# 2235854410/CCVPE

Measured on AMD Instinct MI355X. Metric: query images/sec (VIGOR, 512x512 sat / 320x640 grd), higher is better.
Workload: dtype f32; 1 GPU; vigor_samearea_fov360_b32; variant=vigor_ori_prior, batch_per_gpu=32, global_batch=32, parallelism=image-parallel x1, all_gather of 20 B/query results, schedule=two streams per GPU (aerial encoder + orientation decoder on the second)

## Files before the change

ccvpe_amd/csrc/ccvpe_api.hip:

```cpp
#include "ccvpe_internal.h"

namespace ccvpe { thread_local unsigned long long g_launches = 0; }
static thread_local std::string g_err_storage;
std::string& ccvpe_err() { return g_err_storage; }
int ccvpe_fail(int code, const char* fmt, ...) {
    char buf[1024];
    va_list ap;
    va_start(ap, fmt);
    vsnprintf(buf, sizeof(buf), fmt, ap);
    va_end(ap);
    g_err_storage = buf;
    return code;
}

__global__ __launch_bounds__(256) void checksum_kernel(const uint32_t* __restrict__ p, size_t n, unsigned long long* out) {
    unsigned long long s = 0;
    for (size_t i = (size_t)blockIdx.x * 256 + threadIdx.x; i < n; i += (size_t)gridDim.x * 256) s += (unsigned long long)p[i] * (unsigned long long)((i & 1023) + 1);
    for (int o = 32; o > 0; o >>= 1) s += __shfl_down(s, o);
    if ((threadIdx.x & 63) == 0) atomicAdd(out, s);
}


Switches read_switches() {
    Switches s;
    auto set = [](const char* name) { return getenv(name) != nullptr; };
    auto off = [](const char* name) { const char* e = getenv(name); return e && std::atoi(e) == 0; };
    if (const char* e = getenv("CCVPE_AUTOTUNE")) s.autotune = std::atoi(e) != 0;
    if (const char* e = getenv("CCVPE_FUSE_MBCONV")) s.fuse_mbconv = std::atoi(e);
    if (const char* e = getenv("CCVPE_FUSE_L1")) s.fuse_level1 = std::atoi(e) != 0;
    if (const char* e = getenv("CCVPE_L1_TILE")) s.l1_tile = std::atoi(e);
    if (const char* e = getenv("CCVPE_COMPOSE_L6")) s.compose_l6 = std::atoi(e);
    if (const char* e = getenv("CCVPE_WINOGRAD")) s.wino = std::atoi(e) != 0;
    if (const char* e = getenv("CCVPE_GRAPH")) s.graph_mode = std::atoi(e) != 0;
    if (const char* e = getenv("CCVPE_STREAMS")) s.two_streams = std::atoi(e) >= 2;
    if (const char* e = getenv("CCVPE_PRECISION")) s.precision = (std::string(e) == "bf16x3") ? 1 : 0;
    s.stem_dw = !off("CCVPE_STEM_DW");
    if (const char* e = getenv("CCVPE_FRONT_SPREAD")) s.front_spread = std::atoi(e);
    s.mbconv_image = !off("CCVPE_MBCONV_IMAGE");
    s.se_ticket = !off("CCVPE_SE_TICKET");
    if (const char* e = getenv("CCVPE_SE_PROLOGUE")) s.se_prologue = std::atoi(e) == 1;
    s.split_planes = !set("CCVPE_NO_SPLIT_PLANES");
    s.match_prep_early = !off("CCVPE_MATCH_PREP_EARLY");
    s.match_wide = !off("CCVPE_MATCH_WIDE");
    s.issue_interleaved = !off("CCVPE_ISSUE_ORDER");
    s.log_schedule = set("CCVPE_LOG_SCHEDULE");
    s.no_reuse = set("CCVPE_NO_REUSE");
    s.tune_prefer_pw = set("CCVPE_TUNE_PREFER_PW");
    if (const char* e = getenv("CCVPE_TUNE_PREFER_PROJ")) { s.tune_prefer_proj = true; s.tune_prefer_lat = std::strcmp(e, "lat") == 0; }
    if (const char* e = getenv("CCVPE_TUNE_SPLITK")) s.tune_splitk = std::atoi(e);
    s.tune_no_bf16x3 = set("CCVPE_TUNE_NO_BF16X3");
    s.no_pw = set("CCVPE_NO_PW");
    s.tune_ignore_table = set("CCVPE_TUNE_IGNORE_TABLE");
    s.tune_lat_rows = set("CCVPE_TUNE_LAT_ROWS");
    s.tune_lat_split = set("CCVPE_TUNE_LAT_SPLIT");
    s.tune_no_fused_split = set("CCVPE_TUNE_NO_FUSED_SPLIT");
    if (const char* e = getenv("CCVPE_TUNE_VERBOSE")) s.tune_verbose = e;
    s.no_proj = set("CCVPE_NO_PROJ");
    if (const char* e = getenv("CCVPE_WINO4_MIN_N")) s.wino4_min_n = std::atoi(e);
    s.no_wino4 = set("CCVPE_NO_WINO4");
    s.no_wino4x = set("CCVPE_NO_WINO4X");
    s.pad_concat = !off("CCVPE_PAD_CONCAT");
    if (const char* e = getenv("CCVPE_DIAG_SYNC_BEFORE")) s.diag_sync = e;
    if (const char* e = getenv("CCVPE_DIAG_SNAP")) s.diag_snap = e;
    return s;
}

static int max_micro_batch(const Switches& sw, int variant, float ori_noise, int grd_h, int grd_w) {
    if (variant < 0 || variant > 3) return ccvpe_fail(CCVPE_EINVAL, "unknown variant %d", variant);
    ccvpe_handle_s tmp;
    tmp.cfg.variant = variant; tmp.cfg.ori_noise = ori_noise; tmp.cfg.micro_batch = 1;
    tmp.vs = make_variant(variant);
    tmp.sw = sw;
    tmp.sw.fuse_mbconv = 0; tmp.sw.fuse_level1 = false; tmp.sw.two_streams = false; tmp.sw.graph_mode = 0;
    const int n = (int)(ori_noise / 18.f);
    for (int k = 0; k < 6; ++k) tmp.rolls[k] = (variant == CCVPE_VARIANT_VIGOR_ORI_PRIOR && k > 0) ? 2 * n + 1 : tmp.vs.n_rolls;
    int lo = 0, hi = 1024;
    while (hi - lo > 1) {
        const int mid = (lo + hi) / 2;
        Plan pl;
        PlanKey key;
        key.B = mid; key.gh = grd_h; key.gw = grd_w;
        if (build_plan(&tmp, pl, key) == 0) lo = mid; else hi = mid;
    }
    if (lo == 0) return ccvpe_fail(CCVPE_EINVAL, "ground size %d x %d is not valid for variant %d: %s", grd_h, grd_w, variant, ccvpe_err().c_str());
    return lo;
}

extern "C" {

const char* ccvpe_last_error(void) { return ccvpe_err().c_str(); }
const char* ccvpe_version(void) { return "ccvpe-hip 0.1 (gfx950, fp32 MFMA)"; }
uint64_t ccvpe_launch_count(void) { return ccvpe::g_launches; }

int ccvpe_create(const ccvpe_config* cfg, ccvpe_handle* out) {
    if (!cfg || !out) return ccvpe_fail(CCVPE_EINVAL, "null argument");
    if (cfg->variant < 0 || cfg->variant > 3) return ccvpe_fail(CCVPE_EINVAL, "unknown variant %d", cfg->variant);
    int ndev = 0;
    if (hipGetDeviceCount(&ndev) != hipSuccess || ndev <= 0)
        return ccvpe_fail(CCVPE_EHIP, "no HIP device visible: libccvpe_hip has no CPU fallback");
    if (cfg->device < 0 || cfg->device >= ndev) return ccvpe_fail(CCVPE_EINVAL, "device %d out of range (%d visible)", cfg->device, ndev);
    HIPCHK(hipSetDevice(cfg->device));
    hipDeviceProp_t prop;
    HIPCHK(hipGetDeviceProperties(&prop, cfg->device));
    if (std::string(prop.gcnArchName).find("gfx950") == std::string::npos)
        return ccvpe_fail(CCVPE_EHIP, "device %d is %s; this library carries gfx950 code objects only", cfg->device, prop.gcnArchName);
    auto* h = new ccvpe_handle_s();
    h->cfg = *cfg;
    if (h->cfg.micro_batch <= 0) h->cfg.micro_batch = 32;
    h->vs = make_variant(cfg->variant);
    h->sw = read_switches();
    if (h->sw.precision) h->cfg.reserved[0] = *h->sw.precision;
    if (h->cfg.reserved[0] != 0 && h->cfg.reserved[0] != 1) { delete h; return ccvpe_fail(CCVPE_EINVAL, "unknown precision mode %d", cfg->reserved[0]); }
    const int n = (int)(cfg->ori_noise / 18.f);
    for (int k = 0; k < 6; ++k)
        h->rolls[k] = (cfg->variant == CCVPE_VARIANT_VIGOR_ORI_PRIOR && k > 0) ? 2 * n + 1 : h->vs.n_rolls;
    if (cfg->variant == CCVPE_VARIANT_VIGOR_ORI_PRIOR && (n < 0 || 2 * n + 1 > 32)) {
        delete h;
        return ccvpe_fail(CCVPE_EINVAL, "ori_noise %.1f out of range", cfg->ori_noise);
    }
    build_expect(h);
    *out = h;
    return 0;
}

int ccvpe_max_micro_batch(int32_t variant, float ori_noise, int32_t grd_h, int32_t grd_w) {
    return max_micro_batch(read_switches(), variant, ori_noise, grd_h, grd_w);
}

int ccvpe_destroy(ccvpe_handle h) {
    if (!h) return 0;
    (void)hipSetDevice(h->cfg.device);
    for (void* p : h->dev_allocs) (void)hipFree(p);
    release_level6(h);
    if (h->arena) (void)hipFree(h->arena);
    for (auto* buf : {&h->post_scratch, &h->topk_scratch, &h->prior_scratch}) if (buf->ptr) (void)hipFree(buf->ptr);
    h->plans.clear();
    for (int k = 0; k < 2; ++k) if (h->snap[k]) (void)hipFree(h->snap[k]);
    if (h->capture_stream) (void)hipStreamDestroy(h->capture_stream);
    if (h->aux_stream) (void)hipStreamDestroy(h->aux_stream);
    delete h;
    return 0;
}

int ccvpe_output_channels(ccvpe_handle h, int32_t level) {
    if (!h || level < 0 || level > 5) return ccvpe_fail(CCVPE_EINVAL, "bad level");
    return h->rolls[level];
}

size_t ccvpe_workspace_bytes(ccvpe_handle h, int32_t batch, int32_t grd_h, int32_t grd_w) {
    if (!h || !h->finalized || batch <= 0) { ccvpe_fail(CCVPE_ESTATE, "handle not ready"); return 0; }
    Plan pl;
    PlanKey key;
    key.B = std::min(batch, h->cfg.micro_batch); key.gh = grd_h; key.gw = grd_w;
    if (build_plan(h, pl, key)) return 0;
    return pl.total * sizeof(float);
}

}

static void check_issued_tile(Plan& pl, const Op& op) {
    const int got = conv_tile_last();
    if (!op.tile || (*op.tile & 0xff) == 0 || got == 0) return;
    const int want = *op.tile, ws = (want >> 8) & 0xff, gs = (got >> 8) & 0xff;
    if ((want & 0xff) != (got & 0xff) || (ws > 1 ? ws : 1) != (gs > 1 ? gs : 1))
        std::fprintf(stderr, "ccvpe: launch %s (batch %d) runs %s split %d instead of the planned %s split %d\n", op.name.c_str(), pl.key.B,
                     conv_tile_name(got), gs, conv_tile_name(want), ws);
}

static int run_ops(ccvpe_handle h, Plan& pl, const Ctx& base, hipStream_t s0) {
    const bool check = !pl.tiles_checked;
    pl.tiles_checked = true;
    if (check) (void)conv_tile_last();
    if (!pl.two_streams || h->serial_issue) {
        Ctx c = base;
        c.stream = s0;
        for (auto& op : pl.ops) { op.fn(c); if (check) check_issued_tile(pl, op); }
        base.conv_errors += c.conv_errors;
        return 0;
    }
    if (!h->aux_stream) HIPCHK(hipStreamCreateWithFlags(&h->aux_stream, hipStreamNonBlocking));
    if (pl.events.empty()) {
        pl.events.assign(pl.ops.size() + 2, nullptr);
        for (size_t i = 0; i < pl.events.size(); ++i)
            if (i >= pl.ops.size() || pl.ops[i].signal) HIPCHK(hipEventCreateWithFlags(&pl.events[i], hipEventDisableTiming));
    }
    Ctx c[2] = {base, base};
    hipStream_t st[2] = {s0, h->aux_stream};
    c[0].stream = st[0];
    c[1].stream = st[1];
    pl.set_scratch(c[1], 1);
    const size_t n = pl.ops.size();
    HIPCHK(hipEventRecord(pl.events[n], st[0]));
    HIPCHK(hipStreamWaitEvent(st[1], pl.events[n], 0));
    for (size_t k = 0; k < n; ++k) {
        const size_t i = pl.issue_order.size() == n ? (size_t)pl.issue_order[k] : k;
        Op& op = pl.ops[i];
        for (int d : op.wait_on) HIPCHK(hipStreamWaitEvent(st[op.stream], pl.events[d], 0));
        if (!h->sw.diag_sync.empty() && op.name.find(h->sw.diag_sync) != std::string::npos) HIPCHK(hipDeviceSynchronize());
        const bool snap = !h->sw.diag_snap.empty() && op.name == h->sw.diag_snap;
        auto take_snap = [&](int which) -> int {
            if (!h->snap[0]) {
                h->snap_layout.clear();
                size_t o = 0;
                for (int id : op.uses) { h->snap_layout.push_back({id, o}); o += (pl.size[id] + 63) & ~(size_t)63; }
                h->snap_floats = o;
                for (int k = 0; k < 2; ++k) HIPCHK(hipMalloc((void**)&h->snap[k], o * sizeof(float)));
            }
            for (auto& e : h->snap_layout)
                HIPCHK(hipMemcpyAsync(h->snap[which] + e.second, base.arena + pl.off[e.first], pl.size[e.first] * sizeof(float), hipMemcpyDeviceToDevice, st[op.stream]));
            return 0;
        };
        if (snap) { if (int r = take_snap(0)) return r; }
        op.fn(c[op.stream]);
        if (check) check_issued_tile(pl, op);
        if (snap) { if (int r = take_snap(1)) return r; }
        if (op.signal) HIPCHK(hipEventRecord(pl.events[i], st[op.stream]));
    }
    HIPCHK(hipEventRecord(pl.events[n + 1], st[1]));
    HIPCHK(hipStreamWaitEvent(st[0], pl.events[n + 1], 0));
    base.conv_errors += c[0].conv_errors + c[1].conv_errors;
    return 0;
}

static int micro_batch_cap(ccvpe_handle h, int gh, int gw) {
    int mbmax = h->cfg.micro_batch;
    auto it = h->mb_cap.find({gh, gw});
    if (it == h->mb_cap.end()) {
        const std::string keep = ccvpe_err();
        const int cap = max_micro_batch(h->sw, h->cfg.variant, h->cfg.ori_noise, gh, gw);
        ccvpe_err() = keep;
        it = h->mb_cap.emplace(std::make_pair(gh, gw), cap).first;
    }
    if (it->second > 0) mbmax = std::min(mbmax, it->second);
    return mbmax;
}

static int launch_status(const char* what) {
    hipError_t e = hipGetLastError();
    if (e != hipSuccess) return ccvpe_fail(CCVPE_EHIP, "%s failed: %s", what, hipGetErrorString(e));
    return 0;
}

static Ctx plan_ctx(ccvpe_handle h, const Plan& pl, hipStream_t stream) {
    Ctx c;
    c.arena = h->arena; c.off = &pl.off; c.stream = stream;
    c.tickets = pl.tickets;
    pl.set_scratch(c, 0);
    return c;
}

template <class Slice>
static int for_each_micro_batch(ccvpe_handle h, PlanKey key, int total, hipStream_t stream, Slice slice) {
    const int mbmax = micro_batch_cap(h, key.gh, key.gw);
    for (int pass = 0; pass < 2; ++pass)
        for (int done = 0; done < total; done += key.B) {
            key.B = std::min(mbmax, total - done);
            Plan* pl;
            if (int rc = get_plan(h, key, &pl)) return rc;
            if (pass == 0) continue;
            h->last_plan = pl;
            Ctx c = plan_ctx(h, *pl, stream);
            if (int rc = slice(pl, c, done, key.B)) return rc;
            if (c.conv_errors) return ccvpe_fail(CCVPE_EINVAL, "%d convolution launches were refused (unsupported geometry)", c.conv_errors);
        }
    return 0;
}

static int issue_forward(ccvpe_handle h, Plan* pl, Ctx& c, const ForwardCall& fc, int mb) {
    const int gh = fc.gh, gw = fc.gw;
    const bool profile = fc.profile;
    hipStream_t stream = fc.stream;
    const size_t npx = (size_t)CCVPE_OUT_HW * CCVPE_OUT_HW;
    if (!profile && pl->use_graph && !h->debug) {
        const ccvpe_outputs user = c.out;
        const float* ugrd = c.grd; const float* usat = c.sat;
        c.grd = c.ptr(pl->io_grd); c.sat = c.ptr(pl->io_sat);
        c.out.logits_flattened = c.ptr(pl->io_logits); c.out.heatmap = c.ptr(pl->io_heat); c.out.ori = c.ptr(pl->io_ori);
        for (int k = 0; k < 6; ++k) c.out.matching_score[k] = c.ptr(pl->io_ms[k]);
        {
            const size_t ng = (size_t)mb * 3 * gh * gw, ns = (size_t)mb * 3 * CCVPE_SAT_HW * CCVPE_SAT_HW;
            if (ng % 4 == 0 && ((uintptr_t)ugrd % 16) == 0 && ((uintptr_t)usat % 16) == 0) {
                MultiCopy mc{};
                mc.src[0] = ugrd; mc.dst[0] = (float*)c.grd; mc.n[0] = ng;
                mc.src[1] = usat; mc.dst[1] = (float*)c.sat; mc.n[1] = ns;
                mc.count = 2;
                launch_multi_copy(mc, stream);
            } else {
                HIPCHK(hipMemcpyAsync((void*)c.grd, ugrd, ng * sizeof(float), hipMemcpyDeviceToDevice, stream));
                HIPCHK(hipMemcpyAsync((void*)c.sat, usat, ns * sizeof(float), hipMemcpyDeviceToDevice, stream));
            }
        }
        if (!pl->exec && pl->runs >= 1) {
            hipGraph_t graph = nullptr;
            if (!h->capture_stream) HIPCHK(hipStreamCreateWithFlags(&h->capture_stream, hipStreamNonBlocking));
            HIPCHK(hipStreamBeginCapture(h->capture_stream, hipStreamCaptureModeThreadLocal));
            const int rrc = run_ops(h, *pl, c, h->capture_stream);
            hipError_t ce = hipStreamEndCapture(h->capture_stream, &graph);
            if (rrc) ce = hipErrorUnknown;
            if (ce == hipSuccess && graph) {
                hipGraphExec_t ex = nullptr;
                if (hipGraphInstantiate(&ex, graph, nullptr, nullptr, 0) == hipSuccess) pl->exec = ex;
                (void)hipGraphDestroy(graph);
            }
            if (!pl->exec) { (void)hipGetLastError(); pl->use_graph = false; }
        }
        if (pl->exec) HIPCHK(hipGraphLaunch(pl->exec, stream));
        else if (int rrc = run_ops(h, *pl, c, stream)) return rrc;
        pl->runs++;
        {
            MultiCopy mc{};
            auto add = [&](float* dst, const float* src, size_t n) { mc.src[mc.count] = src; mc.dst[mc.count] = dst; mc.n[mc.count] = n; ++mc.count; };
            add(user.logits_flattened, c.out.logits_flattened, (size_t)mb * npx);
            add(user.heatmap, c.out.heatmap, (size_t)mb * npx);
            add(user.ori, c.out.ori, (size_t)mb * 2 * npx);
            bool aligned = true;
            for (int k = 0; k < 6; ++k) add(user.matching_score[k], c.out.matching_score[k], (size_t)mb * h->rolls[k] * ((size_t)(8 << k) * (8 << k)));
            for (int i = 0; i < mc.count; ++i) aligned = aligned && mc.n[i] % 4 == 0 && ((uintptr_t)mc.dst[i] % 16) == 0 && ((uintptr_t)mc.src[i] % 16) == 0;
            if (aligned) launch_multi_copy(mc, stream);
            else
                for (int i = 0; i < mc.count; ++i) HIPCHK(hipMemcpyAsync(mc.dst[i], mc.src[i], mc.n[i] * sizeof(float), hipMemcpyDeviceToDevice, stream));
        }
    } else if (!profile) {
        if (int rrc = run_ops(h, *pl, c, stream)) return rrc;
    } else {
        hipEvent_t e0, e1;
        HIPCHK(hipEventCreate(&e0));
        HIPCHK(hipEventCreate(&e1));
        for (auto& op : pl->ops) {
            (void)conv_tile_last();
            HIPCHK(hipEventRecord(e0, stream));
            op.fn(c);
            HIPCHK(hipEventRecord(e1, stream));
            HIPCHK(hipEventSynchronize(e1));
            float ms = 0.f;
// ... 1059 lines not shown
```

ccvpe_amd/csrc/ccvpe_internal.h:

```cpp
#pragma once
#include "../../include/ccvpe.h"
#include "kernels.h"

#include <algorithm>
#include <cmath>
#include <cstdarg>
#include <cstdio>
#include <cstdlib>
#include <cstring>
#include <functional>
#include <map>
#include <memory>
#include <optional>
#include <set>
#include <string>
#include <type_traits>
#include <vector>

using namespace ccvpe;

std::string& ccvpe_err();
int ccvpe_fail(int code, const char* fmt, ...);
#define HIPCHK(expr)                                                                           \
    do {                                                                                       \
        hipError_t _e = (expr);                                                                \
        if (_e != hipSuccess) return ccvpe_fail(CCVPE_EHIP, "%s failed: %s", #expr, hipGetErrorString(_e)); \
    } while (0)

struct BlockSpec { int e, k, s, cin, cout; };
static const BlockSpec B0[16] = {
    {1, 3, 1, 32, 16}, {6, 3, 2, 16, 24}, {6, 3, 1, 24, 24}, {6, 5, 2, 24, 40}, {6, 5, 1, 40, 40},
    {6, 3, 2, 40, 80}, {6, 3, 1, 80, 80}, {6, 3, 1, 80, 80}, {6, 5, 1, 80, 112}, {6, 5, 1, 112, 112},
    {6, 5, 1, 112, 112}, {6, 5, 2, 112, 192}, {6, 5, 1, 192, 192}, {6, 5, 1, 192, 192}, {6, 5, 1, 192, 192},
    {6, 3, 1, 192, 320},
};
static const int TAP_BLOCK[5] = {15, 10, 4, 2, 0};
static const float BN_EPS = 1e-3f;

struct DecLevel { int din, dout, skip, mid, out; };
struct VariantSpec {
    int feat_h;
    int head_ch[6];
    int sat_desc;
    int match_ch[6];
    int step[6];
    int n_rolls;
    int centre;
    DecLevel loc[6], ori[6];
};
static const DecLevel VIGOR_LOC[6] = {{1281, 1024, 320, 640, 640}, {641, 320, 112, 320, 320}, {321, 160, 40, 160, 160},
                                      {161, 80, 24, 80, 80},       {81, 40, 16, 40, 40},      {41, 16, 0, 16, 1}};
static const DecLevel VIGOR_ORI[6] = {{1300, 1024, 320, 640, 640}, {640, 256, 112, 256, 256}, {256, 128, 40, 128, 128},
                                      {128, 64, 24, 64, 64},       {64, 32, 16, 32, 32},      {32, 16, 0, 16, 2}};
static const DecLevel KITTI_LOC[6] = {{2049, 1024, 320, 512, 512}, {513, 256, 112, 256, 256}, {257, 128, 40, 128, 128},
                                      {129, 64, 24, 128, 128},     {129, 32, 16, 32, 32},     {33, 16, 0, 16, 1}};
static const DecLevel KITTI_ORI[6] = {{2064, 1024, 320, 512, 512}, {512, 256, 112, 256, 256}, {256, 128, 40, 128, 128},
                                      {128, 64, 24, 64, 64},       {64, 32, 16, 32, 32},      {32, 16, 0, 16, 2}};

static VariantSpec make_variant(int v) {
    VariantSpec s{};
    auto cp = [](DecLevel* d, const DecLevel* src) { for (int i = 0; i < 6; ++i) d[i] = src[i]; };
    if (v == CCVPE_VARIANT_KITTI) {
        s.feat_h = 8;
        int hc[6] = {16, 8, 4, 2, 1, 1}, mc[6] = {2048, 512, 256, 128, 128, 32}, st[6] = {128, 64, 32, 16, 8, 8};
        for (int i = 0; i < 6; ++i) { s.head_ch[i] = hc[i]; s.match_ch[i] = mc[i]; s.step[i] = st[i]; }
        s.sat_desc = 2048; s.n_rolls = 16; s.centre = 0;
        cp(s.loc, KITTI_LOC); cp(s.ori, KITTI_ORI);
    } else {
        int mc[6] = {1280, 640, 320, 160, 80, 40}, st[6] = {64, 32, 16, 8, 4, 2};
        int hv[6] = {64, 32, 16, 8, 4, 2}, ho[6] = {32, 16, 8, 4, 2, 1};
        for (int i = 0; i < 6; ++i) {
            s.match_ch[i] = mc[i]; s.step[i] = st[i];
            s.head_ch[i] = (v == CCVPE_VARIANT_OXFORD) ? ho[i] : hv[i];
        }
        s.feat_h = (v == CCVPE_VARIANT_OXFORD) ? 4 : 10;
        s.sat_desc = 1280; s.n_rolls = 20; s.centre = (v == CCVPE_VARIANT_OXFORD);
        cp(s.loc, VIGOR_LOC); cp(s.ori, VIGOR_ORI);
    }
    return s;
}

static void static_pad(int k, int s, int& lo, int& hi) {
    if (s == 1) { lo = hi = (k - 1) / 2; return; }
    int total = k - 2;
    lo = total / 2; hi = total - lo;
}
static int conv_out(int n, int k, int s) {
    int lo, hi; static_pad(k, s, lo, hi);
    return (n + lo + hi - k) / s + 1;
}
static int se_squeeze(int cin) { return std::max(1, (int)(cin * 0.25)); }
static int round_up(int a, int b) { return (a + b - 1) / b * b; }
static int deconv_width(const DecLevel& l, bool pad) {
    return (pad && l.skip > 0 && (l.dout * 4) % 64 != 0) ? round_up(l.dout, 16) : l.dout;
}

struct Switches {
    bool autotune = true;
    int fuse_mbconv = 1;
    bool fuse_level1 = true;
    int l1_tile = 1;
    std::optional<int> compose_l6;
    bool wino = true;
    int graph_mode = 0;
    bool two_streams = true;
    std::optional<int> precision;
    bool stem_dw = true;
    std::optional<int> front_spread;
    bool mbconv_image = true;
    bool se_ticket = true;
    bool se_prologue = false;
    bool split_planes = true;
    bool match_prep_early = true;
    bool match_wide = true;
    bool issue_interleaved = true;
    bool log_schedule = false;
    bool no_reuse = false;
    bool tune_prefer_pw = false;
    bool tune_prefer_proj = false;
    bool tune_prefer_lat = false;
    std::optional<int> tune_splitk;
    bool tune_no_bf16x3 = false;
    bool no_pw = false;
    bool tune_ignore_table = false;
    bool tune_lat_rows = false;
    bool tune_lat_split = false;
    bool tune_no_fused_split = false;
    std::string tune_verbose;
    bool no_proj = false;
    int wino4_min_n = 40;
    bool no_wino4 = false;
    bool no_wino4x = false;
    bool pad_concat = true;
    std::string diag_sync, diag_snap;

    bool tune_filtered() const {
        return tune_prefer_pw || tune_prefer_proj || tune_splitk || tune_no_bf16x3 || no_pw || tune_ignore_table || tune_lat_rows || tune_lat_split ||
               tune_no_fused_split;
    }
    std::string pack_group() const {
        std::string s;
        if (no_proj) s += "CCVPE_NO_PROJ=1;";
        if (wino4_min_n != 40) s += "CCVPE_WINO4_MIN_N=" + std::to_string(wino4_min_n) + ";";
        if (no_wino4) s += "CCVPE_NO_WINO4=1;";
        if (no_wino4x) s += "CCVPE_NO_WINO4X=1;";
        if (!pad_concat) s += "CCVPE_PAD_CONCAT=0;";
        return s;
    }
};
Switches read_switches();

struct PackedConv {
    float* w = nullptr;
    unsigned short *w_hi = nullptr, *w_lo = nullptr;
    float* bias = nullptr;
    int N = 0, Kpad = 0, nchunks = 0, cinp = 0, KH = 1, KW = 1;
    float* wino = nullptr;
    int wino_n16 = 0;
    size_t wino_bytes = 0;
    float* wino4 = nullptr;
    size_t wino4_bytes = 0;
    float* wino4x = nullptr;
    size_t wino4x_bytes = 0;
    int wino4x_cfg = -1;
    float* proj = nullptr;
    size_t proj_bytes = 0;
};
struct BlockW {
    PackedConv expand, project;
    float* exp_lin = nullptr;
    int exp_cinp = 0;
    float *dw_w = nullptr, *dw_b = nullptr, *se_w1 = nullptr, *se_b1 = nullptr, *se_w2 = nullptr, *se_b2 = nullptr;
    int sq = 0;
};
struct EncoderW {
    float *stem_w = nullptr, *stem_b = nullptr;
    BlockW blk[16];
    PackedConv head;
};
struct DecoderW {
    PackedConv deconv[6], conva[6], convb[5];
    float* tail_w = nullptr;
    float* l1_wt = nullptr;
    float tail_b[2] = {0.f, 0.f};
    float *l1_wc = nullptr, *l1_ws = nullptr, *l1_bc = nullptr;
    int l1_cx = 0, l1_cxp = 0, l1_c0 = 0, l1_ng = 0, l1_score = 0;
};
struct Level6W {
    float* wc = nullptr;
    float* bc = nullptr;
    PackedConv skip;
    int K = 0, Kc = 0, N = 0, Npad = 0;
};
static constexpr int LEVEL6_AUTO_MIN_BATCH = 8;
struct ccvpe_handle_s;
struct DecoderW;
int level6_shape(const ccvpe_handle_s* h, const DecoderW& d, const struct DecLevel& l, int& K, int& Kc, int& N, int& Npad);
int ensure_level6(ccvpe_handle_s* h, int wm);
void release_level6(ccvpe_handle_s* h);
int compose_level1(ccvpe_handle_s* h, DecoderW& d, const std::vector<float>& w, const std::vector<float>& b, const std::vector<float>& wa,
                   const std::vector<float>& ba, int cin, int nscore);
int pack_level1_tail(ccvpe_handle_s* h, DecoderW& d, const std::vector<float>& w2, const std::vector<float>& b2, int cout);

struct Tensor {
    int id = -1; int B = 0, H = 0, W = 0, C = 0;
    bool split = false;
    long long numel() const { return (long long)B * H * W * C; }
};

struct Ctx {
    float* arena = nullptr;
    const std::vector<size_t>* off = nullptr;
    hipStream_t stream = nullptr;
    const float* grd = nullptr;
    const float* sat = nullptr;
    ccvpe_outputs out{};
    float* splitk_scratch = nullptr;
    size_t splitk_floats = 0;
    unsigned* tickets = nullptr;
    const float* cache_in = nullptr;
    float* cache_out = nullptr;
    float* rows = nullptr;
    int topk_k = 0, topk_r = 0;
    const int* tile_index = nullptr;
    int n_tiles = 0;
    const float* grd_cache_in = nullptr;
    const int* query_index = nullptr;
    int n_queries = 0;
    float* stats = nullptr;
    const float* log_prior = nullptr;
    long long prior_stride = 0;
    float* posterior = nullptr;
    float* summary = nullptr;
    int summary_r = 0;
    float* heading = nullptr;
    float* hist = nullptr;
    int heading_bins = 0, heading_r = 0;
    float* ptr(const Tensor& t) const { return arena + (*off)[t.id]; }
    Dst dst(const Tensor& t, int coff = 0) const { return Dst{ptr(t), t.C, coff, t.split ? 1 : 0, t.numel()}; }
    mutable int conv_errors = 0;
    mutable size_t conv_tick_off = 0;
    mutable ConvParams* probe = nullptr;
    void launch_conv(ConvParams& p, int cfg) const {
        p.tickets = tickets ? tickets + conv_tick_off : nullptr;
        p.partial = splitk_scratch;
        p.partial_floats = splitk_floats;
        if (probe) { *probe = p; return; }
        if (launch_conv_igemm(p, cfg, stream) != 0) ++conv_errors;
    }
};

struct PlanKey {
    int B = 0, gh = 0, gw = 0;
    int mode = 0;
    bool pose = false;
    bool topk = false;
    bool summary = false;
    bool heading = false;
    bool operator==(const PlanKey& o) const {
        return B == o.B && gh == o.gh && gw == o.gw && mode == o.mode && pose == o.pose && topk == o.topk && summary == o.summary &&
               heading == o.heading;
    }
};

struct ForwardCall {
    const float* grd = nullptr;
    int gh = 0, gw = 0;
    const float* sat = nullptr;
    const float* cache = nullptr;
    const int32_t* tile_index = nullptr;
    int n_tiles = 0;
    int batch = 0;
    const ccvpe_outputs* out = nullptr;
    float* rows = nullptr;
    int topk_k = 0, topk_r = 0;
    const float* log_prior = nullptr;
    long long prior_stride = 0;
    float* posterior = nullptr;
    float* summary = nullptr;
    int summary_r = 0;
    float* heading = nullptr;
    float* hist = nullptr;
    int heading_bins = 0, heading_r = 0;
    hipStream_t stream = nullptr;
    bool profile = false;
    PlanKey plan_key() const {
        PlanKey key;
        key.gh = gh; key.gw = gw; key.mode = cache ? 2 : 0; key.pose = rows != nullptr; key.topk = rows && topk_k > 0;
        key.summary = rows && summary;
        key.heading = rows && heading;
        return key;
    }
};

struct Op {
    std::string name;
    std::function<void(const Ctx&)> fn;
    std::vector<int> uses;
    double flops = 0, bytes = 0;
    std::shared_ptr<int> tile;
    int gemm_m = 0, gemm_n = 0, gemm_kpad = 0;
    int conv_cin = 0;
    bool bf16x3_only = false;
    bool wino_ok = false;
    bool wino4_ok = false;
    bool wino4x_ok = false;
    bool is_pw = false;
    bool proj_ok = false;
    int stream = 0;
    std::vector<int> wait_on;
    bool signal = false;
};

struct TapInfo { Tensor t; int coff; int C; };

struct Plan {
    PlanKey key;
    bool debug = false;
    std::vector<size_t> size;
    std::vector<size_t> off;
    std::vector<Op> ops;
    std::map<std::string, TapInfo> taps;
    size_t total = 0;
    float* arena = nullptr;
    Tensor scratch;
    bool use_graph = false;
    Tensor io_grd, io_sat, io_logits, io_heat, io_ori, io_ms[6];
    Tensor tune_cache;
    hipGraphExec_t exec = nullptr;
    int runs = 0;
    size_t ticket_words = 0;
    unsigned* tickets = nullptr;
    size_t alloc_tickets(size_t n) { const size_t o = ticket_words; ticket_words += (n + 15) & ~(size_t)15; return o; }
    int l6_wm = 0;
    bool tiles_checked = false;
    bool two_streams = false;
    Tensor scratch2;
    std::vector<hipEvent_t> events;
    std::vector<int> issue_order;
    bool issue_interleaved = true, log_schedule = false, no_reuse = false;
    ~Plan() {
        if (exec) (void)hipGraphExecDestroy(exec);
        for (hipEvent_t e : events) if (e) (void)hipEventDestroy(e);
        if (tickets) (void)hipFree(tickets);
    }
    void schedule() {
        if (!two_streams) return;
        bool any = false;
        for (auto& o : ops) {
            o.stream = (o.name.rfind("sat.", 0) == 0 || o.name.rfind("ori", 0) == 0) ? 1 : 0;
            any = any || o.stream == 1;
            o.wait_on.clear();
            o.signal = false;
        }
        if (!any) { two_streams = false; return; }
        std::map<int, int> last_use;
        for (int i = 0; i < (int)ops.size(); ++i) {
            int dep = -1;
            for (int id : ops[i].uses) {
                auto it = last_use.find(id);
                if (it != last_use.end() && ops[it->second].stream != ops[i].stream) dep = std::max(dep, it->second);
            }
            if (dep >= 0) { ops[i].wait_on.push_back(dep); ops[dep].signal = true; }
            for (int id : ops[i].uses) last_use[id] = i;
        }
        issue_order.clear();
        {
            std::vector<int> q[2];
            for (int i = 0; i < (int)ops.size(); ++i) q[ops[i].stream].push_back(i);
            size_t p[2] = {0, 0};
            std::vector<bool> issued(ops.size(), false);
            while (issue_interleaved && (p[0] < q[0].size() || p[1] < q[1].size())) {
                auto ready = [&](int s) {
                    if (p[s] >= q[s].size()) return false;
                    for (int d : ops[q[s][p[s]]].wait_on) if (!issued[d]) return false;
                    return true;
                };
                const bool r0 = ready(0), r1 = ready(1);
                int s;
                if (r0 && r1) s = (p[1] * q[0].size() < p[0] * q[1].size()) ? 1 : 0;
                else if (r0 || r1) s = r0 ? 0 : 1;
                else { issue_order.clear(); break; }
                const int i = q[s][p[s]++];
                issued[i] = true;
                issue_order.push_back(i);
            }
            if (issue_order.size() != ops.size()) { issue_order.resize(ops.size()); for (int i = 0; i < (int)ops.size(); ++i) issue_order[i] = i; }
        }
        if (log_schedule)
            for (int i = 0; i < (int)ops.size(); ++i) {
                std::fprintf(stderr, "op %3d s%d %-28s wait=%d uses=", i, ops[i].stream, ops[i].name.c_str(), ops[i].wait_on.empty() ? -1 : ops[i].wait_on[0]);
                for (int id : ops[i].uses) std::fprintf(stderr, "%d ", id);
                std::fprintf(stderr, "\n");
            }
    }
    static constexpr size_t SPLITK_FLOATS = 32u << 20;
    void set_scratch(Ctx& c, int stream) const {
        const Tensor& sk = stream ? scratch2 : scratch;
        c.splitk_scratch = c.ptr(sk); c.splitk_floats = SPLITK_FLOATS;
    }

    size_t max_tensor_bytes = 0;
    int max_dims[4] = {0, 0, 0, 0};
    Tensor alloc(int B_, int H, int W, int C) {
        Tensor t; t.id = (int)size.size(); t.B = B_; t.H = H; t.W = W; t.C = C;
        size.push_back((size_t)B_ * H * W * C);
        if (size.back() * sizeof(float) > max_tensor_bytes) {
            max_tensor_bytes = size.back() * sizeof(float);
            max_dims[0] = B_; max_dims[1] = H; max_dims[2] = W; max_dims[3] = C;
        }
        return t;
    }
    void add(const std::string& name, std::vector<Tensor> uses, std::function<void(const Ctx&)> fn, double flops = 0, double bytes = 0) {
        Op o; o.name = name; o.fn = std::move(fn); o.flops = flops; o.bytes = bytes;
        for (auto& t : uses) o.uses.push_back(t.id);
        ops.push_back(std::move(o));
    }
    void add_conv(const std::string& name, std::vector<Tensor> uses, int gemm_m, int gemm_n, int gemm_kpad,
                  std::function<void(const Ctx&, int)> fn, double flops, double bytes) {
        auto tp = std::make_shared<int>(TILE_AUTO);
        const size_t toff = alloc_tickets(CONV_TICKETS);
        add(name, std::move(uses), [fn, tp, toff](const Ctx& c) { c.conv_tick_off = toff; fn(c, *tp); }, flops, bytes);
        ops.back().tile = tp;
        ops.back().gemm_m = gemm_m;
        ops.back().gemm_n = gemm_n;
        ops.back().gemm_kpad = gemm_kpad;
    }
    void assign() {
        const int n = (int)size.size();
        std::vector<int> first(n, 1 << 30), last(n, -1), smask(n, 0);
        for (int i = 0; i < (int)ops.size(); ++i)
            for (int id : ops[i].uses) {
                first[id] = std::min(first[id], i); last[id] = std::max(last[id], i);
                smask[id] |= 1 << (two_streams ? ops[i].stream : 0);
            }
        std::vector<bool> pinned(n, false);
        auto pin = [&](const Tensor& t) { if (t.id >= 0) { pinned[t.id] = true; first[t.id] = 0; last[t.id] = 1 << 30; } };
        if (debug || no_reuse) for (int i = 0; i < n; ++i) if (last[i] >= 0) pinned[i] = true;
        pin(scratch); pin(scratch2); pin(tune_cache);
        if (use_graph)
            for (const Tensor* t : {&io_grd, &io_sat, &io_logits, &io_heat, &io_ori, &io_ms[0], &io_ms[1], &io_ms[2], &io_ms[3], &io_ms[4], &io_ms[5]}) pin(*t);
        for (int i = 0; i < n; ++i) if (smask[i] == 3) pinned[i] = true;
        off.assign(n, 0);
        std::vector<int> order(n);
        for (int i = 0; i < n; ++i) order[i] = i;
        std::stable_sort(order.begin(), order.end(), [&](int a, int b) { return first[a] < first[b]; });
        auto granule = [&](int id) { return (size[id] + 63) & ~(size_t)63; };
        total = 0;
        for (int pool = 1; pool <= 2; ++pool) {
            const size_t base = total;
            std::vector<int> placed;
            for (int id : order) {
                if (last[id] < 0 || pinned[id] || smask[id] != pool) continue;
                const size_t sz = granule(id);
                std::vector<std::pair<size_t, size_t>> busy;
                for (int o : placed)
                    if (!(last[o] < first[id] || last[id] < first[o])) busy.push_back({off[o], off[o] + granule(o)});
                std::sort(busy.begin(), busy.end());
                size_t pos = base;
                for (auto& iv : busy) {
                    if (pos + sz <= iv.first) break;
                    pos = std::max(pos, iv.second);
                }
                off[id] = pos;
                total = std::max(total, pos + sz);
                placed.push_back(id);
            }
        }
        for (int id : order) {
            if (last[id] < 0 || !pinned[id]) continue;
            off[id] = total;
            total += granule(id);
        }
    }
};

struct ccvpe_handle_s {
    ccvpe_config cfg{};
    VariantSpec vs{};
    int rolls[6] = {0};
    std::map<std::string, std::vector<int64_t>> expect;
    std::map<std::string, std::vector<float>> host;
    std::set<std::string> skipped;
    bool finalized = false;
    bool debug = false;
    Switches sw;
    hipStream_t capture_stream = nullptr;
    hipStream_t aux_stream = nullptr;
    bool serial_issue = false;
    std::vector<void*> dev_allocs;
    std::vector<size_t> dev_alloc_bytes;
    EncoderW grd_enc, sat_enc;
    PackedConv grd_heads, sat_desc;
    float* grd_wh[6] = {nullptr};
    float grd_b2[6] = {0};
    DecoderW loc, ori;
    Level6W l6[2];
    int l6_wm = 0;
    std::vector<void*> l6_allocs;
    bool l6_failed = false;
    std::vector<std::unique_ptr<Plan>> plans;
    Plan* last_plan = nullptr;
    float* snap[2] = {nullptr, nullptr};
    size_t snap_floats = 0;
    std::vector<std::pair<int, size_t>> snap_layout;
    std::map<std::pair<int, int>, int> mb_cap;
    std::map<std::string, std::pair<std::string, int>> tuning;
    int tuned_plans = 0;
    float* arena = nullptr;
    size_t arena_floats = 0;
    struct Scratch { void* ptr = nullptr; int batch = 0; };
    Scratch post_scratch;
    Scratch topk_scratch;
    Scratch prior_scratch;
    struct Row { std::string name; float ms; double flops, bytes, issued; };
    std::vector<Row> prof;
};


void build_expect(ccvpe_handle_s* h);
int pack_conv(ccvpe_handle_s* h, PackedConv& pc, int N, int taps, int cin, int cinp, const std::vector<int>& cmap,
              const std::function<float(int, int, int)>& get, const std::vector<float>& bias, int KH, int KW);
std::vector<int> identity_map(int n);
static inline int score_pad(int nscore) { return round_up(nscore, 8); }

ConvParams conv_params(const PackedConv& pc, const float* in, int in_ld, int B, int H, int W, int OH, int OW,
                       int stride, int pad_t, int pad_l, int act);
size_t cache_layout(const VariantSpec& vs, int B, size_t off[6]);
int ground_desc_floats(const ccvpe_handle_s* h, int gh, int gw);
int build_plan(ccvpe_handle_s* h, Plan& pl, const PlanKey& key);

int autotune_plan(ccvpe_handle_s* h, Plan& pl, const std::vector<bool>* known = nullptr);
int get_plan(ccvpe_handle_s* h, const PlanKey& key, Plan** out);
std::string tuning_key(ccvpe_handle_s* h, const Plan& pl, const Op& op);
```

ccvpe_amd/csrc/ccvpe_plan.hip:

```cpp
#include "ccvpe_internal.h"

static int window_offset(const VariantSpec& vs, int level, int L) {
    const int C = vs.match_ch[level];
    return vs.centre ? (int)((double)C / 2 - (double)L / 2) : 0;
}
static int mod(int a, int m) { int r = a % m; return r < 0 ? r + m : r; }

ConvParams conv_params(const PackedConv& pc, const float* in, int in_ld, int B, int H, int W, int OH, int OW,
                              int stride, int pad_t, int pad_l, int act) {
    ConvParams p{};
    p.in = in; p.in_ld = in_ld; p.B = B; p.H = H; p.W = W; p.Cin = pc.cinp; p.OH = OH; p.OW = OW;
    p.KH = pc.KH; p.KW = pc.KW; p.stride = stride; p.pad_t = pad_t; p.pad_l = pad_l;
    p.wpk = pc.w; p.w_hi = pc.w_hi; p.w_lo = pc.w_lo; p.Kpad = pc.Kpad; p.Npad = round_up(pc.N, conv_igemm_npad()); p.nchunks = pc.nchunks; p.bias = pc.bias; p.N = pc.N; p.act = act;
    p.gate = nullptr; p.resid = nullptr; p.resid_ld = 0; p.ndst = 0; p.mode = MODE_CONV; p.deconv_cout = 0;
    p.M = B * OH * OW;
    p.in_bytes = (unsigned)((size_t)B * H * W * in_ld * sizeof(float));
    p.gate_bytes = (unsigned)((size_t)B * pc.cinp * sizeof(float));
    p.w_plane_bytes = (unsigned)((size_t)p.Npad * pc.Kpad * sizeof(unsigned short));
    p.wino_w = pc.wino; p.wino_n16 = pc.wino_n16; p.wino_bytes = (unsigned)pc.wino_bytes;
    p.wino4_w = pc.wino4; p.wino4_bytes = (unsigned)pc.wino4_bytes;
    p.wino4x_w = pc.wino4x; p.wino4x_bytes = (unsigned)pc.wino4x_bytes; p.wino4x_cfg = pc.wino4x_cfg;
    p.proj_w = pc.proj; p.proj_bytes = (unsigned)pc.proj_bytes;
    return p;
}

struct EncOut { Tensor vol; Tensor tap[16]; };

struct TapDst { Tensor t[2]; int coff[2]; int n = 0; };

static void plan_encoder(ccvpe_handle_s* h, Plan& pl, const EncoderW& ew, bool is_grd, int B, int H, int W, bool circular,
                         const TapDst* tapdst, EncOut& out, const std::string& tag) {
    int lo, hi;
    static_pad(3, 2, lo, hi);
    int ch = conv_out(H, 3, 2), cw = conv_out(W, 3, 2);
    const bool stem_dw = h->sw.stem_dw && B0[0].e == 1 && B0[0].k == 3 && B0[0].s == 1 && B0[0].cin == 32 && !(circular && (W & 1)) &&
                         (size_t)B * 3 * H * W * sizeof(float) < ((size_t)1 << 31);
    StemParams stem_sp{};
    stem_sp.B = B; stem_sp.H = H; stem_sp.W = W; stem_sp.OH = ch; stem_sp.OW = cw; stem_sp.pad_t = lo; stem_sp.pad_l = lo; stem_sp.circular = circular;
    stem_sp.w = ew.stem_w; stem_sp.bias = ew.stem_b;
    Tensor cur = stem_dw ? Tensor{} : pl.alloc(B, ch, cw, 32);
    if (!stem_dw) {
        const StemParams sp = stem_sp;
        Tensor o = cur;
        pl.add(tag + ".stem", {o}, [sp, o, is_grd](const Ctx& c) {
            StemParams q = sp; q.in = is_grd ? c.grd : c.sat; q.out = c.ptr(o);
            launch_stem(q, c.stream);
        }, 2.0 * B * ch * cw * 32 * 27, 4.0 * B * (3.0 * H * W + 32.0 * ch * cw));
    }
    for (int i = 0; i < 16; ++i) {
        const BlockSpec& b = B0[i];
        const BlockW& bw = ew.blk[i];
        const int mid = b.cin * b.e;
        const std::string bn = tag + ".b" + std::to_string(i);
        Tensor xin = cur;
        Tensor e = xin;
        static_pad(b.k, b.s, lo, hi);
        const int oh = conv_out(ch, b.k, b.s), ow = conv_out(cw, b.k, b.s);
        MbFrontParams mp{};
        mp.B = B; mp.H = ch; mp.W = cw; mp.Cin = b.cin; mp.cinp = bw.exp_cinp; mp.mid = mid;
        mp.we = bw.exp_lin; mp.be = bw.expand.bias; mp.wd = bw.dw_w; mp.bd = bw.dw_b;
        mp.k = b.k; mp.s = b.s; mp.pad_t = lo; mp.pad_l = lo; mp.circular = circular; mp.OH = oh; mp.OW = ow;
        {
            const double share = (double)H * W / ((double)H * W + (double)CCVPE_SAT_HW * CCVPE_SAT_HW);
            const int dflt = is_grd ? std::max(64, std::min(128, (int)(256.0 * share / 16.0 + 0.5) * 16)) : 144;
            mp.spread = h->sw.front_spread.value_or(dflt);
        }
        const bool image = b.e != 1 && bw.exp_lin != nullptr && h->sw.fuse_mbconv != 0 && h->sw.mbconv_image && mbconv_image_supported(mp);
        const bool fused = image || (b.e != 1 && bw.exp_lin != nullptr && mbconv_front_supported(b.k, b.s, b.cin, mid) &&
                           (h->sw.fuse_mbconv == 2 || (h->sw.fuse_mbconv == 1 && mbconv_front_profitable(b.k))));
        Tensor d = pl.alloc(B, oh, ow, mid);
        const bool with_stem = stem_dw && i == 0;
        const bool ticket_on = h->sw.se_ticket && mid <= 1152 && bw.sq <= 64;
        const int trows = !ticket_on ? 0 : with_stem ? stem_dw_tiles(oh, ow) : image ? mbconv_image_ticket_rows(mp) : fused ? mbconv_front_ticket_rows(mp) : 0;
        bool sep = false;
        if (trows > 0 && image && bw.project.proj != nullptr && h->cfg.reserved[0] == 0 && h->sw.se_prologue) {
            ConvParams q = conv_params(bw.project, nullptr, mid, B, oh, ow, oh, ow, 1, 0, 0, ACT_NONE);
            q.M = B * oh * ow;
            q.se_rows = reinterpret_cast<const float*>(1); q.se_nrows = trows * (mid / 16); q.se_sq = bw.sq;
            sep = conv_proj_supported(q, 101);
        }
        const bool ticket = trows > 0 && !sep;
        const int S = ticket ? trows : with_stem ? stem_dw_tiles(oh, ow) : image ? mbconv_image_strips(mp) : fused ? mbconv_front_tiles(b.k, b.s, oh, ow) : depthwise_strip_lanes(B, oh, ow, mid, b.k, b.s);
        Tensor pool = pl.alloc(B, 1, S, mid);
        Tensor gate = pl.alloc(B, 1, 1, mid);
        SeTicket se{};
        size_t tick_off = 0;
        if (sep) {
            se.per_sample = trows * (mid / 16);
            se.S = trows; se.C = mid; se.SQ = bw.sq; se.inv_hw = 1.f / (float)(oh * ow);
            se.w1 = bw.se_w1;
        }
        if (ticket) {
            tick_off = pl.alloc_tickets((size_t)B);
            se.per_sample = with_stem ? S : image ? S * (mid / 16) : S * mbconv_front_ticket_split(mp);
            se.S = S; se.C = mid; se.SQ = bw.sq; se.inv_hw = 1.f / (float)(oh * ow);
            se.w1 = bw.se_w1; se.b1 = bw.se_b1; se.w2 = bw.se_w2; se.b2 = bw.se_b2;
            se.spec = (long long)B * se.per_sample <= 256 ? 1 : 0;
        }
        const bool parts = (ticket && image) || sep;
        Tensor sqp = parts ? pl.alloc(B, 1, se.per_sample, bw.sq) : Tensor{};
        auto fill_se = [=](const Ctx& c) {
            SeTicket t = se;
            if (ticket) { t.counter = c.tickets + tick_off; t.pool = c.ptr(pool); t.gate = c.ptr(gate); }
            if (parts) t.sqpart = c.ptr(sqp);
            return t;
        };
        const double se_flops = ticket ? 4.0 * B * mid * bw.sq : 0.0;
        if (with_stem) {
            StemDwParams sd{};
            sd.st = stem_sp; sd.wd = bw.dw_w; sd.bd = bw.dw_b;
            std::vector<Tensor> uses = {d, pool};
            if (ticket) uses.push_back(gate);
            pl.add(tag + ".stem_b0dw", uses, [=](const Ctx& c) {
                StemDwParams q = sd; q.st.in = is_grd ? c.grd : c.sat; q.out = c.ptr(d); q.pool_partial = c.ptr(pool); q.se = fill_se(c);
                launch_stem_dw(q, c.stream);
            }, 2.0 * B * ch * cw * 32 * 27 + 2.0 * B * oh * ow * mid * 9 + se_flops, 4.0 * B * (3.0 * H * W + 32.0 * oh * ow));
        } else if (fused) {
            std::vector<Tensor> uses = {xin, d, pool};
            if (ticket) uses.push_back(gate);
            if (parts) uses.push_back(sqp);
            (void)sep;
            pl.add(bn + ".expand_dw", uses, [=](const Ctx& c) {
                MbFrontParams q = mp; q.x = c.ptr(xin); q.out = c.ptr(d); q.pool = c.ptr(pool); q.se = fill_se(c);
                if (image) launch_mbconv_image(q, c.stream); else launch_mbconv_front(q, c.stream);
            }, 2.0 * B * ch * cw * b.cin * mid + 2.0 * B * oh * ow * mid * b.k * b.k + se_flops, 4.0 * B * ((double)ch * cw * b.cin + (double)oh * ow * mid));
        } else {
        if (b.e != 1) {
            e = pl.alloc(B, ch, cw, mid);
            const PackedConv* pc = &bw.expand;
            const int hh = ch, ww = cw;
            pl.add_conv(bn + ".expand", {xin, e}, B * hh * ww, pc->N, pc->Kpad, [=](const Ctx& c, int tile) {
                ConvParams p = conv_params(*pc, c.ptr(xin), xin.C, B, hh, ww, hh, ww, 1, 0, 0, ACT_SWISH);
                p.dst[0] = {c.ptr(e), mid, 0}; p.ndst = 1;
                c.launch_conv(p, tile);
            }, 2.0 * B * ch * cw * b.cin * mid, 4.0 * B * ch * cw * (b.cin + mid));
            pl.ops.back().is_pw = true;
        }
        {
            DwParams dp{};
            dp.B = B; dp.H = ch; dp.W = cw; dp.C = mid; dp.OH = oh; dp.OW = ow; dp.k = b.k; dp.stride = b.s;
            dp.pad_t = lo; dp.pad_l = lo; dp.circular = circular; dp.w = bw.dw_w; dp.bias = bw.dw_b; dp.S = S;
            pl.add(bn + ".dw", {e, d, pool}, [=](const Ctx& c) {
                DwParams q = dp; q.in = c.ptr(e); q.out = c.ptr(d); q.pool_partial = c.ptr(pool);
                launch_depthwise(q, c.stream);
            }, 2.0 * B * oh * ow * mid * b.k * b.k, 4.0 * B * mid * ((double)ch * cw + (double)oh * ow));
        }
        }
        const int SC = std::max(1, std::min(16, S / 32));
        Tensor pooled = pl.alloc(B, 1, SC, mid);
        Tensor sqt = pl.alloc(B, 1, 1, 64);
        if (!ticket && !sep) {
            SeParams sp{};
            sp.B = B; sp.S = S; sp.C = mid; sp.SQ = bw.sq; sp.inv_hw = 1.f / (float)(oh * ow); sp.SC = SC;
            sp.w1 = bw.se_w1; sp.b1 = bw.se_b1; sp.w2 = bw.se_w2; sp.b2 = bw.se_b2;
            pl.add(bn + ".se", {pool, gate, pooled, sqt}, [=](const Ctx& c) {
                SeParams q = sp; q.pool_partial = c.ptr(pool); q.gate = c.ptr(gate); q.pooled = c.ptr(pooled); q.sq = c.ptr(sqt);
                launch_se(q, c.stream);
            }, 4.0 * B * mid * bw.sq, 4.0 * B * S * mid);
        }
        Tensor o = pl.alloc(B, oh, ow, b.cout);
        {
            const PackedConv* pc = &bw.project;
            const bool skip = (b.s == 1 && b.cin == b.cout);
            TapDst td;
            if (tapdst) for (int t = 0; t < 5; ++t) if (TAP_BLOCK[t] == i) td = tapdst[t];
            std::vector<Tensor> uses = {d, sep ? sqp : gate, o};
            if (skip) uses.push_back(xin);
            for (int t = 0; t < td.n; ++t) uses.push_back(td.t[t]);
            const int se_nrows = se.per_sample, se_sq = bw.sq;
            const float se_inv = se.inv_hw;
            const float *se_b1 = bw.se_b1, *se_w2 = bw.se_w2, *se_b2 = bw.se_b2;
            pl.add_conv(bn + (sep ? ".se_project" : ".project"), uses, B * oh * ow, pc->N, pc->Kpad, [=](const Ctx& c, int tile) {
                ConvParams p = conv_params(*pc, c.ptr(d), mid, B, oh, ow, oh, ow, 1, 0, 0, ACT_NONE);
                if (sep) {
                    p.se_rows = c.ptr(sqp); p.se_nrows = se_nrows; p.se_sq = se_sq; p.se_inv_hw = se_inv; p.se_b1 = se_b1; p.se_w2 = se_w2; p.se_b2 = se_b2;
                    tile = conv_proj_lat_tile();
                } else {
                    p.gate = c.ptr(gate);
                }
                if (skip) { p.resid = c.ptr(xin); p.resid_ld = xin.C; }
                p.dst[0] = {c.ptr(o), o.C, 0}; p.ndst = 1;
                for (int t = 0; t < td.n; ++t) p.dst[p.ndst++] = c.dst(td.t[t], td.coff[t]);
                c.launch_conv(p, tile);
            }, 2.0 * B * oh * ow * mid * b.cout + (sep ? 4.0 * B * mid * bw.sq : 0.0), 4.0 * B * oh * ow * (mid + b.cout * (1 + td.n)));
            pl.ops.back().is_pw = true;
            pl.ops.back().proj_ok = pc->proj != nullptr && h->cfg.reserved[0] == 0;
            if (sep) pl.ops.back().tile.reset();
        }
        out.tap[i] = o;
        pl.taps[tag + "_block" + std::to_string(i)] = {o, 0, o.C};
        cur = o; ch = oh; cw = ow;
    }
    Tensor vol = pl.alloc(B, ch, cw, 1280);
    {
        const PackedConv* pc = &ew.head;
        Tensor x = cur;
        const int hh = ch, ww = cw;
        pl.add_conv(tag + ".head", {x, vol}, B * hh * ww, pc->N, pc->Kpad, [=](const Ctx& c, int tile) {
            ConvParams p = conv_params(*pc, c.ptr(x), x.C, B, hh, ww, hh, ww, 1, 0, 0, ACT_SWISH);
            p.dst[0] = {c.ptr(vol), 1280, 0}; p.ndst = 1;
            c.launch_conv(p, tile);
        }, 2.0 * B * ch * cw * 320 * 1280, 4.0 * B * ch * cw * 1600);
        pl.ops.back().is_pw = true;
    }
    out.vol = vol;
    pl.taps[tag + "_volume"] = {vol, 0, 1280};
}

static const int TAP_HW[5] = {256, 1024, 4096, 16384, 65536};
static const int TAP_C[5] = {320, 112, 40, 24, 16};
size_t cache_layout(const VariantSpec& vs, int B, size_t off[6]) {
    size_t o = 0;
    off[0] = o; o += (size_t)B * 64 * vs.sat_desc;
    for (int t = 0; t < 5; ++t) { off[t + 1] = o; o += (size_t)B * TAP_HW[t] * TAP_C[t]; }
    return o;
}

static int build_aerial_plan(ccvpe_handle_s* h, Plan& pl, int B);
static int build_ground_plan(ccvpe_handle_s* h, Plan& pl, int B, int gh, int gw);
extern "C" int ccvpe_max_micro_batch(int32_t variant, float ori_noise, int32_t grd_h, int32_t grd_w);

static int grd_geometry(const VariantSpec& vs, bool circular, int gh, int gw, int& fh, int& fw, int L[6]) {
    if (gh <= 0 || gw <= 0) return ccvpe_fail(CCVPE_EINVAL, "ground image size %d x %d is not positive", gh, gw);
    fh = gh; fw = gw;
    for (int i = -1; i < 16; ++i) {
        const int k = i < 0 ? 3 : B0[i].k, s = i < 0 ? 2 : B0[i].s;
        int lo, hi;
        static_pad(k, s, lo, hi);
        const std::string layer = i < 0 ? "the stem" : "block " + std::to_string(i);
        if (fh + lo + hi < k || fw + lo + hi < k)
            return ccvpe_fail(CCVPE_EINVAL, "ground image %d x %d is too small: it reaches the %d x %d kernel of %s as %d x %d", gh, gw, k, k,
                              layer.c_str(), fh, fw);
        if (circular && fw < std::max(lo, hi))
            return ccvpe_fail(CCVPE_EINVAL, "ground image %d x %d is too narrow for circular padding: %s pads %d columns around a width of %d "
                              "(the padding would wrap more than once)", gh, gw, layer.c_str(), std::max(lo, hi), fw);
        fh = conv_out(fh, k, s); fw = conv_out(fw, k, s);
    }
    if (fh != vs.feat_h)
        return ccvpe_fail(CCVPE_EINVAL, "ground image %dx%d gives a %d-row feature volume, the descriptor heads expect %d rows", gh, gw, fh, vs.feat_h);
    for (int k = 0; k < 6; ++k) {
        L[k] = fw * vs.head_ch[k];
        if (L[k] > vs.match_ch[k])
            return ccvpe_fail(CCVPE_EINVAL, "descriptor length %d exceeds aerial channels %d at level %d", L[k], vs.match_ch[k], k + 1);
    }
    return 0;
}

int ground_desc_floats(const ccvpe_handle_s* h, int gh, int gw) {
    int fh, fw, L[6];
    if (int rc = grd_geometry(h->vs, h->cfg.circular_padding != 0, gh, gw, fh, fw, L)) return rc;
    int ltot = 0;
    for (int k = 0; k < 6; ++k) ltot += round_up(L[k], 4);
    return ltot;
}

static Tensor plan_grd_desc(ccvpe_handle_s* h, Plan& pl, int B, int fh, int fw, Tensor vol, bool to_cache) {
    const VariantSpec& vs = h->vs;
    int ntot = 0, ltot = 0, hoff[6], loff[6];
    for (int k = 0; k < 6; ++k) { hoff[k] = ntot; ntot += vs.head_ch[k]; loff[k] = ltot; ltot += round_up(fw * vs.head_ch[k], 4); }
    Tensor ghead = pl.alloc(B, fh, fw, ntot);
    Tensor desc = to_cache ? Tensor{} : pl.alloc(B, 1, 1, ltot);
    const PackedConv* pc = &h->grd_heads;
    Tensor x = vol;
    pl.add_conv("grd.heads", {x, ghead}, B * fh * fw, pc->N, pc->Kpad, [=](const Ctx& c, int tile) {
        ConvParams p = conv_params(*pc, c.ptr(x), 1280, B, fh, fw, fh, fw, 1, 0, 0, ACT_NONE);
        p.dst[0] = {c.ptr(ghead), ntot, 0}; p.ndst = 1;
        c.launch_conv(p, tile);
    }, 2.0 * B * fh * fw * 1280 * ntot, 4.0 * B * fh * fw * (1280 + ntot));
    pl.ops.back().is_pw = true;
    pl.ops.back().proj_ok = pc->proj != nullptr && h->cfg.reserved[0] == 0;
    GrdDescParams gp{};
    gp.B = B; gp.Hf = fh; gp.Wf = fw; gp.Ntot = ntot; gp.nlev = 6; gp.Ltot = ltot;
    for (int k = 0; k < 6; ++k) { gp.c[k] = vs.head_ch[k]; gp.off[k] = hoff[k]; gp.wh[k] = h->grd_wh[k]; gp.b2[k] = h->grd_b2[k]; gp.loff[k] = loff[k]; }
    std::vector<Tensor> uses = {ghead};
    if (!to_cache) uses.push_back(desc);
    pl.add("grd.desc", uses, [=](const Ctx& c) {
        GrdDescParams q = gp; q.y = c.ptr(ghead); q.desc = to_cache ? c.cache_out : c.ptr(desc);
        launch_grd_desc(q, c.stream);
    }, 2.0 * B * fh * fw * ntot, 4.0 * B * fh * fw * ntot);
    return desc;
}

int build_plan(ccvpe_handle_s* h, Plan& pl, const PlanKey& key) {
    const int B = key.B, gh = key.gh, gw = key.gw, mode = key.mode;
    const bool pose = key.pose;
    pl.key = key;
    pl.key.topk = pose && key.topk;
    pl.key.summary = pose && !key.topk && key.summary;
    pl.key.heading = key.heading;
    if (key.heading && (!pose || key.topk || mode == 4)) return ccvpe_fail(CCVPE_EINVAL, "heading plans are argmax pose plans (no top-K, no pairs)");
    if (mode == 1) return build_aerial_plan(h, pl, B);
    if (mode == 3) return build_ground_plan(h, pl, B, gh, gw);
    const bool cached = mode == 2 || mode == 4;
    const bool grd_cached = mode == 4;
    if (grd_cached && (!pose || key.topk)) return ccvpe_fail(CCVPE_EINVAL, "pair plans are single-hypothesis pose plans");
    const VariantSpec& vs = h->vs;
    pl.debug = h->debug;
    pl.scratch = pl.alloc(1, 1, 1, (int)Plan::SPLITK_FLOATS);
    pl.two_streams = h->sw.two_streams && !h->debug;
    pl.issue_interleaved = h->sw.issue_interleaved; pl.log_schedule = h->sw.log_schedule; pl.no_reuse = h->sw.no_reuse;
    if (pl.two_streams) pl.scratch2 = pl.alloc(1, 1, 1, (int)Plan::SPLITK_FLOATS);
    pl.use_graph = !cached && !pose && h->sw.graph_mode == 1;
    if (pl.use_graph) {
        pl.io_grd = pl.alloc(B, 3, gh, gw);
        pl.io_sat = pl.alloc(B, 3, CCVPE_SAT_HW, CCVPE_SAT_HW);
        pl.io_logits = pl.alloc(B, 1, CCVPE_OUT_HW, CCVPE_OUT_HW);
        pl.io_heat = pl.alloc(B, 1, CCVPE_OUT_HW, CCVPE_OUT_HW);
        pl.io_ori = pl.alloc(B, 2, CCVPE_OUT_HW, CCVPE_OUT_HW);
        for (int k = 0; k < 6; ++k) pl.io_ms[k] = pl.alloc(B, h->rolls[k], 8 << k, 8 << k);
    }

    int fh, fw, L[6];
    if (int rc = grd_geometry(vs, h->cfg.circular_padding != 0, gh, gw, fh, fw, L)) return rc;

    const int D = vs.sat_desc;
    const int rfull = vs.n_rolls;
    const int rpad = score_pad(rfull);
    Tensor loc_in[6], ori_in6;
    Tensor loc_cat[6], ori_cat[6];
    for (int j = 0; j < 6; ++j) {
        const int hw_in = 8 << j;
        loc_in[j] = pl.alloc(B, hw_in, hw_in, 8 + vs.match_ch[j]);
        loc_cat[j] = pl.alloc(B, hw_in * 2, hw_in * 2, deconv_width(vs.loc[j], h->sw.pad_concat) + vs.loc[j].skip);
        ori_cat[j] = pl.alloc(B, hw_in * 2, hw_in * 2, deconv_width(vs.ori[j], h->sw.pad_concat) + vs.ori[j].skip);
        if (h->cfg.reserved[0] == 1 && j < 5 && h->sw.split_planes) { loc_cat[j].split = true; ori_cat[j].split = true; }
    }
    const bool l6_forced = h->sw.compose_l6 && (*h->sw.compose_l6 == 1 || *h->sw.compose_l6 == 2);
    int l6_wm = !h->finalized || h->cfg.reserved[0] != 0 || !h->sw.wino ? 0
                : h->sw.compose_l6 ? (*h->sw.compose_l6 == 1 ? 4 : *h->sw.compose_l6 == 2 ? 2 : 0)
                : (B >= LEVEL6_AUTO_MIN_BATCH && !h->l6_failed) ? 4 : 0;
    Level6Params l6p[2] = {};
    if (l6_wm) {
        bool ok = true;
        for (int d = 0; d < 2; ++d) {
            Level6Params& q = l6p[d];
            q.wm = l6_wm; q.B = B;
            ok = ok && level6_shape(h, d ? h->ori : h->loc, d ? vs.ori[0] : vs.loc[0], q.K, q.Kc, q.N, q.Npad) == 0;
            q.R = level6_rows(B, l6_wm, &q.bm);
            ok = ok && level6_supported(q) && q.K == (d ? rpad + D : loc_in[0].C);
        }
        if (!ok && l6_forced) return ccvpe_fail(CCVPE_ESTATE, "composed level 6: the packed weights do not fit the plan's level-6 inputs");
        if (!ok) l6_wm = 0;
    }
    pl.l6_wm = l6_wm;
    Tensor skip15;
    ori_in6 = pl.alloc(B, 8, 8, rpad + D);
    pl.taps["ori_in6"] = {ori_in6, 0, ori_in6.C};

    EncOut genc, senc;
    if (!grd_cached) plan_encoder(h, pl, h->grd_enc, true, B, gh, gw, h->cfg.circular_padding != 0, nullptr, genc, "grd");
    TapDst td[5];
    for (int t = 0; t < 5; ++t) {
        td[t].n = 2;
        td[t].t[0] = loc_cat[t]; td[t].coff[0] = deconv_width(vs.loc[t], h->sw.pad_concat);
        td[t].t[1] = ori_cat[t]; td[t].coff[1] = deconv_width(vs.ori[t], h->sw.pad_concat);
    }
    if (l6_wm) td[0].n = 0;
    size_t coff[6];
    cache_layout(vs, B, coff);
    if (!cached) {
        plan_encoder(h, pl, h->sat_enc, false, B, CCVPE_SAT_HW, CCVPE_SAT_HW, false, td, senc, "sat");
        skip15 = senc.tap[TAP_BLOCK[0]];
    } else {
        if (l6_wm) skip15 = pl.alloc(B, 16, 16, TAP_C[0]);
        size_t one[6];
        cache_layout(vs, 1, one);
        for (int t = 0; t < 5; ++t) {
            Tensor lc = loc_cat[t], oc = ori_cat[t];
            const int lcoff = deconv_width(vs.loc[t], h->sw.pad_concat), ocoff = deconv_width(vs.ori[t], h->sw.pad_concat);
            const size_t src_off = coff[t + 1], src_off1 = one[t + 1];
            const int C = TAP_C[t], hw = TAP_HW[t];
            const long long P = (long long)B * TAP_HW[t];
            if (t == 0 && l6_wm) {
                const Tensor sk = skip15;
                pl.add("sat.cached_tap" + std::to_string(TAP_BLOCK[t]), {sk}, [=](const Ctx& c) {
                    if (c.tile_index)
                        launch_gather_channels(c.cache_in + src_off1 * c.n_tiles, C, hw, c.tile_index, B, c.dst(sk), Dst{nullptr, 0, 0, 0, 0}, 1, c.stream);
                    else
                        launch_scatter_channels(c.cache_in + src_off, C, P, c.dst(sk), Dst{nullptr, 0, 0, 0, 0}, 1, c.stream);
                }, 0, 4.0 * P * C * 2);
                continue;
            }
            pl.add("sat.cached_tap" + std::to_string(TAP_BLOCK[t]), {lc, oc}, [=](const Ctx& c) {
                if (c.tile_index)
                    launch_gather_channels(c.cache_in + src_off1 * c.n_tiles, C, hw, c.tile_index, B, c.dst(lc, lcoff), c.dst(oc, ocoff), 2, c.stream);
                else
                    launch_scatter_channels(c.cache_in + src_off, C, P, c.dst(lc, lcoff), c.dst(oc, ocoff), 2, c.stream);
            }, 0, 4.0 * P * C * 3);
        }
    }

    int ltot = 0, loff[6];
    for (int k = 0; k < 6; ++k) { loff[k] = ltot; ltot += round_up(L[k], 4); }
    Tensor desc;
    if (grd_cached) {
        desc = pl.alloc(B, 1, 1, ltot);
        Tensor d = desc;
        pl.add("grd.cached_desc", {d}, [=](const Ctx& c) {
            launch_gather_channels(c.grd_cache_in, ltot, 1, c.query_index, B, c.dst(d), Dst{nullptr, 0, 0, 0, 0}, 1, c.stream);
        }, 0, 8.0 * B * ltot);
    } else {
        desc = plan_grd_desc(h, pl, B, fh, fw, genc.vol, false);
    }
    for (int k = 0; k < 6; ++k) pl.taps["grd_desc" + std::to_string(k + 1)] = {desc, loff[k], L[k]};

    Tensor dmap = pl.alloc(B, 8, 8, D);
    if (cached) {
        Tensor dm = dmap;
        const long long P = (long long)B * 64;
        pl.add("sat.cached_descmap", {dm}, [=](const Ctx& c) {
            if (c.tile_index)
                launch_gather_channels(c.cache_in, D, 64, c.tile_index, B, c.dst(dm), Dst{nullptr, 0, 0, 0, 0}, 1, c.stream);
            else
                launch_scatter_channels(c.cache_in, D, P, c.dst(dm), Dst{nullptr, 0, 0, 0, 0}, 1, c.stream);
        }, 0, 8.0 * P * D);
        pl.taps["sat_descriptor_map"] = {dmap, 0, D};
    } else {
        const PackedConv* pc = &h->sat_desc;
        Tensor x = senc.vol;
        pl.add_conv("sat.descmap", {x, dmap}, B * 8 * 8, pc->N, pc->Kpad, [=](const Ctx& c, int tile) {
            ConvParams p = conv_params(*pc, c.ptr(x), 1280, B, 16, 16, 8, 8, 2, 0, 0, ACT_NONE);
            p.dst[0] = {c.ptr(dmap), D, 0}; p.ndst = 1;
            c.launch_conv(p, tile);
        }, 2.0 * B * 64 * 5120.0 * D, 4.0 * (B * 256 * 1280.0 + 5120.0 * D));
        pl.ops.back().proj_ok = pc->proj != nullptr && h->cfg.reserved[0] == 0;
        pl.taps["sat_descriptor_map"] = {dmap, 0, D};
    }

    auto plan_level = [&](const DecoderW& dw, const DecLevel* lv, int j, Tensor din, Tensor cat, const std::string& tag) -> Tensor {
        const int hin = 8 << j, hout = hin * 2;
        const DecLevel& l = lv[j];
        Tensor mid = pl.alloc(B, hout, hout, l.mid);
        if (j == 0 && l6_wm) {
            const Level6W* w6 = &h->l6[&dw == &h->ori ? 1 : 0];
            const Level6Params lp = l6p[&dw == &h->ori ? 1 : 0];
            const int G = 4 * level6_positions(l6_wm);
            Tensor V = pl.alloc(G, 1, lp.R, lp.Kc), Mp = pl.alloc(G, 1, lp.R, lp.N), sk = pl.alloc(B, hout, hout, l.mid);
            const Tensor s15 = skip15;
            pl.add(tag + ".l6_transform", {din, V}, [=](const Ctx& c) {
                Level6Params q = lp; q.x = c.ptr(din); q.v = c.ptr(V);
                launch_level6_transform(q, c.stream);
            }, 0.0, 4.0 * ((double)din.numel() + (double)V.numel()));
            pl.add(tag + ".l6_gemm", {V, Mp}, [=](const Ctx& c) {
                Level6Params q = lp; q.v = c.ptr(V); q.wc = w6->wc; q.mp = c.ptr(Mp);
                launch_level6_gemm(q, c.stream);
            }, 2.0 * G * lp.R * (double)lp.N * lp.Kc, 4.0 * ((double)V.numel() + (double)G * lp.Npad * lp.Kc + (double)Mp.numel()));
            {
                const PackedConv* pc = &w6->skip;
                pl.add_conv(tag + ".conv_skip", {s15, sk}, B * hout * hout, lp.N, round_up(9 * l.skip, 32), [=](const Ctx& c, int tile) {
                    ConvParams p = conv_params(*pc, c.ptr(s15), s15.C, B, hout, hout, hout, hout, 1, 1, 1, ACT_NONE);
                    p.dst[0] = c.dst(sk); p.ndst = 1;
                    c.launch_conv(p, tile);
                }, 2.0 * B * hout * hout * 9.0 * s15.C * l.mid, 4.0 * B * hout * hout * ((double)s15.C + l.mid));
                pl.ops.back().conv_cin = s15.C;
                pl.ops.back().wino_ok = l.skip % 8 == 0;
                pl.ops.back().wino4_ok = pl.ops.back().wino_ok && lp.N >= h->sw.wino4_min_n && !h->sw.no_wino4;
                pl.ops.back().wino4x_ok = pl.ops.back().wino_ok && lp.N >= 24 && conv_wino4x_config(lp.N) >= 0 && !h->sw.no_wino4x;
            }
            pl.add(tag + ".l6_combine", {Mp, sk, mid}, [=](const Ctx& c) {
                Level6Params q = lp; q.mp = c.ptr(Mp); q.skip = c.ptr(sk); q.bc = w6->bc; q.out = c.ptr(mid);
                launch_level6_combine(q, c.stream);
            }, 0.0, 4.0 * ((double)Mp.numel() + 2.0 * (double)mid.numel()));
        } else {
            {
                const PackedConv* pc = &dw.deconv[j];
                const int cout = deconv_width(l, h->sw.pad_concat);
                pl.add_conv(tag + ".deconv", {din, cat}, B * hin * hin, pc->N, pc->Kpad, [=](const Ctx& c, int tile) {
                    ConvParams p = conv_params(*pc, c.ptr(din), din.C, B, hin, hin, hin, hin, 1, 0, 0, ACT_NONE);
                    p.mode = MODE_DECONV; p.deconv_cout = cout;
                    p.dst[0] = c.dst(cat); p.ndst = 1;
                    c.launch_conv(p, tile);
                }, 2.0 * B * hin * hin * (double)l.din * 4 * l.dout, 4.0 * B * hin * hin * ((double)din.C + 4.0 * l.dout));
                pl.ops.back().is_pw = !din.split;
                pl.ops.back().proj_ok = pc->proj != nullptr && !din.split && h->cfg.reserved[0] == 0;
            }
            mid.split = cat.split;
            {
                const PackedConv* pc = &dw.conva[j];
                pl.add_conv(tag + ".conv_a", {cat, mid}, B * hout * hout, pc->N, pc->Kpad, [=](const Ctx& c, int tile) {
                    ConvParams p = conv_params(*pc, c.ptr(cat), cat.C, B, hout, hout, hout, hout, 1, 1, 1, ACT_RELU);
                    p.in_split = cat.split; p.in_plane_bytes = (unsigned)(cat.numel() * 2);
                    p.dst[0] = c.dst(mid); p.ndst = 1;
                    c.launch_conv(p, tile);
                }, 2.0 * B * hout * hout * 9.0 * cat.C * l.mid, 4.0 * B * hout * hout * ((double)cat.C + l.mid));
                pl.ops.back().bf16x3_only = cat.split;
                pl.ops.back().conv_cin = cat.C;
                pl.ops.back().wino_ok = pc->wino != nullptr && !cat.split && h->sw.wino && h->cfg.reserved[0] == 0;
                pl.ops.back().wino4_ok = pl.ops.back().wino_ok && pc->wino4 != nullptr;
                pl.ops.back().wino4x_ok = pl.ops.back().wino_ok && pc->wino4x != nullptr;
            }
        }
        if (j == 5) return mid;
        Tensor o = pl.alloc(B, hout, hout, l.out);
        {
            const PackedConv* pc = &dw.convb[j];
            pl.add_conv(tag + ".conv_b", {mid, o}, B * hout * hout, pc->N, pc->Kpad, [=](const Ctx& c, int tile) {
                ConvParams p = conv_params(*pc, c.ptr(mid), mid.C, B, hout, hout, hout, hout, 1, 1, 1, ACT_NONE);
                p.in_split = mid.split; p.in_plane_bytes = (unsigned)(mid.numel() * 2);
                p.dst[0] = {c.ptr(o), o.C, 0}; p.ndst = 1;
                c.launch_conv(p, tile);
            }, 2.0 * B * hout * hout * 9.0 * l.mid * l.out, 4.0 * B * hout * hout * ((double)l.mid + l.out));
            pl.ops.back().bf16x3_only = mid.split;
            pl.ops.back().conv_cin = mid.C;
            pl.ops.back().wino_ok = pc->wino != nullptr && !mid.split && h->sw.wino && h->cfg.reserved[0] == 0;
            pl.ops.back().wino4_ok = pl.ops.back().wino_ok && pc->wino4 != nullptr;
            pl.ops.back().wino4x_ok = pl.ops.back().wino_ok && pc->wino4x != nullptr;
        }
        return o;
    };

    auto plan_level1_fused = [&](const DecoderW& dw, Tensor din, int cin_real, int cout, bool is_ori, Tensor raw, const std::string& tag, Tensor out_ws = Tensor{}) {
        Level1Params lp{};
        lp.x_ld = din.C; lp.cx = dw.l1_cx; lp.cxp = dw.l1_cxp; lp.B = B; lp.H = CCVPE_OUT_HW; lp.W = CCVPE_OUT_HW;
        lp.c0 = dw.l1_c0; lp.ng = dw.l1_ng; lp.score = dw.l1_score; lp.wc = dw.l1_wc; lp.ws = dw.l1_ws; lp.bc = dw.l1_bc; lp.wt = dw.l1_wt;
        lp.bt[0] = dw.tail_b[0]; lp.bt[1] = dw.tail_b[1]; lp.cout = cout; lp.normalize = is_ori ? 1 : 0;
        lp.tile = h->sw.l1_tile;
        const bool has_raw = raw.id >= 0;
        std::vector<Tensor> uses = {din};
        if (has_raw) uses.push_back(raw);
        if (out_ws.id >= 0) uses.push_back(out_ws);
        const double px = (double)B * CCVPE_OUT_HW * CCVPE_OUT_HW;
        pl.add(tag + ".fused", uses, [=](const Ctx& c) {
            Level1Params q = lp;
            q.x = c.ptr(din);
            q.out = out_ws.id >= 0 ? c.ptr(out_ws) : is_ori ? c.out.ori : c.out.logits_flattened;
            q.raw = has_raw ? c.ptr(raw) : nullptr;
            launch_level1(q, c.stream);
        }, px / 4 * 2.0 * cin_real * 64 + px * 2.0 * 144 * 16 + px * 2.0 * 144 * cout, 4.0 * (px / 4 * lp.cx + px * cout));
    };

    Tensor x = dmap;
    Tensor loc_mid;
    const Tensor logits_ws = pose ? pl.alloc(B, 1, CCVPE_OUT_HW, CCVPE_OUT_HW) : Tensor{};
    const bool prep_early = h->sw.match_prep_early;
    size_t first_match_op = (size_t)-1;
    std::vector<std::function<MatchParams(const Ctx&)>> prep_fills;
    std::vector<Tensor> prep_uses;
    for (int k = 0; k < 6; ++k) {
        MatchParams mp{};
        const int hw = (8 << k) * (8 << k);
        const int C = vs.match_ch[k];
        mp.x_ld = x.C; mp.B = B; mp.HW = hw; mp.C = C; mp.g_ld = ltot; mp.L = L[k];
        const int off = window_offset(vs, k, L[k]);
        const bool prior = h->cfg.variant == CCVPE_VARIANT_VIGOR_ORI_PRIOR;
        const int n = prior ? (int)(h->cfg.ori_noise / 18.f) : 0;
        if (k == 0 || !prior) {
            mp.R = rfull;
            for (int r = 0; r < rfull; ++r) mp.shift[r] = mod(off + r * vs.step[k], C);
            mp.inmax = 0;
            if (prior) { for (int i = -n; i <= n; ++i) mp.inmax |= 1u << mod(i, rfull); }
            else mp.inmax = rfull >= 32 ? 0xffffffffu : ((1u << rfull) - 1u);
        } else {
            mp.R = 2 * n + 1;
            for (int r = 0; r < mp.R; ++r) mp.shift[r] = mod(off + (r - n) * vs.step[k], C);
            mp.inmax = (mp.R >= 32) ? 0xffffffffu : ((1u << mp.R) - 1u);
        }
        mp.rpad = rpad;
        mp.P = match_pixels_per_block(hw, C);
        mp.no_wide = h->sw.match_wide ? 0 : 1;
        mp.cat_max_ld = 8 + C;
        mp.cat_all_ld = rpad + C;
        Tensor xin = x, lin = loc_in[k];
        Tensor ggs = pl.alloc(B, 1, 1, (int)match_scratch_floats(C));
        const bool first = (k == 0);
        const int goff = loff[k];
        const int R = mp.R;
        std::vector<Tensor> uses = {xin, desc, lin, ggs};
        if (first) uses.push_back(ori_in6);
        mp.prep_done = prep_early ? 1 : 0;
        auto fill = [=](const Ctx& c) {
            MatchParams q = mp;
            q.x = c.ptr(xin); q.g = c.ptr(desc) + goff;
            q.ms = pose ? nullptr : c.out.matching_score[k];
            q.cat_max = c.ptr(lin);
            q.cat_all = first ? c.ptr(ori_in6) : nullptr;
            q.gg_scratch = c.ptr(ggs);
            return q;
        };
        if (first_match_op == (size_t)-1) first_match_op = pl.ops.size();
        if (prep_early) {
            prep_fills.push_back(fill);
            if (prep_uses.empty()) prep_uses.push_back(desc);
            prep_uses.push_back(ggs);
        }
        pl.add("match" + std::to_string(k + 1), uses, [=](const Ctx& c) { launch_match(fill(c), c.stream); },
               4.0 * B * hw * (double)R * L[k], 4.0 * B * hw * (2.0 * C + R + 8));
        pl.taps["loc_in" + std::to_string(6 - k)] = {lin, 0, lin.C};
        if (k == 5 && h->sw.fuse_level1) { plan_level1_fused(h->loc, lin, vs.loc[5].din, 1, false, Tensor{}, "loc1", logits_ws); break; }
        Tensor o = plan_level(h->loc, vs.loc, k, lin, loc_cat[k], "loc" + std::to_string(6 - k));
        if (k < 5) { pl.taps["loc_level" + std::to_string(6 - k)] = {o, 0, o.C}; x = o; }
        else loc_mid = o;
    }
    if (!prep_fills.empty()) {
        const size_t n0 = pl.ops.size();
        pl.add("match.prep", prep_uses, [prep_fills](const Ctx& c) {
            MatchParams ps[6];
            const int n = (int)std::min<size_t>(prep_fills.size(), 6);
            for (int i = 0; i < n; ++i) ps[i] = prep_fills[i](c);
            launch_match_prep_all(ps, n, c.stream);
        }, 0.0, 0.0);
        std::rotate(pl.ops.begin() + first_match_op, pl.ops.begin() + n0, pl.ops.end());
    }
    if (!h->sw.fuse_level1) {
        Tensor m = loc_mid;
        const float* tw = h->loc.tail_w;
        const float tb = h->loc.tail_b[0];
        std::vector<Tensor> uses = {m};
        if (pose) uses.push_back(logits_ws);
        pl.add("loc1.tail", uses, [=](const Ctx& c) {
            TailConvParams p{};
            p.in = c.ptr(m); p.B = B; p.H = CCVPE_OUT_HW; p.W = CCVPE_OUT_HW; p.w = tw; p.bias[0] = tb; p.cout = 1;
            p.normalize = 0; p.out = pose ? c.ptr(logits_ws) : c.out.logits_flattened; p.raw = nullptr;
            launch_tail_conv(p, c.stream);
        }, 2.0 * B * 262144.0 * 144, 4.0 * B * 262144.0 * 17);
    }
    Tensor pose_index;
    Tensor pose_part;
    const bool heading = pl.key.heading;
    if (pose) {
        static_assert(CCVPE_OUT_HW * CCVPE_OUT_HW == 64 * 4096, "pose_argmax_kernel: 64 chunks of 4096 values");
        const bool topk = pl.key.topk;
        Tensor part = pl.alloc(B, 1, 64, 2), keys = pl.alloc(B, 1, 64, topk ? 2 * TOPK_MAX_K : 2);
        pose_index = pl.alloc(B, 1, 1, topk ? TOPK_MAX_K : 1);
        pose_part = part;
        static_assert(sizeof(double) == 2 * sizeof(float), "the hand-off is allocated in floats");
        const bool summ = pl.key.summary;
        const Tensor spart = summ ? pl.alloc(B, 1, 64, 2 * SUMMARY_PART) : Tensor{};
        const Tensor lg = logits_ws, idx = pose_index;
        pl.add("softmax.partial", {lg, part}, [=](const Ctx& c) {
            SoftmaxParams p{};
            p.logits = c.ptr(lg); p.B = B; p.n = CCVPE_OUT_HW * CCVPE_OUT_HW; p.partial = c.ptr(part); p.chunks = 64; p.out = nullptr;
            p.prior = c.log_prior; p.prior_stride = c.prior_stride;
            launch_softmax_partial(p, c.stream);
        }, 0, 4.0 * B * 262144.0);
        const size_t toff = pl.alloc_tickets((size_t)B);
        if (topk) pl.add("topk.peaks", {lg, part, keys, idx}, [=](const Ctx& c) {
            TopkParams p{};
            p.heat = nullptr; p.logits = c.ptr(lg); p.partial = c.ptr(part); p.B = B; p.k = c.topk_k; p.r = c.topk_r;
            p.keys = reinterpret_cast<unsigned long long*>(c.ptr(keys)); p.tickets = c.tickets + toff;
            p.index = reinterpret_cast<int*>(c.ptr(idx)); p.rows = c.rows;
            p.prior = c.log_prior; p.prior_stride = c.prior_stride;
            launch_topk_peaks(p, c.stream);
        }, 0, 4.0 * B * 262144.0);
        else pl.add("pose.argmax", summ ? std::vector<Tensor>{lg, part, keys, idx, spart} : std::vector<Tensor>{lg, part, keys, idx}, [=](const Ctx& c) {
            PoseArgmaxParams p{};
            p.logits = c.ptr(lg); p.partial = c.ptr(part); p.B = B; p.n = CCVPE_OUT_HW * CCVPE_OUT_HW; p.chunks = 64;
            p.pairs = c.ptr(keys); p.tickets = c.tickets + toff; p.index = reinterpret_cast<int*>(c.ptr(idx)); p.rows = c.rows;
            p.stats = c.stats; p.prior = c.log_prior; p.prior_stride = c.prior_stride; p.posterior = c.posterior;
            if (summ) { p.summary = c.summary; p.summ_part = reinterpret_cast<double*>(c.ptr(spart)); p.summary_r = c.summary_r; }
            launch_pose_argmax(p, c.stream);
        }, 0, 4.0 * B * 262144.0);
    } else {
        Tensor part = pl.alloc(B, 1, 64, 2);
        pl.add("softmax", {part}, [=](const Ctx& c) {
            SoftmaxParams p{};
            p.logits = c.out.logits_flattened; p.B = B; p.n = CCVPE_OUT_HW * CCVPE_OUT_HW; p.partial = c.ptr(part); p.chunks = 64;
            p.out = c.out.heatmap;
            launch_softmax(p, c.stream);
        }, 0, 4.0 * B * 262144.0 * 3);
    }
    {
        Tensor xo = ori_in6;
        Tensor ori_mid;
        Tensor raw;
        Tensor ori_field;
        if (h->debug && !pose) { raw = pl.alloc(B, 2, CCVPE_OUT_HW, CCVPE_OUT_HW); pl.taps["ori_level1_nchw"] = {raw, 0, -1}; }
        bool fused_done = false;
        for (int j = 0; j < 6; ++j) {
            if (j == 5 && h->sw.fuse_level1 && pose && !heading) {
                const DecoderW& dw = h->ori;
                Level1Params lp{};
                lp.x_ld = xo.C; lp.cx = dw.l1_cx; lp.cxp = dw.l1_cxp; lp.B = B; lp.H = CCVPE_OUT_HW; lp.W = CCVPE_OUT_HW;
                lp.c0 = dw.l1_c0; lp.ng = dw.l1_ng; lp.score = dw.l1_score; lp.wc = dw.l1_wc; lp.ws = dw.l1_ws; lp.bc = dw.l1_bc; lp.wt = dw.l1_wt;
                lp.bt[0] = dw.tail_b[0]; lp.bt[1] = dw.tail_b[1]; lp.cout = 2; lp.normalize = 1;
                const Tensor din = xo, idx = pose_index;
                const bool topk = pl.key.topk;
                const double px = (double)B * (topk ? 8 : 1) * 16 * 16, cin_real = vs.ori[5].din;
                const double flops = px / 4 * 2.0 * cin_real * 64 + px * 2.0 * 144 * 16 + px * 2.0 * 144 * 2, bytes = 4.0 * px / 4 * lp.cx;
                if (topk) pl.add("ori1.topk", {din, idx}, [=](const Ctx& c) {
                    Level1Params q = lp;
                    q.x = c.ptr(din); q.out = nullptr; q.raw = nullptr;
                    launch_level1_topk(q, reinterpret_cast<const int*>(c.ptr(idx)), c.topk_k, c.rows, c.stream);
                }, flops, bytes);
                else pl.add("ori1.pose", {din, idx}, [=](const Ctx& c) {
                    Level1Params q = lp;
                    q.x = c.ptr(din); q.out = nullptr; q.raw = nullptr;
                    launch_level1_pose(q, reinterpret_cast<const int*>(c.ptr(idx)), c.rows, c.stream);
                }, flops, bytes);
                fused_done = true;
                break;
            }
            if (j == 5 && h->sw.fuse_level1 && heading) {
                ori_field = pl.alloc(B, 2, CCVPE_OUT_HW, CCVPE_OUT_HW);
                plan_level1_fused(h->ori, xo, vs.ori[5].din, 2, true, raw, "ori1", ori_field);
                fused_done = true;
                break;
            }
            if (j == 5 && h->sw.fuse_level1) { plan_level1_fused(h->ori, xo, vs.ori[5].din, 2, true, raw, "ori1"); fused_done = true; break; }
            Tensor o = plan_level(h->ori, vs.ori, j, xo, ori_cat[j], "ori" + std::to_string(6 - j));
            if (j < 5) { pl.taps["ori_level" + std::to_string(6 - j)] = {o, 0, o.C}; xo = o; }
            else ori_mid = o;
        }
        if (!fused_done) {
        Tensor m = ori_mid;
        const float* tw = h->ori.tail_w;
        const float tb0 = h->ori.tail_b[0], tb1 = h->ori.tail_b[1];
        const bool dbg = h->debug && !pose;
        std::vector<Tensor> uses = {m};
        if (dbg) uses.push_back(raw);
        const Tensor ori_ws = pose ? pl.alloc(B, 2, CCVPE_OUT_HW, CCVPE_OUT_HW) : Tensor{};
        if (pose) uses.push_back(ori_ws);
        pl.add("ori1.tail", uses, [=](const Ctx& c) {
            TailConvParams p{};
            p.in = c.ptr(m); p.B = B; p.H = CCVPE_OUT_HW; p.W = CCVPE_OUT_HW; p.w = tw; p.bias[0] = tb0; p.bias[1] = tb1; p.cout = 2;
            p.normalize = 1; p.out = pose ? c.ptr(ori_ws) : c.out.ori; p.raw = dbg ? c.ptr(raw) : nullptr;
            launch_tail_conv(p, c.stream);
        }, 2.0 * B * 262144.0 * 288, 4.0 * B * 262144.0 * 18);
        if (pl.key.topk) {
            const Tensor idx = pose_index;
            pl.add("ori1.topk_gather", {ori_ws, idx}, [=](const Ctx& c) {
                launch_topk_gather(c.ptr(ori_ws), reinterpret_cast<const int*>(c.ptr(idx)), B, c.topk_k, CCVPE_OUT_HW * CCVPE_OUT_HW, c.rows, c.stream);
            }, 0, 12.0 * B * 8);
        } else if (pose) {
            const Tensor idx = pose_index;
            pl.add("ori1.gather", {ori_ws, idx}, [=](const Ctx& c) {
                launch_pose_gather(c.ptr(ori_ws), reinterpret_cast<const int*>(c.ptr(idx)), B, CCVPE_OUT_HW * CCVPE_OUT_HW, c.rows, c.stream);
            }, 0, 12.0 * B);
            ori_field = ori_ws;
        }
        } else if (heading) {
            const Tensor idx = pose_index, of = ori_field;
            pl.add("ori1.gather", {of, idx}, [=](const Ctx& c) {
                launch_pose_gather(c.ptr(of), reinterpret_cast<const int*>(c.ptr(idx)), B, CCVPE_OUT_HW * CCVPE_OUT_HW, c.rows, c.stream);
            }, 0, 12.0 * B);
        }
        if (heading) {
            static_assert(sizeof(double) == 2 * sizeof(float) && sizeof(unsigned long long) == 2 * sizeof(unsigned), "allocated in words");
            const Tensor lg = logits_ws, part = pose_part, idx = pose_index, of = ori_field;
            const Tensor hpart = pl.alloc(B, 1, 64, 2 * HEADING_PART);
            const size_t toff = pl.alloc_tickets((size_t)B), boff = pl.alloc_tickets((size_t)B * HEADING_MAX_BINS * 2);
            pl.add("pose.heading", {lg, part, idx, of, hpart}, [=](const Ctx& c) {
                HeadingParams p{};
                p.logits = c.ptr(lg); p.partial = c.ptr(part); p.prior = c.log_prior; p.prior_stride = c.prior_stride;
                p.ori = c.ptr(of); p.index = reinterpret_cast<const int*>(c.ptr(idx)); p.B = B; p.nbins = c.heading_bins; p.r = c.heading_r;
                p.part = reinterpret_cast<double*>(c.ptr(hpart)); p.bins = reinterpret_cast<unsigned long long*>(c.tickets + boff);
                p.tickets = c.tickets + toff; p.heading = c.heading; p.hist = c.hist;
                launch_heading_reduce(p, c.stream);
            }, 0, 4.0 * B * 262144.0 * 3);
        }
    }
    pl.max_tensor_bytes = std::max(pl.max_tensor_bytes, (size_t)B * 3 * std::max(gh * gw, CCVPE_SAT_HW * CCVPE_SAT_HW) * sizeof(float));
    if (pl.max_tensor_bytes >= ((size_t)1 << 31))
        return ccvpe_fail(CCVPE_EINVAL, "micro-batch %d needs a %d x %d x %d x %d tensor of %zu bytes; the kernels address tensors with 32-bit byte offsets (< 2 GiB): "
                    "use a smaller micro_batch (ccvpe_max_micro_batch)", B, pl.max_dims[0], pl.max_dims[1], pl.max_dims[2], pl.max_dims[3], pl.max_tensor_bytes);
    pl.schedule();
    pl.assign();
    return 0;
}

static int build_ground_plan(ccvpe_handle_s* h, Plan& pl, int B, int gh, int gw) {
    pl.debug = false;
    pl.no_reuse = h->sw.no_reuse;
// ... 49 lines not shown
```

ccvpe_amd/csrc/ccvpe_tune.hip:

```cpp
#include "ccvpe_internal.h"


static constexpr size_t TUNING_KEY_MAX = 255;
std::string tuning_key(ccvpe_handle_s* h, const Plan& pl, const Op& op) {
    char head[64], tail[64];
    std::snprintf(head, sizeof(head), "v%d_r%d_c%d_p%d_b%d|", h->cfg.variant, h->rolls[1], h->cfg.circular_padding, h->cfg.reserved[0], pl.key.B);
    std::snprintf(tail, sizeof(tail), "|%dx%dx%d|%d%d%d%d%s%s", op.gemm_m, op.gemm_n, op.gemm_kpad, op.wino_ok ? 1 : 0, op.wino4_ok ? 1 : 0,
                  op.is_pw ? 1 : 0, op.bf16x3_only ? 1 : 0, op.wino4x_ok ? "x" : "", op.proj_ok ? "p" : "");
    std::string key = std::string(head) + op.name + tail;
    if (key.size() > TUNING_KEY_MAX || key.find_first_of(" \t\n") != std::string::npos) return std::string();
    return key;
}

static int tile_by_name(const std::string& name) {
    if (name == "auto") return 0;
    for (int t = 1; t <= conv_num_tiles(); ++t)
        if (name == conv_tile_name(t)) return t;
    return -1;
}

static int apply_tuning(ccvpe_handle_s* h, Plan& pl, std::vector<bool>& known) {
    int missing = 0;
    known.assign(pl.ops.size(), false);
    for (size_t i = 0; i < pl.ops.size(); ++i) {
        Op& op = pl.ops[i];
        if (!op.tile) continue;
        int t = -1, split = 0;
        if (!h->sw.tune_filtered()) {
            const std::string key = tuning_key(h, pl, op);
            auto e = key.empty() ? h->tuning.end() : h->tuning.find(key);
            if (e != h->tuning.end()) { t = tile_by_name(e->second.first); split = e->second.second; }
        }
        if (t < 0) { ++missing; continue; }
        *op.tile = t | (split << 8);
        known[i] = true;
    }
    return missing;
}

static void record_tuning(ccvpe_handle_s* h, const Plan& pl) {
    for (const auto& op : pl.ops) {
        if (!op.tile) continue;
        const int cfg = *op.tile;
        const std::string key = tuning_key(h, pl, op);
        if (!key.empty()) h->tuning[key] = {(cfg & 0xff) ? conv_tile_name(cfg) : "auto", (cfg >> 8) & 0xff};
    }
}

extern "C" {

int ccvpe_import_tuning(ccvpe_handle h, const char* text) {
    if (!h || !text) return ccvpe_fail(CCVPE_EINVAL, "null argument");
    std::map<std::string, std::pair<std::string, int>> parsed;
    const char* p = text;
    while (*p) {
        const char* e = std::strchr(p, '\n');
        const std::string line(p, e ? (size_t)(e - p) : std::strlen(p));
        p = e ? e + 1 : p + line.size();
        char a[TUNING_KEY_MAX + 2], b[66];
        int split = 0;
        if (std::sscanf(line.c_str(), "op %256s %65s %d", a, b, &split) == 3 && std::strlen(a) <= TUNING_KEY_MAX && std::strlen(b) <= 64 && split >= 0 && split <= 255)
            parsed[a] = {b, split};
        else if (!line.empty() && line[0] != '#') return ccvpe_fail(CCVPE_EINVAL, "tuning table: cannot parse '%.200s'", line.c_str());
    }
    for (auto& kv : parsed) h->tuning[kv.first] = kv.second;
    return (int)parsed.size();
}

int ccvpe_export_tuning(ccvpe_handle h, char* buf, size_t capacity, size_t* needed) {
    if (!h) return ccvpe_fail(CCVPE_EINVAL, "null handle");
    std::string out;
    for (const auto& op : h->tuning) out += "op " + op.first + " " + op.second.first + " " + std::to_string(op.second.second) + "\n";
    if (needed) *needed = out.size() + 1;
    if (!buf || capacity < out.size() + 1) return buf ? ccvpe_fail(CCVPE_EINVAL, "tuning table needs %zu bytes", out.size() + 1) : 0;
    std::memcpy(buf, out.c_str(), out.size() + 1);
    return 0;
}

int ccvpe_tuning_generation(ccvpe_handle h) { return h ? h->tuned_plans : ccvpe_fail(CCVPE_EINVAL, "null handle"); }

}

int autotune_plan(ccvpe_handle_s* h, Plan& pl, const std::vector<bool>* known) {
    Ctx c;
    c.arena = h->arena; c.off = &pl.off; c.stream = nullptr;
    c.tickets = pl.tickets;
    pl.set_scratch(c, 0);
    if (pl.tune_cache.id >= 0) c.cache_out = c.ptr(pl.tune_cache);
    HIPCHK(hipDeviceSynchronize());
    hipEvent_t e0, e1;
    HIPCHK(hipEventCreate(&e0));
    HIPCHK(hipEventCreate(&e1));
    launch_fill_random(h->arena, pl.total, 0x9e3779b9u, nullptr);
    const int nt = conv_num_tiles();
    const Switches& sw = h->sw;
    for (size_t oi = 0; oi < pl.ops.size(); ++oi) {
        Op& op = pl.ops[oi];
        if (!op.tile || (known && (*known)[oi])) continue;
        ConvParams q{};
        c.probe = &q;
        op.fn(c);
        c.probe = nullptr;
        int best = 0;
        float best_ms = 1e30f;
        const int nkt = op.gemm_kpad / 32;
        for (int t = 1; t <= nt; ++t) {
            const ConvTile& ct = *conv_tile(t);
            const int splits = conv_tile_splits(ct);
            const bool wino = ct.family == TILE_WINO, pw = ct.family == TILE_PW;
            if (conv_tile_util(q, ct) < 0.45 || !conv_tile_runs(ct, q)) continue;
            if (ct.family == TILE_BF16X3 ? h->cfg.reserved[0] != 1 || sw.tune_no_bf16x3 : op.bf16x3_only) continue;
            if (wino && !(ct.xcfg >= 0 ? op.wino4x_ok : ct.wino_f == 4 ? op.wino4_ok : op.wino_ok)) continue;
            if (pw && (sw.no_pw || !(ct.proj_rt > 0 ? op.proj_ok : op.is_pw))) continue;
            if (sw.tune_prefer_pw && op.is_pw && !op.bf16x3_only && !pw && op.gemm_kpad <= 512) continue;
            if (sw.tune_prefer_proj && op.proj_ok && ct.proj_rt == 0) continue;
            if (sw.tune_prefer_lat && op.proj_ok && op.gemm_m <= 4096 && ct.proj_rt < 100) continue;
            if (ct.proj_rt > 104 && (!sw.tune_lat_rows || op.gemm_m > 1024)) continue;
            const long long blocks = conv_tile_blocks(q, ct);
            const bool no_split = sw.tune_splitk == 0;
            static const int SPLITS[] = {1, 255, 2, 3, 4, 5, 6, 8, 12, 16};
            for (int split : SPLITS) {
                if (split > 1 && no_split) break;
                if (split == 255 && !(splits & SPLIT_TAIL)) continue;
                if (split > 1 && (split & (split - 1)) && !wino) continue;
                const bool lat_split = sw.tune_lat_split && ct.proj_rt >= 100 && op.gemm_m <= 256;
                if (split > 1 && pw && !lat_split) break;
                if (split > 1 && split != 255) {
                    if (blocks >= (wino ? 2048 : 512) || blocks * split > (wino ? 8192 : 2048) || nkt < 4 * split) break;
                    if ((size_t)split * op.gemm_m * op.gemm_n > Plan::SPLITK_FLOATS) break;
                }
                for (int fuse = (split > 1 && pw) ? 1 : 0; fuse < 2; ++fuse) {
                if (fuse && (split <= 1 || split == 255 || !(splits & SPLIT_SELF) || pl.tickets == nullptr || sw.tune_no_fused_split)) break;
                const int cfg = t | ((fuse ? split + SPLIT_FUSED : split) << 8);
                *op.tile = cfg;
                op.fn(c);
                const int ran = conv_tile_last();
                if ((ran & 0xff) != t) break;
                if (split == 255 && (ran >> 8) != 255) break;
                if (split > 1 && pw && ((ran >> 8) & 0xff) <= 1) break;
                float ms = 1e30f;
                for (int trial = 0; trial < 3; ++trial) {
                    HIPCHK(hipEventRecord(e0, nullptr));
                    op.fn(c);
                    op.fn(c);
                    HIPCHK(hipEventRecord(e1, nullptr));
                    HIPCHK(hipEventSynchronize(e1));
                    float t = 0.f;
                    HIPCHK(hipEventElapsedTime(&t, e0, e1));
                    ms = std::min(ms, t);
                }
                if (!sw.tune_verbose.empty() && op.name.find(sw.tune_verbose) != std::string::npos)
                    std::fprintf(stderr, "tune %-28s %-28s split %3d%s: %8.1f us\n", op.name.c_str(), ct.name, split, fuse ? " self-reducing" : "", 500.0 * ms);
                if (ms < best_ms) { best_ms = ms; best = cfg; }
                }
            }
        }
        *op.tile = best;
    }
    (void)hipEventDestroy(e0);
    (void)hipEventDestroy(e1);
    HIPCHK(hipDeviceSynchronize());
    hipError_t e = hipGetLastError();
    if (e != hipSuccess) return ccvpe_fail(CCVPE_EHIP, "autotune launch failed: %s", hipGetErrorString(e));
    return 0;
}

int get_plan(ccvpe_handle_s* h, const PlanKey& key, Plan** out) {
    for (auto& p : h->plans)
        if (p->key == key && (key.mode == 1 || key.mode == 3 || p->debug == h->debug)) { *out = p.get(); return 0; }
    auto pl = std::make_unique<Plan>();
    int rc = build_plan(h, *pl, key);
    if (rc) return rc;
    if (pl->l6_wm && (rc = ensure_level6(h, pl->l6_wm)) != 0) {
        if (h->sw.compose_l6) return rc;
        (void)hipGetLastError();
        h->l6_failed = true;
        pl = std::make_unique<Plan>();
        if ((rc = build_plan(h, *pl, key))) return rc;
    }
    if (pl->total > h->arena_floats) {
        HIPCHK(hipDeviceSynchronize());
        if (h->arena) HIPCHK(hipFree(h->arena));
        h->arena = nullptr;
        for (auto& q : h->plans)
            if (q->exec) { (void)hipGraphExecDestroy(q->exec); q->exec = nullptr; q->runs = 0; }
        void* d = nullptr;
        hipError_t e = hipMalloc(&d, pl->total * sizeof(float));
        if (e != hipSuccess) { h->arena_floats = 0; return ccvpe_fail(CCVPE_ENOMEM, "workspace of %zu bytes: %s", pl->total * sizeof(float), hipGetErrorString(e)); }
        h->arena = (float*)d;
        h->arena_floats = pl->total;
    }
    if (pl->ticket_words) {
        HIPCHK(hipMalloc((void**)&pl->tickets, pl->ticket_words * sizeof(unsigned)));
        HIPCHK(hipMemset(pl->tickets, 0, pl->ticket_words * sizeof(unsigned)));
    }
    std::vector<bool> known;
    if (apply_tuning(h, *pl, known) > 0 && h->sw.autotune) {
        int rc2 = autotune_plan(h, *pl, &known);
        if (rc2) return rc2;
        if (!h->sw.tune_filtered()) {
            record_tuning(h, *pl);
            h->tuned_plans++;
        }
    }
    *out = pl.get();
    h->plans.push_back(std::move(pl));
    return 0;
}
```

ccvpe_amd/csrc/ccvpe_weights.hip:

```cpp
#include "ccvpe_internal.h"

#include <unistd.h>

static void add_bn(std::map<std::string, std::vector<int64_t>>& m, const std::string& p, int c) {
    m[p + ".weight"] = {c}; m[p + ".bias"] = {c}; m[p + ".running_mean"] = {c}; m[p + ".running_var"] = {c};
    m[p + ".num_batches_tracked"] = {};
}
static void add_encoder(std::map<std::string, std::vector<int64_t>>& m, const std::string& p) {
    m[p + "._conv_stem.weight"] = {32, 3, 3, 3};
    add_bn(m, p + "._bn0", 32);
    for (int i = 0; i < 16; ++i) {
        const BlockSpec& b = B0[i];
        std::string q = p + "._blocks." + std::to_string(i);
        int mid = b.cin * b.e;
        if (b.e != 1) { m[q + "._expand_conv.weight"] = {mid, b.cin, 1, 1}; add_bn(m, q + "._bn0", mid); }
        m[q + "._depthwise_conv.weight"] = {mid, 1, b.k, b.k};
        add_bn(m, q + "._bn1", mid);
        int sq = se_squeeze(b.cin);
        m[q + "._se_reduce.weight"] = {sq, mid, 1, 1}; m[q + "._se_reduce.bias"] = {sq};
        m[q + "._se_expand.weight"] = {mid, sq, 1, 1}; m[q + "._se_expand.bias"] = {mid};
        m[q + "._project_conv.weight"] = {b.cout, mid, 1, 1};
        add_bn(m, q + "._bn2", b.cout);
    }
    m[p + "._conv_head.weight"] = {1280, 320, 1, 1};
    add_bn(m, p + "._bn1", 1280);
    m[p + "._fc.weight"] = {1000, 1280};
    m[p + "._fc.bias"] = {1000};
}
void build_expect(ccvpe_handle_s* h) {
    auto& m = h->expect;
    add_encoder(m, "grd_efficientnet");
    add_encoder(m, "sat_efficientnet");
    for (int k = 0; k < 6; ++k) {
        std::string p = "grd_feature_to_descriptor" + std::to_string(k + 1);
        m[p + ".0.weight"] = {h->vs.head_ch[k], 1280, 1, 1}; m[p + ".0.bias"] = {h->vs.head_ch[k]};
        m[p + ".2.weight"] = {1, h->vs.feat_h, 1, 1};        m[p + ".2.bias"] = {1};
    }
    m["sat_feature_to_descriptors.1.weight"] = {h->vs.sat_desc, 5120};
    m["sat_feature_to_descriptors.1.bias"] = {h->vs.sat_desc};
    for (int d = 0; d < 2; ++d) {
        const DecLevel* lv = d ? h->vs.ori : h->vs.loc;
        std::string sfx = d ? "_ori" : "";
        for (int j = 0; j < 6; ++j) {
            std::string n = std::to_string(6 - j);
            m["deconv" + n + sfx + ".weight"] = {lv[j].din, lv[j].dout, 2, 2};
            m["deconv" + n + sfx + ".bias"] = {lv[j].dout};
            m["conv" + n + sfx + ".0.weight"] = {lv[j].mid, lv[j].dout + lv[j].skip, 3, 3};
            m["conv" + n + sfx + ".0.bias"] = {lv[j].mid};
            m["conv" + n + sfx + ".2.weight"] = {lv[j].out, lv[j].mid, 3, 3};
            m["conv" + n + sfx + ".2.bias"] = {lv[j].out};
        }
    }
}

static int upload(ccvpe_handle_s* h, const std::vector<float>& v, float** out) {
    void* d = nullptr;
    size_t bytes = std::max<size_t>(v.size(), 4) * sizeof(float);
    HIPCHK(hipMalloc(&d, bytes));
    h->dev_allocs.push_back(d);
    h->dev_alloc_bytes.push_back(bytes);
    HIPCHK(hipMemcpy(d, v.data(), v.size() * sizeof(float), hipMemcpyHostToDevice));
    *out = (float*)d;
    return 0;
}

extern "C" const char* ccvpe_pack_switches(void) {
    static thread_local std::string s;
    s = read_switches().pack_group();
    return s.c_str();
}

int pack_conv(ccvpe_handle_s* h, PackedConv& pc, int N, int taps, int cin, int cinp, const std::vector<int>& cmap,
                     const std::function<float(int, int, int)>& get, const std::vector<float>& bias, int KH, int KW) {
    const int npad = round_up(N, conv_igemm_npad());
    const int K = taps * cinp;
    const int kpad = round_up(K, 32);
    std::vector<float> w((size_t)npad * kpad, 0.f);
    for (int n = 0; n < N; ++n)
        for (int t = 0; t < taps; ++t)
            for (int c = 0; c < cin; ++c) w[(size_t)n * kpad + conv_igemm_k_index(cinp, taps, t, cmap[c])] = get(n, t, c);
    pc.N = N; pc.Kpad = kpad; pc.nchunks = K / 8; pc.cinp = cinp; pc.KH = KH; pc.KW = KW;
    int rc = upload(h, w, &pc.w);
    if (rc) return rc;
    if (((KH == 1 && KW == 1 && taps == 1 && cin == cinp && conv_proj_wanted(N, cin)) || conv_proj_lat_wanted(taps, KH, KW, cinp)) && !h->sw.no_proj) {
        std::vector<int> inv(cinp, -1);
        for (int c = 0; c < cin; ++c) inv[cmap[c]] = c;
        std::vector<float> up;
        conv_proj_pack(N, cinp, [&](int n, int k) { const int t = k / cinp, c = inv[k - t * cinp]; return c >= 0 ? get(n, t, c) : 0.f; }, up, taps);
        pc.proj_bytes = up.size() * sizeof(float);
        if ((rc = upload(h, up, &pc.proj))) return rc;
    }
    if (KH == 3 && KW == 3 && cin == cinp && cin % 8 == 0 && (size_t)(cin / 8) * 16 * ((N + 15) / 16) * 512 < (1u << 31)) {
        std::vector<float> u;
        conv_wino_pack(N, cin, get, u, &pc.wino_n16);
        pc.wino_bytes = u.size() * sizeof(float);
        if ((rc = upload(h, u, &pc.wino))) return rc;
        if (N >= h->sw.wino4_min_n && (size_t)((cin + 15) / 16) * 4 * 9 * ((N + 15) / 16) * 1024 < (1u << 31) && !h->sw.no_wino4) {
            std::vector<float> u4;
            conv_wino4_pack(N, cin, get, u4);
            pc.wino4_bytes = u4.size() * sizeof(float);
            if ((rc = upload(h, u4, &pc.wino4))) return rc;
        }
        if (N >= 24 && conv_wino4x_config(N) >= 0 && !h->sw.no_wino4x) {
            std::vector<float> ux;
            conv_wino4x_pack(N, cin, get, ux, &pc.wino4x_cfg);
            pc.wino4x_bytes = ux.size() * sizeof(float);
            if ((rc = upload(h, ux, &pc.wino4x))) return rc;
        }
    }
    if (h->cfg.reserved[0] == 1) {
        auto to_bf16 = [](float f) -> unsigned short {
            uint32_t u; std::memcpy(&u, &f, 4);
            if ((u & 0x7fffffffu) > 0x7f800000u) return (unsigned short)((u >> 16) | 0x40);
            return (unsigned short)((u + 0x7fffu + ((u >> 16) & 1u)) >> 16);
        };
        std::vector<unsigned short> hi(w.size()), lo(w.size());
        for (size_t i = 0; i < w.size(); ++i) {
            hi[i] = to_bf16(w[i]);
            uint32_t hu = (uint32_t)hi[i] << 16; float hf; std::memcpy(&hf, &hu, 4);
            lo[i] = to_bf16(w[i] - hf);
        }
        for (int plane = 0; plane < 2; ++plane) {
            void* d = nullptr;
            HIPCHK(hipMalloc(&d, hi.size() * sizeof(unsigned short)));
            h->dev_allocs.push_back(d);
            h->dev_alloc_bytes.push_back(hi.size() * sizeof(unsigned short));
            HIPCHK(hipMemcpy(d, plane ? lo.data() : hi.data(), hi.size() * sizeof(unsigned short), hipMemcpyHostToDevice));
            (plane ? pc.w_lo : pc.w_hi) = (unsigned short*)d;
        }
    }
    return upload(h, bias, &pc.bias);
}
std::vector<int> identity_map(int n) { std::vector<int> m(n); for (int i = 0; i < n; ++i) m[i] = i; return m; }

struct BnFold { std::vector<float> scale, shift; };
static BnFold fold_bn(ccvpe_handle_s* h, const std::string& p) {
    const auto& g = h->host[p + ".weight"]; const auto& b = h->host[p + ".bias"];
    const auto& mu = h->host[p + ".running_mean"]; const auto& var = h->host[p + ".running_var"];
    BnFold f; f.scale.resize(g.size()); f.shift.resize(g.size());
    for (size_t i = 0; i < g.size(); ++i) {
        float s = g[i] / std::sqrt(var[i] + BN_EPS);
        f.scale[i] = s; f.shift[i] = b[i] - mu[i] * s;
    }
    return f;
}

static int pack_pointwise_bn(ccvpe_handle_s* h, PackedConv& pc, const std::string& wkey, const std::string& bnkey, int cout, int cin) {
    const auto& w = h->host[wkey];
    BnFold f = fold_bn(h, bnkey);
    return pack_conv(h, pc, cout, 1, cin, cin, identity_map(cin),
                     [&](int n, int, int c) { return w[(size_t)n * cin + c] * f.scale[n]; }, f.shift, 1, 1);
}

static int build_encoder(ccvpe_handle_s* h, EncoderW& e, const std::string& p) {
    int rc;
    {
        const auto& w = h->host[p + "._conv_stem.weight"];
        BnFold f = fold_bn(h, p + "._bn0");
        std::vector<float> pk(27 * 32);
        for (int o = 0; o < 32; ++o)
            for (int k = 0; k < 27; ++k) pk[k * 32 + o] = w[o * 27 + k] * f.scale[o];
        if ((rc = upload(h, pk, &e.stem_w))) return rc;
        if ((rc = upload(h, f.shift, &e.stem_b))) return rc;
    }
    for (int i = 0; i < 16; ++i) {
        const BlockSpec& b = B0[i];
        BlockW& bw = e.blk[i];
        std::string q = p + "._blocks." + std::to_string(i);
        const int mid = b.cin * b.e;
        if (b.e != 1 && (rc = pack_pointwise_bn(h, bw.expand, q + "._expand_conv.weight", q + "._bn0", mid, b.cin))) return rc;
        if (b.e != 1 && (mbconv_front_supported(b.k, b.s, b.cin, mid) || b.cin % 8 == 0)) {
            const auto& w = h->host[q + "._expand_conv.weight"];
            BnFold f = fold_bn(h, q + "._bn0");
            bw.exp_cinp = round_up(b.cin, 16);
            std::vector<float> lin((size_t)mid * bw.exp_cinp, 0.f);
            for (int n = 0; n < mid; ++n)
                for (int c = 0; c < b.cin; ++c) lin[(size_t)n * bw.exp_cinp + c] = w[(size_t)n * b.cin + c] * f.scale[n];
            if ((rc = upload(h, lin, &bw.exp_lin))) return rc;
        }
        {
            const auto& w = h->host[q + "._depthwise_conv.weight"];
            BnFold f = fold_bn(h, q + "._bn1");
            const int kk = b.k * b.k;
            std::vector<float> pk((size_t)kk * mid);
            for (int c = 0; c < mid; ++c)
                for (int t = 0; t < kk; ++t) pk[(size_t)t * mid + c] = w[(size_t)c * kk + t] * f.scale[c];
            if ((rc = upload(h, pk, &bw.dw_w))) return rc;
            if ((rc = upload(h, f.shift, &bw.dw_b))) return rc;
        }
        bw.sq = se_squeeze(b.cin);
        if ((rc = upload(h, h->host[q + "._se_reduce.weight"], &bw.se_w1))) return rc;
        if ((rc = upload(h, h->host[q + "._se_reduce.bias"], &bw.se_b1))) return rc;
        {
            const auto& w2 = h->host[q + "._se_expand.weight"];
            std::vector<float> t((size_t)mid * bw.sq);
            for (int c = 0; c < mid; ++c)
                for (int j = 0; j < bw.sq; ++j) t[(size_t)j * mid + c] = w2[(size_t)c * bw.sq + j];
            if ((rc = upload(h, t, &bw.se_w2))) return rc;
        }
        if ((rc = upload(h, h->host[q + "._se_expand.bias"], &bw.se_b2))) return rc;
        if ((rc = pack_pointwise_bn(h, bw.project, q + "._project_conv.weight", q + "._bn2", b.cout, mid))) return rc;
    }
    return pack_pointwise_bn(h, e.head, p + "._conv_head.weight", p + "._bn1", 1280, 320);
}


int compose_level1(ccvpe_handle_s* h, DecoderW& d, const std::vector<float>& w, const std::vector<float>& b, const std::vector<float>& wa,
                   const std::vector<float>& ba, int cin, int nscore) {
    int rc;
    const int cout = 16;
    const int spad = score_pad(nscore);
    const int cd = cin - nscore;
    d.l1_cx = spad + cd;
    d.l1_cxp = round_up(d.l1_cx, 16);
    d.l1_c0 = spad; d.l1_ng = (cd + 3) / 4; d.l1_score = nscore;
    std::vector<double> wc((size_t)16 * cin * 16, 0.0);
    for (int py = 0; py < 2; ++py)
        for (int px = 0; px < 2; ++px)
            for (int ky = 0; ky < 3; ++ky)
                for (int kx = 0; kx < 3; ++kx) {
                    const int ty = py + ky + 1, tx = px + kx + 1, a = (ty >> 1) - py, bb = (tx >> 1) - px;
                    const int qd = (ty & 1) * 2 + (tx & 1);
                    double* dst = &wc[(size_t)(((py * 2 + px) * 2 + a) * 2 + bb) * cin * 16];
                    for (int c = 0; c < cin; ++c)
                        for (int o = 0; o < 16; ++o) {
                            double acc = 0.0;
                            for (int m = 0; m < cout; ++m)
                                acc += (double)wa[((size_t)o * 16 + m) * 9 + ky * 3 + kx] * (double)w[((size_t)c * cout + m) * 4 + qd];
                            dst[(size_t)c * 16 + o] += acc;
                        }
                }
    std::vector<float> pk((size_t)4 * d.l1_ng * 64 * 4, 0.f), sc(4 * 64, 0.f);
    for (int par = 0; par < 4; ++par)
        for (int l = 0; l < 64; ++l) {
            const double* src = &wc[(size_t)(par * 4 + (l >> 4)) * cin * 16];
            const int o = l & 15;
            for (int k = 0; k < 4 * d.l1_ng; ++k)
                if (k < cd) pk[((size_t)(par * d.l1_ng + k / 4) * 64 + l) * 4 + k % 4] = (float)src[(size_t)(nscore + k) * 16 + o];
            if (nscore) sc[par * 64 + l] = (float)src[o];
        }
    if ((rc = upload(h, pk, &d.l1_wc))) return rc;
    if (nscore && (rc = upload(h, sc, &d.l1_ws))) return rc;
    std::vector<float> bc(9 * 16);
    for (int rcase = 0; rcase < 3; ++rcase)
        for (int ccase = 0; ccase < 3; ++ccase)
            for (int o = 0; o < 16; ++o) {
                double acc = ba[o];
                for (int ky = 0; ky < 3; ++ky)
                    for (int kx = 0; kx < 3; ++kx) {
                        if ((rcase == 1 && ky == 0) || (rcase == 2 && ky == 2) || (ccase == 1 && kx == 0) || (ccase == 2 && kx == 2)) continue;
                        for (int m = 0; m < cout; ++m) acc += (double)wa[((size_t)o * 16 + m) * 9 + ky * 3 + kx] * (double)b[m];
                    }
                bc[(rcase * 3 + ccase) * 16 + o] = (float)acc;
            }
    if ((rc = upload(h, bc, &d.l1_bc))) return rc;
    return 0;
}

int pack_level1_tail(ccvpe_handle_s* h, DecoderW& d, const std::vector<float>& w2, const std::vector<float>& b2, int cout) {
    std::vector<float> pk1(9 * 16 * cout);
    for (int o = 0; o < cout; ++o)
        for (int c = 0; c < 16; ++c)
            for (int t = 0; t < 9; ++t) pk1[(t * cout + o) * 16 + c] = w2[((size_t)o * 16 + c) * 9 + t];
    if (int rc = upload(h, pk1, &d.l1_wt)) return rc;
    for (int o = 0; o < cout; ++o) d.tail_b[o] = b2[o];
    return 0;
}

static int build_decoder(ccvpe_handle_s* h, DecoderW& d, const DecLevel* lv, const std::string& sfx, int nscore_l6, bool every_level_scored) {
    int rc;
    for (int j = 0; j < 6; ++j) {
        std::string n = std::to_string(6 - j);
        {
            const auto& w = h->host["deconv" + n + sfx + ".weight"];
            const auto& b = h->host["deconv" + n + sfx + ".bias"];
            const int cin = lv[j].din, cout = lv[j].dout, cw = deconv_width(lv[j], h->sw.pad_concat);
            int nscore = 0;
            if (every_level_scored) nscore = 1;
            else if (j == 0) nscore = nscore_l6;
            const int spad = score_pad(nscore);
            const int cinp = spad + (cin - nscore);
            std::vector<int> cmap(cin);
            for (int c = 0; c < cin; ++c) cmap[c] = c < nscore ? c : c - nscore + spad;
            std::vector<float> bias(4 * cw, 0.f);
            for (int qd = 0; qd < 4; ++qd) for (int o = 0; o < cout; ++o) bias[qd * cw + o] = b[o];
            if ((rc = pack_conv(h, d.deconv[j], 4 * cw, 1, cin, cinp, cmap,
                                [&](int nn, int, int c) { int qd = nn / cw, o = nn % cw; return o < cout ? w[((size_t)c * cout + o) * 4 + qd] : 0.f; },
                                bias, 1, 1))) return rc;
        }
        if (j == 5) {
            if ((rc = compose_level1(h, d, h->host["deconv" + n + sfx + ".weight"], h->host["deconv" + n + sfx + ".bias"], h->host["conv" + n + sfx + ".0.weight"],
                                     h->host["conv" + n + sfx + ".0.bias"], lv[j].din, every_level_scored ? 1 : 0))) return rc;
        }
        {
            const auto& w = h->host["conv" + n + sfx + ".0.weight"];
            const int dout = lv[j].dout, cw = deconv_width(lv[j], h->sw.pad_concat);
            const int cin = dout + lv[j].skip, cinw = cw + lv[j].skip, cout = lv[j].mid;
            if ((rc = pack_conv(h, d.conva[j], cout, 9, cinw, cinw, identity_map(cinw),
                                [&](int nn, int t, int c) {
                                    if (c >= dout && c < cw) return 0.f;
                                    const int cr = c < dout ? c : c - (cw - dout);
                                    return w[((size_t)nn * cin + cr) * 9 + t];
                                },
                                h->host["conv" + n + sfx + ".0.bias"], 3, 3))) return rc;
        }
        const auto& w2 = h->host["conv" + n + sfx + ".2.weight"];
        const auto& b2 = h->host["conv" + n + sfx + ".2.bias"];
        if (j < 5) {
            const int cin = lv[j].mid, cout = lv[j].out;
            if ((rc = pack_conv(h, d.convb[j], cout, 9, cin, cin, identity_map(cin),
                                [&](int nn, int t, int c) { return w2[((size_t)nn * cin + c) * 9 + t]; }, b2, 3, 3))) return rc;
        } else {
            const int cout = lv[j].out;
            std::vector<float> pk(9 * 16 * cout);
            for (int o = 0; o < cout; ++o)
                for (int c = 0; c < 16; ++c)
                    for (int t = 0; t < 9; ++t) pk[(t * 16 + c) * cout + o] = w2[((size_t)o * 16 + c) * 9 + t];
            if ((rc = upload(h, pk, &d.tail_w))) return rc;
            if ((rc = pack_level1_tail(h, d, w2, b2, cout))) return rc;
        }
    }
    return 0;
}

void release_level6(ccvpe_handle_s* h) {
    for (void* p : h->l6_allocs) (void)hipFree(p);
    h->l6_allocs.clear();
    h->l6[0] = Level6W{}; h->l6[1] = Level6W{};
    h->l6_wm = 0;
}

int level6_shape(const ccvpe_handle_s* h, const DecoderW& d, const DecLevel& l, int& K, int& Kc, int& N, int& Npad) {
    const PackedConv& dc = d.deconv[0];
    const PackedConv& ac = d.conva[0];
    const int cw = deconv_width(l, h->sw.pad_concat);
    if (!dc.w || !ac.w || ac.cinp != cw + l.skip || dc.N != 4 * cw || l.dout % 8 || dc.cinp % 4 || ac.N % 4 || l.skip % 8) return -1;
    K = dc.cinp; Kc = round_up(K, 32); N = ac.N; Npad = round_up(N, 128);
    return 0;
}

struct Level6AllocScope {
    ccvpe_handle_s* h;
    std::vector<void*> allocs;
    std::vector<size_t> bytes;
    explicit Level6AllocScope(ccvpe_handle_s* h_) : h(h_) { allocs.swap(h->dev_allocs); bytes.swap(h->dev_alloc_bytes); }
    ~Level6AllocScope() {
        h->l6_allocs.insert(h->l6_allocs.end(), h->dev_allocs.begin(), h->dev_allocs.end());
        h->dev_allocs.swap(allocs); h->dev_alloc_bytes.swap(bytes);
    }
    Level6AllocScope(const Level6AllocScope&) = delete;
    Level6AllocScope& operator=(const Level6AllocScope&) = delete;
};

static int derive_level6(ccvpe_handle_s* h, Level6W& o, const DecoderW& d, const DecLevel& l, int wm) {
    const PackedConv& dc = d.deconv[0];
    const PackedConv& ac = d.conva[0];
    if (level6_shape(h, d, l, o.K, o.Kc, o.N, o.Npad)) return ccvpe_fail(CCVPE_ESTATE, "level 6 cannot be composed from these packed weights");
    const int cw = deconv_width(l, h->sw.pad_concat), cinw = cw + l.skip, N = ac.N;
    const size_t arows = (size_t)round_up(N, conv_igemm_npad());
    std::vector<float> aw(arows * ac.Kpad), ba(N), bd(4 * cw);
    HIPCHK(hipMemcpy(aw.data(), ac.w, aw.size() * sizeof(float), hipMemcpyDeviceToHost));
    HIPCHK(hipMemcpy(ba.data(), ac.bias, ba.size() * sizeof(float), hipMemcpyDeviceToHost));
    HIPCHK(hipMemcpy(bd.data(), dc.bias, bd.size() * sizeof(float), hipMemcpyDeviceToHost));
    const auto wa = [&](int n, int t, int c) { return aw[(size_t)n * ac.Kpad + conv_igemm_k_index(cinw, 9, t, c)]; };
    std::vector<double> tapsum((size_t)9 * N, 0.0);
    for (int n = 0; n < N; ++n)
        for (int t = 0; t < 9; ++t) {
            double acc = 0.0;
            for (int m = 0; m < l.dout; ++m) acc += (double)wa(n, t, m) * (double)bd[m];
            tapsum[(size_t)t * N + n] = acc;
        }
    std::vector<float> bc((size_t)9 * N);
    for (int rcase = 0; rcase < 3; ++rcase)
        for (int ccase = 0; ccase < 3; ++ccase)
            for (int n = 0; n < N; ++n) {
                double acc = ba[n];
                for (int ky = 0; ky < 3; ++ky)
                    for (int kx = 0; kx < 3; ++kx) {
                        if ((rcase == 1 && ky == 0) || (rcase == 2 && ky == 2) || (ccase == 1 && kx == 0) || (ccase == 2 && kx == 2)) continue;
                        acc += tapsum[(size_t)(ky * 3 + kx) * N + n];
                    }
                bc[(size_t)(rcase * 3 + ccase) * N + n] = (float)acc;
            }
    {
        Level6AllocScope scope(h);
        if (int rc = upload(h, bc, &o.bc)) return rc;
        if (int rc = pack_conv(h, o.skip, N, 9, l.skip, l.skip, identity_map(l.skip), [&](int n, int t, int c) { return wa(n, t, cw + c); },
                               std::vector<float>(N, 0.f), 3, 3)) return rc;
    }
    const int P = level6_positions(wm);
    const size_t wc_bytes = (size_t)4 * P * o.Npad * o.Kc * sizeof(float), w2_bytes = (size_t)16 * N * o.Kc * sizeof(double);
    void *wc = nullptr, *w2 = nullptr;
    HIPCHK(hipMalloc(&wc, wc_bytes));
    h->l6_allocs.push_back(wc);
    o.wc = (float*)wc;
    HIPCHK(hipMemset(wc, 0, wc_bytes));
    HIPCHK(hipMalloc(&w2, w2_bytes));
    Level6ComposeParams cp{};
    cp.wm = wm; cp.dw = dc.w; cp.cw = cw; cp.dout = l.dout; cp.dkpad = dc.Kpad; cp.aw = ac.w; cp.cinw = cinw; cp.akpad = ac.Kpad;
    cp.K = o.K; cp.Kc = o.Kc; cp.N = N; cp.Npad = o.Npad; cp.w2 = (double*)w2; cp.wc = o.wc;
    launch_level6_compose(cp, nullptr);
    const hipError_t e = hipDeviceSynchronize();
    (void)hipFree(w2);
    if (e != hipSuccess) return ccvpe_fail(CCVPE_EHIP, "composing level 6 failed: %s", hipGetErrorString(e));
    return 0;
}

int ensure_level6(ccvpe_handle_s* h, int wm) {
    if (h->l6_wm == wm) return 0;
    if (!h->finalized) return ccvpe_fail(CCVPE_ESTATE, "ccvpe_finalize_weights has not been called");
    release_level6(h);
    int rc = derive_level6(h, h->l6[0], h->loc, h->vs.loc[0], wm);
    if (!rc) rc = derive_level6(h, h->l6[1], h->ori, h->vs.ori[0], wm);
    if (rc) { release_level6(h); return rc; }
    h->l6_wm = wm;
    return 0;
}

struct PackedHeader {
    char magic[8];
    int32_t variant, precision, circular, fuse_level1;
    char pack_group[128];
    uint64_t n_allocs, sz_encoder, sz_decoder, sz_conv;
    uint64_t n_relocs;
};
static void packed_state_io(ccvpe_handle_s* h, const std::function<void(void*, size_t)>& io) {
    io(&h->grd_enc, sizeof(EncoderW)); io(&h->sat_enc, sizeof(EncoderW));
    io(&h->grd_heads, sizeof(PackedConv)); io(&h->sat_desc, sizeof(PackedConv));
    io(h->grd_wh, sizeof(h->grd_wh)); io(h->grd_b2, sizeof(h->grd_b2));
    io(&h->loc, sizeof(DecoderW)); io(&h->ori, sizeof(DecoderW));
}

extern "C" {


int ccvpe_skip_weight(ccvpe_handle h, const char* key) {
    if (!h || !key) return ccvpe_fail(CCVPE_EINVAL, "null argument");
    if (!h->expect.count(key)) return ccvpe_fail(CCVPE_EKEY, "unexpected state_dict key '%s'", key);
    h->skipped.insert(key);
    return 0;
}

int ccvpe_set_weight(ccvpe_handle h, const char* key, const float* data, const int64_t* shape, int32_t ndim) {
    if (!h || !key || !data) return ccvpe_fail(CCVPE_EINVAL, "null argument");
    auto it = h->expect.find(key);
    if (it == h->expect.end()) return ccvpe_fail(CCVPE_EKEY, "unexpected state_dict key '%s'", key);
    const auto& es = it->second;
    bool ok = (int)es.size() == ndim;
    size_t n = 1;
    for (int i = 0; ok && i < ndim; ++i) { ok = es[i] == shape[i]; n *= (size_t)shape[i]; }
    if (!ok) return ccvpe_fail(CCVPE_EINVAL, "shape mismatch for '%s'", key);
    HIPCHK(hipSetDevice(h->cfg.device));
    std::vector<float> v(n);
    HIPCHK(hipMemcpy(v.data(), data, n * sizeof(float), hipMemcpyDefault));
    h->host[key] = std::move(v);
    h->finalized = false;
    return 0;
}

int ccvpe_finalize_weights(ccvpe_handle h) {
    if (!h) return ccvpe_fail(CCVPE_EINVAL, "null handle");
    HIPCHK(hipSetDevice(h->cfg.device));
    for (auto& kv : h->expect) {
        const std::string& k = kv.first;
        const bool optional = k.find("num_batches_tracked") != std::string::npos || k.find("._fc.") != std::string::npos;
        if (!h->host.count(k) && !(optional || h->skipped.count(k)))
            return ccvpe_fail(CCVPE_EKEY, "missing state_dict key '%s'", k.c_str());
        if (!h->host.count(k) && !optional) return ccvpe_fail(CCVPE_EKEY, "key '%s' was skipped but is required", k.c_str());
    }
    release_level6(h);
    h->l6_failed = false;
    for (void* p : h->dev_allocs) (void)hipFree(p);
    h->dev_allocs.clear();
    h->dev_alloc_bytes.clear();
    h->plans.clear();
    h->last_plan = nullptr;
    int rc;
    if ((rc = build_encoder(h, h->grd_enc, "grd_efficientnet"))) return rc;
    if ((rc = build_encoder(h, h->sat_enc, "sat_efficientnet"))) return rc;
    {
        int ntot = 0;
        for (int k = 0; k < 6; ++k) ntot += h->vs.head_ch[k];
        std::vector<float> bias(ntot);
        std::vector<const std::vector<float>*> ws(6);
        std::vector<int> lvl(ntot), loc(ntot);
        int o = 0;
        for (int k = 0; k < 6; ++k) {
            std::string p = "grd_feature_to_descriptor" + std::to_string(k + 1);
            ws[k] = &h->host[p + ".0.weight"];
            const auto& b = h->host[p + ".0.bias"];
            for (int c = 0; c < h->vs.head_ch[k]; ++c, ++o) { bias[o] = b[c]; lvl[o] = k; loc[o] = c; }
            if ((rc = upload(h, h->host[p + ".2.weight"], &h->grd_wh[k]))) return rc;
            h->grd_b2[k] = h->host[p + ".2.bias"][0];
        }
        if ((rc = pack_conv(h, h->grd_heads, ntot, 1, 1280, 1280, identity_map(1280),
                            [&](int n, int, int c) { return (*ws[lvl[n]])[(size_t)loc[n] * 1280 + c]; }, bias, 1, 1))) return rc;
    }
    {
        const auto& w = h->host["sat_feature_to_descriptors.1.weight"];
        const int D = h->vs.sat_desc;
        if ((rc = pack_conv(h, h->sat_desc, D, 4, 1280, 1280, identity_map(1280),
                            [&](int n, int t, int c) { return w[(size_t)n * 5120 + c * 4 + t]; },
                            h->host["sat_feature_to_descriptors.1.bias"], 2, 2))) return rc;
    }
    if ((rc = build_decoder(h, h->loc, h->vs.loc, "", 1, true))) return rc;
    if ((rc = build_decoder(h, h->ori, h->vs.ori, "_ori", h->vs.n_rolls, false))) return rc;
    h->host.clear();
    if (!level1_supported(h->loc.l1_cxp) || !level1_supported(h->ori.l1_cxp)) h->sw.fuse_level1 = false;
    h->finalized = true;
    return 0;
}


int ccvpe_save_packed(ccvpe_handle h, const char* path) {
    if (!h || !path) return ccvpe_fail(CCVPE_EINVAL, "null argument");
    if (!h->finalized) return ccvpe_fail(CCVPE_ESTATE, "ccvpe_finalize_weights has not been called");
    static_assert(std::is_trivially_copyable<EncoderW>::value && std::is_trivially_copyable<DecoderW>::value && std::is_trivially_copyable<PackedConv>::value,
                  "descriptor structs are written as plain bytes");
    HIPCHK(hipSetDevice(h->cfg.device));
    char suffix[64];
    std::snprintf(suffix, sizeof(suffix), ".tmp.%ld.%llx", (long)getpid(), (unsigned long long)(uintptr_t)h ^ (unsigned long long)std::rand());
    const std::string tmp = std::string(path) + suffix;
    FILE* f = std::fopen(tmp.c_str(), "wb");
    if (!f) return ccvpe_fail(CCVPE_EINVAL, "cannot open %s for writing", tmp.c_str());
    std::map<uint64_t, uint64_t> index_of;
    for (size_t i = 0; i < h->dev_allocs.size(); ++i) index_of[(uint64_t)(uintptr_t)h->dev_allocs[i]] = i;
    std::vector<uint64_t> relocs;
    uint64_t word0 = 0;
    packed_state_io(h, [&](void* p, size_t n) {
        const uint64_t* w = reinterpret_cast<const uint64_t*>(p);
        for (size_t i = 0; i + 8 <= n; i += 8, ++w) {
            auto it = *w ? index_of.find(*w) : index_of.end();
            if (it != index_of.end()) { relocs.push_back(word0 + i / 8); relocs.push_back(it->second); }
        }
        word0 += n / 8;
    });
    PackedHeader hd{};
    std::memcpy(hd.magic, "CCVPEPK5", 8);
    std::snprintf(hd.pack_group, sizeof(hd.pack_group), "%s", h->sw.pack_group().c_str());
    hd.variant = h->cfg.variant; hd.precision = h->cfg.reserved[0]; hd.circular = h->cfg.circular_padding; hd.fuse_level1 = h->sw.fuse_level1 ? 1 : 0;
    hd.n_allocs = h->dev_allocs.size(); hd.sz_encoder = sizeof(EncoderW); hd.sz_decoder = sizeof(DecoderW); hd.sz_conv = sizeof(PackedConv);
    hd.n_relocs = relocs.size() / 2;
    bool ok = std::fwrite(&hd, sizeof(hd), 1, f) == 1;
    packed_state_io(h, [&](void* p, size_t n) { ok = ok && std::fwrite(p, 1, n, f) == n; });
    ok = ok && (relocs.empty() || std::fwrite(relocs.data(), 8, relocs.size(), f) == relocs.size());
    std::vector<char> buf;
    for (size_t i = 0; ok && i < h->dev_allocs.size(); ++i) {
        const uint64_t bytes = h->dev_alloc_bytes[i];
        buf.resize(bytes);
        if (hipMemcpy(buf.data(), h->dev_allocs[i], bytes, hipMemcpyDeviceToHost) != hipSuccess) { ok = false; break; }
        ok = std::fwrite(&bytes, 8, 1, f) == 1 && std::fwrite(buf.data(), 1, bytes, f) == bytes;
    }
    ok = (std::fclose(f) == 0) && ok;
    if (!ok || std::rename(tmp.c_str(), path) != 0) { std::remove(tmp.c_str()); return ccvpe_fail(CCVPE_EINVAL, "writing %s failed", path); }
    return 0;
}

int ccvpe_load_packed(ccvpe_handle h, const char* path) {
    if (!h || !path) return ccvpe_fail(CCVPE_EINVAL, "null argument");
    HIPCHK(hipSetDevice(h->cfg.device));
    FILE* f = std::fopen(path, "rb");
    if (!f) return ccvpe_fail(CCVPE_EINVAL, "cannot open %s", path);
    PackedHeader hd{};
    auto bad = [&](const char* why) { std::fclose(f); return ccvpe_fail(CCVPE_EINVAL, "%s: %s", path, why); };
    if (std::fread(&hd, sizeof(hd), 1, f) != 1 || std::memcmp(hd.magic, "CCVPEPK5", 8) != 0) return bad("not a packed-weight file of this library version");
    if (hd.variant != h->cfg.variant || hd.precision != h->cfg.reserved[0] || hd.circular != h->cfg.circular_padding) return bad("packed for a different variant / precision / padding mode");
    hd.pack_group[sizeof(hd.pack_group) - 1] = 0;
    if (h->sw.pack_group() != hd.pack_group) return bad("packed under other packer switches (CCVPE_NO_PROJ, CCVPE_WINO4_MIN_N, CCVPE_NO_WINO4, CCVPE_NO_WINO4X, CCVPE_PAD_CONCAT)");
    if (hd.sz_encoder != sizeof(EncoderW) || hd.sz_decoder != sizeof(DecoderW) || hd.sz_conv != sizeof(PackedConv)) return bad("descriptor layout mismatch");
    if (hd.n_allocs == 0 || hd.n_allocs > 100000 || hd.n_relocs > 100000) return bad("implausible buffer / relocation counts");
    release_level6(h);
    h->l6_failed = false;
    for (void* p : h->dev_allocs) (void)hipFree(p);
    h->dev_allocs.clear(); h->dev_alloc_bytes.clear(); h->plans.clear(); h->last_plan = nullptr; h->finalized = false;
    bool ok = true;
    uint64_t nwords = 0;
    packed_state_io(h, [&](void* p, size_t n) { ok = ok && std::fread(p, 1, n, f) == n; nwords += n / 8; });
    std::vector<uint64_t> relocs(hd.n_relocs * 2);
    ok = ok && (relocs.empty() || std::fread(relocs.data(), 8, relocs.size(), f) == relocs.size());
    for (size_t i = 0; ok && i < relocs.size(); i += 2) ok = relocs[i] < nwords && relocs[i + 1] < hd.n_allocs;
    std::vector<char> buf;
    for (uint64_t i = 0; ok && i < hd.n_allocs; ++i) {
        uint64_t bytes = 0;
        if (std::fread(&bytes, 8, 1, f) != 1 || bytes == 0 || bytes > ((uint64_t)1 << 33)) { ok = false; break; }
        buf.resize(bytes);
        if (std::fread(buf.data(), 1, bytes, f) != bytes) { ok = false; break; }
        void* d = nullptr;
        if (hipMalloc(&d, bytes) != hipSuccess) { ok = false; break; }
        h->dev_allocs.push_back(d); h->dev_alloc_bytes.push_back(bytes);
        if (hipMemcpy(d, buf.data(), bytes, hipMemcpyHostToDevice) != hipSuccess) { ok = false; break; }
    }
    ok = ok && std::fgetc(f) == EOF;
    std::fclose(f);
    if (!ok) {
        for (void* p : h->dev_allocs) (void)hipFree(p);
        h->dev_allocs.clear(); h->dev_alloc_bytes.clear();
        packed_state_io(h, [&](void* p, size_t n) { std::memset(p, 0, n); });
        ccvpe_err() = std::string(path) + ": truncated, inconsistent or unreadable packed-weight file";
        return CCVPE_EINVAL;
    }
    std::map<uint64_t, uint64_t> patch;
    for (size_t i = 0; i < relocs.size(); i += 2) patch[relocs[i]] = (uint64_t)(uintptr_t)h->dev_allocs[relocs[i + 1]];
    uint64_t word0 = 0;
    packed_state_io(h, [&](void* p, size_t n) {
        uint64_t* w = reinterpret_cast<uint64_t*>(p);
        for (auto it = patch.lower_bound(word0); it != patch.end() && it->first < word0 + n / 8; ++it) w[it->first - word0] = it->second;
        word0 += n / 8;
    });
    const int want_desc = h->vs.sat_desc;
    if (h->sat_desc.N != want_desc || h->grd_enc.head.N != 1280 || h->sat_enc.head.N != 1280 || h->loc.conva[0].N != h->vs.loc[0].mid || h->ori.conva[0].N != h->vs.ori[0].mid) {
        for (void* p : h->dev_allocs) (void)hipFree(p);
        h->dev_allocs.clear(); h->dev_alloc_bytes.clear();
        packed_state_io(h, [&](void* p, size_t n) { std::memset(p, 0, n); });
        return ccvpe_fail(CCVPE_EINVAL, "%s: layer sizes do not match this variant", path);
    }
    const auto l1_ok = [&](const DecoderW& d) {
        return d.l1_wc && d.l1_bc && (d.l1_score == 0 || d.l1_ws) && d.l1_ng > 0 && d.l1_c0 + 4 * d.l1_ng <= d.l1_cxp && level1_supported(d.l1_cxp);
    };
    if (hd.fuse_level1 != 0 && !(l1_ok(h->loc) && l1_ok(h->ori))) {
        for (void* p : h->dev_allocs) (void)hipFree(p);
        h->dev_allocs.clear(); h->dev_alloc_bytes.clear();
        packed_state_io(h, [&](void* p, size_t n) { std::memset(p, 0, n); });
        return ccvpe_fail(CCVPE_EINVAL, "%s: no composed level-1 weights", path);
    }
    h->host.clear();
    h->sw.fuse_level1 = hd.fuse_level1 != 0 && h->sw.fuse_level1;
    h->finalized = true;
    return 0;
}

}
```

ccvpe_amd/csrc/kernels.h:

```cpp
#pragma once
#include <functional>
#include <vector>
#include <hip/hip_runtime.h>
#include <stdint.h>
#include "ticket.h"

namespace ccvpe {

extern thread_local unsigned long long g_launches;
#define CCVPE_LAUNCH(...) do { ++::ccvpe::g_launches; hipLaunchKernelGGL(__VA_ARGS__); } while (0)

struct LdsAttr { size_t set[16] = {0}; };
inline void ensure_dynamic_lds(LdsAttr& state, const void* kernel, size_t bytes) {
    int dev = 0;
    if (hipGetDevice(&dev) != hipSuccess || dev < 0 || dev >= 16) dev = 0;
    if (bytes > state.set[dev] && hipFuncSetAttribute(kernel, hipFuncAttributeMaxDynamicSharedMemorySize, (int)bytes) == hipSuccess) state.set[dev] = bytes;
}

enum Act { ACT_NONE = 0, ACT_RELU = 1, ACT_SWISH = 2 };

struct Dst {
    float* ptr;
    int ld;
    int coff;
    int split;
    long long plane;
};

enum { MODE_CONV = 0, MODE_DECONV = 1 };

struct ConvParams {
    const float* in;
    int in_ld;
    int B, H, W, Cin;
    int OH, OW;
    int KH, KW, stride, pad_t, pad_l;
    const float* wpk;
    const unsigned short* w_hi;
    const unsigned short* w_lo;
    int Kpad;
    int Npad;
    int nchunks;
    const float* bias;
    int N;
    int act;
    const float* gate;
    const float* resid;
    int resid_ld;
    Dst dst[3];
    int ndst;
    int mode;
    int deconv_cout;
    int M;
    unsigned in_bytes;
    int in_split;
    unsigned in_plane_bytes;
    unsigned w_plane_bytes;
    unsigned gate_bytes;
    int taps4;
    int kfull_chunks;
    int kfull_c0;
    int knc;
    int div_4t_mul;
    int div_nc_mul;
    int div_kw_mul;
    int vec_epi;
    int splitk;
    float* partial;
    size_t partial_floats;
    unsigned* tickets;
    int split_fused;
    unsigned fdw_mul, fdw_shift, fdh_mul, fdh_shift;
    const float* wino_w;
    int wino_n16;
    int wino_nb, wino_n16_off;
    unsigned wino_bytes;
    const float* wino4_w;
    unsigned wino4_bytes;
    const float* wino4x_w;
    unsigned wino4x_bytes;
    int wino4x_cfg;
    const float* proj_w;
    unsigned proj_bytes;
    const float* se_rows;
    int se_nrows, se_sq;
    float se_inv_hw;
    const float* se_b1;
    const float* se_w2;
    const float* se_b2;
};

enum { TILE_AUTO = 0 };
enum TileFamily { TILE_IGEMM, TILE_BF16X3, TILE_WINO, TILE_PW };
using ConvLaunch = void (*)(const ConvParams&, hipStream_t);
struct ConvTile {
    int bm, bn;
    const char* name;
    ConvLaunch launch;
    TileFamily family;
    double intrinsic = 0.0;
    int wino_f = 0;
    int xcfg = -1;
    int proj_rt = 0;
};
constexpr ConvTile igemm_tile(int bm, int bn, const char* name, ConvLaunch l, double intrinsic) { return {bm, bn, name, l, TILE_IGEMM, intrinsic}; }
constexpr ConvTile bf16x3_tile(int bm, int bn, const char* name, ConvLaunch l) { return {bm, bn, name, l, TILE_BF16X3}; }
constexpr ConvTile wino_tile(int bm, int bn, const char* name, ConvLaunch l, int f, int xcfg = -1) { return {bm, bn, name, l, TILE_WINO, 0.0, f, xcfg}; }
constexpr ConvTile pw_tile(int bm, int bn, const char* name, ConvLaunch l, int proj_rt = 0) { return {bm, bn, name, l, TILE_PW, 0.0, 0, -1, proj_rt}; }
static constexpr int CONV_TICKETS = 8192;
static constexpr int SPLIT_FUSED = 64;
int conv_num_tiles();
const ConvTile* conv_tile(int id);
const char* conv_tile_name(int id);
int conv_proj_lat_tile();
bool conv_tile_runs(const ConvTile& t, const ConvParams& p);
enum { SPLIT_SELF = 1, SPLIT_TAIL = 2 };
int conv_tile_splits(const ConvTile& t);
double conv_tile_util(const ConvParams& p, const ConvTile& t);
long long conv_tile_blocks(const ConvParams& p, const ConvTile& t);
int conv_tile_last();
void conv_tile_note_unfused();
int conv_igemm_prepare(ConvParams& p);
int conv_igemm_k_index(int cin, int taps, int tap, int c);
int launch_conv_igemm(const ConvParams& p, int tile, hipStream_t s);
int conv_igemm_npad();
void launch_splitk_reduce(const ConvParams& p, hipStream_t s);
const ConvTile* conv_bf16x3_tiles(int* n);
const ConvTile* conv_wino_tiles(int* n);
bool conv_wino_supported(const ConvParams& p);
bool conv_wino4_supported(const ConvParams& p);
void launch_wino4_64(const ConvParams& p, hipStream_t s);
void launch_wino4_128(const ConvParams& p, hipStream_t s);
bool conv_wino4_tail_applied();
void launch_wino4x(const ConvParams& p, hipStream_t s);
bool conv_wino4x_supported(const ConvParams& p);
int conv_wino4x_config(int N);
size_t conv_wino4x_pack(int N, int cin, const std::function<float(int, int, int)>& get, std::vector<float>& out, int* cfg_out);
size_t conv_wino4_pack(int N, int cin, const std::function<float(int, int, int)>& get, std::vector<float>& out);
size_t conv_wino_pack(int N, int cin, const std::function<float(int, int, int)>& get, std::vector<float>& out, int* n16_out);
const ConvTile* conv_pw_tiles(int* n);
bool conv_pw_supported(const ConvParams& p);
bool conv_pw_fits(int bn, int kpad);
bool conv_proj_supported(const ConvParams& p, int rt);
void launch_proj(const ConvParams& p, int rt, hipStream_t s);
bool conv_proj_wanted(int N, int cin);
size_t conv_proj_pack(int N, int cin, const std::function<float(int, int)>& get, std::vector<float>& out, int taps = 1);
bool conv_proj_lat_wanted(int taps, int KH, int KW, int cinp);

struct StemParams {
    const float* in;
    int B, H, W, OH, OW;
    int pad_t, pad_l;
    int circular;
    const float* w;
    const float* bias;
    float* out;
};
void launch_stem(const StemParams& p, hipStream_t s);

struct StemDwParams {
    StemParams st;
    const float* wd;
    const float* bd;
    float* out;
    float* pool_partial;
    SeTicket se;
};
int stem_dw_tiles(int OH, int OW);
void launch_stem_dw(const StemDwParams& p, hipStream_t s);

struct DwParams {
    const float* in;
    int B, H, W, C, OH, OW;
    int k, stride, pad_t, pad_l, circular;
    const float* w;
    const float* bias;
    float* out;
    float* pool_partial;
    int S;
    SeTicket se;
};
void launch_depthwise(const DwParams& p, hipStream_t s);
int depthwise_strip_lanes(int B, int OH, int OW, int C, int k, int stride);

struct MbFrontParams {
    const float* x;
    int B, H, W, Cin, cinp;
    int mid;
    const float* we;
    const float* be;
    const float* wd;
    const float* bd;
    int k, s, pad_t, pad_l, circular, OH, OW;
    float* out;
    float* pool;
    SeTicket se;
    int spread;
};
void launch_mbconv_front(const MbFrontParams& p, hipStream_t s);
int mbconv_front_tiles(int k, int s, int OH, int OW);
int mbconv_front_ticket_rows(const MbFrontParams& p);
int mbconv_image_ticket_rows(const MbFrontParams& p);
int mbconv_front_ticket_split(const MbFrontParams& p);
bool mbconv_front_supported(int k, int s, int cin, int mid);
bool mbconv_front_profitable(int k);
bool mbconv_image_supported(const MbFrontParams& p);
int mbconv_image_strips(const MbFrontParams& p);
void launch_mbconv_image(const MbFrontParams& p, hipStream_t s);

struct SeParams {
    const float* pool_partial;
    int B, S, C, SQ;
    float inv_hw;
    const float* w1;
    const float* b1;
    const float* w2;
    const float* b2;
    float* gate;
    float* pooled;
    int SC;
    float* sq;
};
void launch_se(const SeParams& p, hipStream_t s);

struct GrdDescParams {
    const float* y;
    int B, Hf, Wf, Ntot;
    int nlev;
    int c[6], off[6];
    const float* wh[6];
    float b2[6];
    float* desc;
    int loff[6];
    int Ltot;
};
void launch_grd_desc(const GrdDescParams& p, hipStream_t s);

struct MatchParams {
    const float* x;
    int x_ld;
    int B, HW, C;
    const float* g;
    int g_ld, L;
    int R;
    int shift[32];
    uint32_t inmax;
    float* ms;
    float* cat_max;  int cat_max_ld;
    float* cat_all;  int cat_all_ld;  int rpad;
    int P;
    float* gg_scratch;
    int prep_done;
    int no_wide;
};
void launch_match(const MatchParams& p, hipStream_t s);
void launch_match_prep(const MatchParams& p, hipStream_t s);
void launch_match_prep_all(const MatchParams* ps, int n, hipStream_t s);
int match_pixels_per_block(int HW, int C);
size_t match_scratch_floats(int C);

struct TailConvParams {
    const float* in;
    int B, H, W;
    const float* w;
    float bias[2];
    int cout;
    int normalize;
    float* out;
    float* raw;
};
void launch_tail_conv(const TailConvParams& p, hipStream_t s);

struct Level1Params {
    const float* x;
    int x_ld, cx, cxp;
    int B, H, W;
    int c0, ng, score;
    const float* wc;
    const float* ws;
    const float* bc;
    const float* wt;
    float bt[2];
    int cout, normalize;
    float* out;
    float* raw;
    int tile;
    int max_wg;
};
void launch_level1(const Level1Params& p, hipStream_t s);
int level1_tile(const Level1Params& p);
bool level1_supported(int cxp);
void launch_level1_pose(const Level1Params& p, const int* index, float* rows, hipStream_t s);
void launch_level1_topk(const Level1Params& p, const int* index, int k, float* rows, hipStream_t s);

struct Level6Params {
    int wm;
    int B;
    int K, Kc;
    int N, Npad;
    int R, bm;
    const float* x;
    float* v;
    const float* wc;
    float* mp;
    const float* skip;
    const float* bc;
    float* out;
};
int level6_positions(int wm);
int level6_rows(int B, int wm, int* bm_out);
bool level6_supported(const Level6Params& p);
void launch_level6_transform(const Level6Params& p, hipStream_t s);
void launch_level6_gemm(const Level6Params& p, hipStream_t s);
void launch_level6_combine(const Level6Params& p, hipStream_t s);
struct Level6ComposeParams {
    int wm;
    const float* dw;
    int cw, dout, dkpad;
    const float* aw;
    int cinw, akpad;
    int K, Kc, N, Npad;
    double* w2;
    float* wc;
};
void launch_level6_compose(const Level6ComposeParams& p, hipStream_t s);

__device__ __forceinline__ float pose_angle_deg(float cs, float sn) {
    float ang = acosf(fminf(fmaxf(cs, -1.f), 1.f)) * 57.29577951308232f;
    if (sn < 0.f) { ang = fmodf(-ang, 360.f); if (ang < 0.f) ang += 360.f; }
    return ang;
}

struct SoftmaxParams {
    const float* logits;
    int B, n;
    float* partial;
    int chunks;
    float* out;
    const float* prior;
    long long prior_stride;
};
void launch_softmax(const SoftmaxParams& p, hipStream_t s);
void launch_softmax_partial(const SoftmaxParams& p, hipStream_t s);

struct PoseArgmaxParams {
    const float* logits;
    const float* partial;
    int B, n, chunks;
    float* pairs;
    unsigned* tickets;
    int* index;
    float* rows;
    float* stats;
    const float* prior;
    long long prior_stride;
    float* posterior;
    float* summary;
    double* summ_part;
    int summary_r;
};
void launch_pose_argmax(const PoseArgmaxParams& p, hipStream_t s);

static constexpr int SUMMARY_COLS = 16, SUMMARY_PART = 8, SUMMARY_MAX_R = 32;
struct BeliefSummaryParams {
    const float* belief;
    int B, r;
    float* pairs;
    double* summ_part;
    unsigned* tickets;
    float* summary;
};
void launch_belief_summary(const BeliefSummaryParams& p, hipStream_t s);
void launch_pose_gather(const float* ori, const int* index, int B, int n, float* rows, hipStream_t s);

static constexpr int HEADING_COLS = 12, HEADING_PART = 4, HEADING_MIN_BINS = 4, HEADING_MAX_BINS = 360, HEADING_MAX_R = 32;
struct HeadingParams {
    const float* logits;
    const float* partial;
    const float* prior;
    long long prior_stride;
    const float* ori;
    const int* index;
    int B, nbins, r;
    double* part;
    unsigned long long* bins;
    unsigned* tickets;
    float* heading;
    float* hist;
};
void launch_heading_reduce(const HeadingParams& p, hipStream_t s);

static constexpr int TOPK_MAX_K = 64, TOPK_MAX_R = 32;
struct TopkParams {
    const float* heat;
    const float* logits;
    const float* partial;
    int B, k, r;
    unsigned long long* keys;
    unsigned* tickets;
    int* index;
    float* rows;
    const float* prior;
    long long prior_stride;
};
void launch_topk_peaks(const TopkParams& p, hipStream_t s);
void launch_topk_gather(const float* ori, const int* index, int B, int K, int n, float* rows, hipStream_t s);
size_t topk_scratch_bytes(int B);

struct PreprocParams {
    const unsigned char* in;
    int B, H, W, crop_w;
    const int* shift;
    float mean[3], stdv[3];
    float* out;
};
void launch_preprocess(const PreprocParams& p, hipStream_t s);
struct ResizeParams {
    const unsigned char* in;
    int B, IH, IW, OH, OW, crop_w;
    unsigned char* tmp;
    const int* shift;
    float mean[3], stdv[3];
    float* out;
    const int* origin;
    int map_h, map_w;
};
int launch_resize(const ResizeParams& p, hipStream_t s);

static constexpr int WARP_MAX_STAGES = 4;
static constexpr int WARP_MAX_BILINEAR = 2;
struct WarpParams {
    const unsigned char* in;
    const double* mat;
    int B, H, W, n;
    unsigned bilinear;
    int top, left, out_h, out_w;
    float mean[3], stdv[3];
    float* out;
};
int launch_warp(const WarpParams& p, hipStream_t s);

void launch_scatter_channels(const float* src, int C, long long P, Dst d0, Dst d1, int ndst, hipStream_t s);
static constexpr int GATHER_MAX_SAMPLES = 16;
struct GatherParams {
    const float* src;
    Dst d0, d1;
    int ndst;
    int C, hw;
    int b0;
    int tile[GATHER_MAX_SAMPLES];
};
void launch_gather_channels(const float* src, int C, int hw, const int* tile, int B, Dst d0, Dst d1, int ndst, hipStream_t s);

static constexpr int REGION_MAX_QUERIES = 64;
struct RegionParams {
    const float* stats;
    const float* pair_rows;
    float* rows;
    int* best_pair;
    float* tile_prob;
    int g0;
    int off[REGION_MAX_QUERIES + 1];
};
void launch_region_reduce(const float* stats, const float* pair_rows, const int* offsets, int G, float* rows, int* best_pair, float* tile_prob,
                          hipStream_t s);

static constexpr int TRACK_MAX_R = 32;
struct TrackPredictParams {
    const float* belief;
    const float* shift;
    const float* taps;
    int taps_stride;
    int radius;
    const float* floor;
    float* log_prior;
    int B;
};
void launch_track_predict(const TrackPredictParams& p, hipStream_t s);

struct TrackPredictAffineParams {
    const float* belief;
    const double* matrix;
    const float* taps;
    int taps_stride;
    int radius;
    const float* floor;
    float* log_prior;
    int B;
};
void launch_track_predict_affine(const TrackPredictAffineParams& p, hipStream_t s);

struct PoseOut { int32_t index; float prob, cos_v, sin_v, angle_deg; };
static constexpr int PP_MAX_BATCH = 4096;
size_t postprocess_scratch_bytes(int B);
void launch_postprocess(const float* heat, const float* ori, int B, int n, PoseOut* out, float* rows, void* scratch, hipStream_t s);

struct MetricsOut { double pixel_distance, meter_distance, prob_at_gt, angle_pred_deg, angle_gt_deg, orientation_error_deg, longitudinal_m, lateral_m; };
void launch_metrics(const PoseOut* pose, const float* heat, int B, int W, int n, const int* gt_index, const float* gt_cos_sin,
                    const double* meter_per_pixel, const double* heading_deg, MetricsOut* out, hipStream_t s);

struct MultiCopy { const float* src[12]; float* dst[12]; unsigned long long n[12]; int count; };
void launch_multi_copy(const MultiCopy& mc, hipStream_t s);
void launch_fill_random(float* p, size_t n, uint32_t seed, hipStream_t s);
void launch_nhwc_to_nchw(const float* in, int in_ld, int coff, int C, int B, int HW, float* out, hipStream_t s);

}
```

ccvpe_amd/csrc/kernels_level6.hip:

```cpp
#include "igemm_common.h"

namespace ccvpe {

template <int M> struct Wino;
template <> struct Wino<4> {
    static constexpr int NP = 5;
    static __host__ __device__ constexpr float bt(int u, int i) {
        constexpr float t[5][5] = {{2, -1, -2, 1, 0}, {0, -2, -1, 1, 0}, {0, 2, -3, 1, 0}, {0, -1, 0, 1, 0}, {0, 2, -1, -2, 1}};
        return t[u][i];
    }
    static __host__ __device__ constexpr float at(int i, int u) {
        constexpr float t[4][5] = {{1, 1, 1, 1, 0}, {0, 1, -1, 2, 0}, {0, 1, 1, 4, 0}, {0, 1, -1, 8, 1}};
        return t[i][u];
    }
    static __host__ __device__ constexpr double g(int u, int a) {
        constexpr double t[5][2] = {{0.5, 0.0}, {-0.5, -0.5}, {-1.0 / 6.0, 1.0 / 6.0}, {1.0 / 6.0, 1.0 / 3.0}, {0.0, 1.0}};
        return t[u][a];
    }
};
template <> struct Wino<2> {
    static constexpr int NP = 3;
    static __host__ __device__ constexpr float bt(int u, int i) {
        constexpr float t[3][3] = {{-1, 1, 0}, {0, 1, 0}, {0, -1, 1}};
        return t[u][i];
    }
    static __host__ __device__ constexpr float at(int i, int u) {
        constexpr float t[2][3] = {{1, 1, 0}, {0, 1, 1}};
        return t[i][u];
    }
    static __host__ __device__ constexpr double g(int u, int a) {
        constexpr double t[3][2] = {{-1.0, 0.0}, {1.0, 1.0}, {0.0, 1.0}};
        return t[u][a];
    }
};

int level6_positions(int wm) { return (wm + 1) * (wm + 1); }
int level6_rows(int B, int wm, int* bm_out) {
    const int t = 8 / wm, rows = B * t * t;
    const int bm = rows > 64 ? 128 : rows > 32 ? 64 : 32;
    if (bm_out) *bm_out = bm;
    return (rows + bm - 1) / bm * bm;
}

template <int M>
__global__ __launch_bounds__(128) void level6_transform_kernel(const Level6Params p) {
    using W = Wino<M>;
    constexpr int NP = W::NP, T = 8 / M;
    const int k = (blockIdx.x * 128 + threadIdx.x) * 4;
    if (k >= p.Kc) return;
    const int row = blockIdx.y, cls = blockIdx.z;
    const int b = row / (T * T), t = row - b * (T * T);
    const int y0 = M * (t / T) - 1 + (cls >> 1), x0 = M * (t % T) - 1 + (cls & 1);
    const bool live = b < p.B && k < p.K;
    f32x4 d[NP][NP];
#pragma unroll
    for (int i = 0; i < NP; ++i)
#pragma unroll
        for (int j = 0; j < NP; ++j) {
            const int y = y0 + i, x = x0 + j;
            d[i][j] = f32x4{0.f, 0.f, 0.f, 0.f};
            if (live && (unsigned)y < 8u && (unsigned)x < 8u) d[i][j] = *reinterpret_cast<const f32x4*>(p.x + ((size_t)(b * 8 + y) * 8 + x) * p.K + k);
        }
    f32x4 c[NP][NP];
#pragma unroll
    for (int u = 0; u < NP; ++u)
#pragma unroll
        for (int j = 0; j < NP; ++j) {
            f32x4 s = {0.f, 0.f, 0.f, 0.f};
#pragma unroll
            for (int i = 0; i < NP; ++i)
                if (W::bt(u, i) != 0.f) s += W::bt(u, i) * d[i][j];
            c[u][j] = s;
        }
    float* dst = p.v + ((size_t)cls * NP * NP * p.R + row) * p.Kc + k;
    const size_t gstride = (size_t)p.R * p.Kc;
#pragma unroll
    for (int u = 0; u < NP; ++u)
#pragma unroll
        for (int v = 0; v < NP; ++v) {
            f32x4 s = {0.f, 0.f, 0.f, 0.f};
#pragma unroll
            for (int j = 0; j < NP; ++j)
                if (W::bt(v, j) != 0.f) s += W::bt(v, j) * c[u][j];
            *reinterpret_cast<f32x4*>(dst + (size_t)(u * NP + v) * gstride) = s;
            __builtin_amdgcn_sched_barrier(0);
            asm volatile("s_nop 1");
            __builtin_amdgcn_sched_barrier(0);
        }
}

template <int BM, int WGM, int WGN>
__global__ __launch_bounds__(256) void level6_gemm_kernel(const Level6Params p) {
    constexpr int BN = 128, MT = 32;
    constexpr int WM = BM / WGM, WN = BN / WGN, TM = WM / MT, TN = WN / MT;
    static_assert(WGM * WGN == 4 && TM >= 1 && TN >= 1 && TM * MT * WGM == BM && TN * MT * WGN == BN, "whole MFMA tiles, 4 waves");
    constexpr int AR = BM / 32, BR = BN / 32;
    constexpr int KSTEP = 8, NKK = BK / KSTEP;

    extern __shared__ __attribute__((aligned(16))) float smem[];
    float* As = smem;
    float* Bs = smem + 2 * BM * LDK;

    const int tid = threadIdx.x, lane = tid & 63, wave = tid >> 6;
    const int wm = wave / WGN, wn = wave % WGN;
    const int nbn = p.Npad / BN, mblocks = p.R / BM;
    const int lid = xcd_remap(blockIdx.x, gridDim.x);
    const int nb = lid % nbn, rest = lid / nbn;
    const int mb = rest % mblocks, g = rest / mblocks;
    const int m0 = mb * BM, n0 = nb * BN;
    const int kq = tid & 7, r0 = tid >> 3;

    const float* arow = p.v + ((size_t)g * p.R + m0 + r0) * p.Kc + kq * 4;
    const float* brow = p.wc + ((size_t)g * p.Npad + n0 + r0) * p.Kc + kq * 4;
    const size_t rstep = (size_t)32 * p.Kc;

    f32x4 ra[AR], rb[BR];
    f32x16 acc[TM][TN];
#pragma unroll
    for (int i = 0; i < TM; ++i)
#pragma unroll
        for (int j = 0; j < TN; ++j)
#pragma unroll
            for (int r = 0; r < 16; ++r) acc[i][j][r] = 0.f;

    const int nkt = p.Kc / BK;
#pragma unroll
    for (int j = 0; j < AR; ++j) ra[j] = *reinterpret_cast<const f32x4*>(arow + j * rstep);
#pragma unroll
    for (int j = 0; j < BR; ++j) rb[j] = *reinterpret_cast<const f32x4*>(brow + j * rstep);
#pragma unroll
    for (int j = 0; j < AR; ++j) *reinterpret_cast<f32x4*>(As + (r0 + 32 * j) * LDK + kq * 4) = ra[j];
#pragma unroll
    for (int j = 0; j < BR; ++j) *reinterpret_cast<f32x4*>(Bs + (r0 + 32 * j) * LDK + kq * 4) = rb[j];
    __syncthreads();

    const int a_row = wm * WM + (lane & 31);
    const int b_row = wn * WN + (lane & 31);
    const int k_lane = (lane >> 5) * 4;

    for (int kt = 0; kt < nkt; ++kt) {
        const int stage = kt & 1;
        const int ktn = min(kt + 1, nkt - 1);
#pragma unroll
        for (int j = 0; j < AR; ++j) ra[j] = *reinterpret_cast<const f32x4*>(arow + j * rstep + ktn * BK);
#pragma unroll
        for (int j = 0; j < BR; ++j) rb[j] = *reinterpret_cast<const f32x4*>(brow + j * rstep + ktn * BK);
        __builtin_amdgcn_sched_barrier(0);
        const float* as = As + stage * BM * LDK + a_row * LDK + k_lane;
        const float* bs = Bs + stage * BN * LDK + b_row * LDK + k_lane;
        f32x4 a[2][TM], b[2][TN];
#pragma unroll
        for (int i = 0; i < TM; ++i) a[0][i] = *reinterpret_cast<const f32x4*>(as + i * MT * LDK);
#pragma unroll
        for (int j = 0; j < TN; ++j) b[0][j] = *reinterpret_cast<const f32x4*>(bs + j * MT * LDK);
#pragma unroll
        for (int kk = 0; kk < NKK; ++kk) {
            const int cur = kk & 1, nxt = cur ^ 1;
            if (kk + 1 < NKK) {
#pragma unroll
                for (int i = 0; i < TM; ++i) a[nxt][i] = *reinterpret_cast<const f32x4*>(as + i * MT * LDK + (kk + 1) * KSTEP);
#pragma unroll
                for (int j = 0; j < TN; ++j) b[nxt][j] = *reinterpret_cast<const f32x4*>(bs + j * MT * LDK + (kk + 1) * KSTEP);
            }
#pragma unroll
            for (int i = 0; i < TM; ++i)
#pragma unroll
                for (int j = 0; j < TN; ++j) {
                    acc[i][j] = __builtin_amdgcn_mfma_f32_32x32x2f32(b[cur][j].x, a[cur][i].x, acc[i][j], 0, 0, 0);
                    acc[i][j] = __builtin_amdgcn_mfma_f32_32x32x2f32(b[cur][j].y, a[cur][i].y, acc[i][j], 0, 0, 0);
                    acc[i][j] = __builtin_amdgcn_mfma_f32_32x32x2f32(b[cur][j].z, a[cur][i].z, acc[i][j], 0, 0, 0);
                    acc[i][j] = __builtin_amdgcn_mfma_f32_32x32x2f32(b[cur][j].w, a[cur][i].w, acc[i][j], 0, 0, 0);
                }
        }
        __builtin_amdgcn_sched_barrier(0);
#pragma unroll
        for (int j = 0; j < AR; ++j) *reinterpret_cast<f32x4*>(As + (stage ^ 1) * BM * LDK + (r0 + 32 * j) * LDK + kq * 4) = ra[j];
#pragma unroll
        for (int j = 0; j < BR; ++j) *reinterpret_cast<f32x4*>(Bs + (stage ^ 1) * BN * LDK + (r0 + 32 * j) * LDK + kq * 4) = rb[j];
        __syncthreads();
    }

    constexpr int LDC = BN + 4;
    float* Cs = smem;
#pragma unroll
    for (int j = 0; j < TN; ++j)
#pragma unroll
        for (int q = 0; q < 4; ++q) {
            const int nl = wn * WN + j * MT + 8 * q + 4 * (lane >> 5);
#pragma unroll
            for (int i = 0; i < TM; ++i) {
                const int ml = wm * WM + i * MT + (lane & 31);
                f32x4 v;
#pragma unroll
                for (int e = 0; e < 4; ++e) v[e] = acc[i][j][4 * q + e];
                *reinterpret_cast<f32x4*>(Cs + ml * LDC + nl) = v;
            }
        }
    __syncthreads();
    constexpr int C4 = BN / 4;
    for (int it = tid; it < BM * C4; it += 256) {
        const int ml = it / C4, c4 = it - ml * C4;
        const int n = n0 + c4 * 4;
        if (n >= p.N) continue;
        *reinterpret_cast<f32x4*>(p.mp + ((size_t)g * p.R + m0 + ml) * p.N + n) = *reinterpret_cast<const f32x4*>(Cs + ml * LDC + c4 * 4);
    }
}

template <int M>
__global__ __launch_bounds__(64) void level6_combine_kernel(const Level6Params p) {
    using W = Wino<M>;
    constexpr int NP = W::NP, T = 8 / M;
    const int n = (blockIdx.x * 64 + threadIdx.x) * 4;
    if (n >= p.N) return;
    const int row = blockIdx.y, cls = blockIdx.z;
    const int b = row / (T * T), t = row - b * (T * T);
    const int ty = t / T, tx = t - ty * T, py = cls >> 1, px = cls & 1;
    const float* src = p.mp + ((size_t)cls * NP * NP * p.R + row) * p.N + n;
    const size_t gstride = (size_t)p.R * p.N;
    f32x4 m[NP][NP];
#pragma unroll
    for (int u = 0; u < NP; ++u)
#pragma unroll
        for (int v = 0; v < NP; ++v) m[u][v] = *reinterpret_cast<const f32x4*>(src + (size_t)(u * NP + v) * gstride);
    f32x4 c[M][NP];
#pragma unroll
    for (int i = 0; i < M; ++i)
#pragma unroll
        for (int v = 0; v < NP; ++v) {
            f32x4 s = {0.f, 0.f, 0.f, 0.f};
#pragma unroll
            for (int u = 0; u < NP; ++u)
                if (W::at(i, u) != 0.f) s += W::at(i, u) * m[u][v];
            c[i][v] = s;
        }
#pragma unroll
    for (int i = 0; i < M; ++i)
#pragma unroll
        for (int j = 0; j < M; ++j) {
            f32x4 s = {0.f, 0.f, 0.f, 0.f};
#pragma unroll
            for (int v = 0; v < NP; ++v)
                if (W::at(j, v) != 0.f) s += W::at(j, v) * c[i][v];
            const int oy = 2 * (M * ty + i) + py, ox = 2 * (M * tx + j) + px;
            const int rcase = oy == 0 ? 1 : oy == 15 ? 2 : 0, ccase = ox == 0 ? 1 : ox == 15 ? 2 : 0;
            const size_t e = ((size_t)(b * 16 + oy) * 16 + ox) * p.N + n;
            s += *reinterpret_cast<const f32x4*>(p.skip + e);
            s += *reinterpret_cast<const f32x4*>(p.bc + (rcase * 3 + ccase) * p.N + n);
#pragma unroll
            for (int q = 0; q < 4; ++q) s[q] = fmaxf(s[q], 0.f);
            *reinterpret_cast<f32x4*>(p.out + e) = s;
        }
}

bool level6_supported(const Level6Params& p) {
    int bm = 0;
    return (p.wm == 4 || p.wm == 2) && p.B > 0 && p.K > 0 && p.K % 4 == 0 && p.Kc % BK == 0 && p.Kc >= p.K && p.N > 0 && p.N % 4 == 0 &&
           p.Npad % 128 == 0 && p.Npad >= p.N && p.R == level6_rows(p.B, p.wm, &bm) && p.bm == bm;
}

void launch_level6_transform(const Level6Params& p, hipStream_t s) {
    const dim3 grid((p.Kc / 4 + 127) / 128, p.R, 4);
    if (p.wm == 4) CCVPE_LAUNCH(level6_transform_kernel<4>, grid, dim3(128), 0, s, p);
    else CCVPE_LAUNCH(level6_transform_kernel<2>, grid, dim3(128), 0, s, p);
}

template <int BM, int WGM, int WGN>
static void launch_gemm_t(const Level6Params& p, hipStream_t s) {
    constexpr size_t lds = std::max<size_t>(2 * (BM + 128) * LDK, BM * (128 + 4)) * sizeof(float);
    static LdsAttr attr;
    auto kern = level6_gemm_kernel<BM, WGM, WGN>;
    ensure_dynamic_lds(attr, reinterpret_cast<const void*>(kern), lds);
    const int blocks = 4 * level6_positions(p.wm) * (p.R / BM) * (p.Npad / 128);
    CCVPE_LAUNCH(kern, dim3(blocks), dim3(256), lds, s, p);
}
void launch_level6_gemm(const Level6Params& p, hipStream_t s) {
    if (p.bm == 128) launch_gemm_t<128, 2, 2>(p, s);
    else if (p.bm == 64) launch_gemm_t<64, 2, 2>(p, s);
    else launch_gemm_t<32, 1, 4>(p, s);
}

void launch_level6_combine(const Level6Params& p, hipStream_t s) {
    const int t = 8 / p.wm;
    const dim3 grid((p.N / 4 + 63) / 64, p.B * t * t, 4);
    if (p.wm == 4) CCVPE_LAUNCH(level6_combine_kernel<4>, grid, dim3(64), 0, s, p);
    else CCVPE_LAUNCH(level6_combine_kernel<2>, grid, dim3(64), 0, s, p);
}

__device__ __forceinline__ int k_index_dev(int cin, int taps, int tap, int c) {
    const int full = cin / 32, cg = c / 32;
    const int g = cg < full ? cg * 4 * taps + tap * 4 + (c % 32) / 8 : full * 4 * taps + tap * ((cin % 32) / 8) + (c - full * 32) / 8;
    return g * 8 + (c % 8);
}

__global__ __launch_bounds__(256) void level6_compose_kernel(const Level6ComposeParams p) {
    __shared__ double As[8][128];
    __shared__ double Bs[8][128];
    const int tid = threadIdx.x;
    const int slot = blockIdx.z, cls = slot >> 2, a = (slot >> 1) & 1, b = slot & 1, py = cls >> 1, px = cls & 1;
    const int n0 = blockIdx.y * 128, k0 = blockIdx.x * 128;
    const int tk = tid & 15, tn = tid >> 4;
    double acc[8][8];
#pragma unroll
    for (int i = 0; i < 8; ++i)
#pragma unroll
        for (int j = 0; j < 8; ++j) acc[i][j] = 0.0;
    const int an = n0 + (tid >> 1), ah = (tid & 1) * 4;
    const int bm = tid >> 5, bk = k0 + (tid & 31) * 4;
    for (int ky = 0; ky < 3; ++ky) {
        if ((((py + ky + 1) >> 1) - py) != a) continue;
        for (int kx = 0; kx < 3; ++kx) {
            if ((((px + kx + 1) >> 1) - px) != b) continue;
            const int t = ky * 3 + kx, qd = ((py + ky + 1) & 1) * 2 + ((px + kx + 1) & 1);
            for (int m0 = 0; m0 < p.dout; m0 += 8) {
                f32x4 va = {0.f, 0.f, 0.f, 0.f}, vb = {0.f, 0.f, 0.f, 0.f};
                if (an < p.N) va = *reinterpret_cast<const f32x4*>(p.aw + (size_t)an * p.akpad + k_index_dev(p.cinw, 9, t, m0 + ah));
                if (bk < p.K) vb = *reinterpret_cast<const f32x4*>(p.dw + (size_t)(qd * p.cw + m0 + bm) * p.dkpad + bk);
                __syncthreads();
#pragma unroll
                for (int e = 0; e < 4; ++e) { As[ah + e][tid >> 1] = (double)va[e]; Bs[bm][(tid & 31) * 4 + e] = (double)vb[e]; }
                __syncthreads();
#pragma unroll
                for (int mm = 0; mm < 8; ++mm) {
                    double ar[8], br[8];
#pragma unroll
                    for (int i = 0; i < 8; ++i) { ar[i] = As[mm][tn * 8 + i]; br[i] = Bs[mm][tk * 8 + i]; }
#pragma unroll
                    for (int i = 0; i < 8; ++i)
#pragma unroll
                        for (int j = 0; j < 8; ++j) acc[i][j] = fma(ar[i], br[j], acc[i][j]);
                }
            }
        }
    }
#pragma unroll
    for (int i = 0; i < 8; ++i) {
        const int n = n0 + tn * 8 + i;
        if (n >= p.N) continue;
#pragma unroll
        for (int j = 0; j < 8; ++j) {
            const int k = k0 + tk * 8 + j;
            if (k < p.Kc) p.w2[((size_t)slot * p.N + n) * p.Kc + k] = acc[i][j];
        }
    }
}

template <int M>
__global__ __launch_bounds__(256) void level6_filter_kernel(const Level6ComposeParams p) {
    using W = Wino<M>;
    constexpr int NP = W::NP;
    const size_t per = (size_t)p.N * p.Kc;
    const size_t i = (size_t)blockIdx.x * 256 + threadIdx.x;
    if (i >= per) return;
    const int cls = blockIdx.y;
    const int n = (int)(i / p.Kc), k = (int)(i - (size_t)n * p.Kc);
    double w[2][2];
#pragma unroll
    for (int a = 0; a < 2; ++a)
#pragma unroll
        for (int b = 0; b < 2; ++b) w[a][b] = p.w2[(size_t)(cls * 4 + a * 2 + b) * per + i];
#pragma unroll
    for (int u = 0; u < NP; ++u)
#pragma unroll
        for (int v = 0; v < NP; ++v) {
            double s = 0.0;
#pragma unroll
            for (int a = 0; a < 2; ++a)
#pragma unroll
                for (int b = 0; b < 2; ++b) s += W::g(u, a) * W::g(v, b) * w[a][b];
            p.wc[((size_t)(cls * NP * NP + u * NP + v) * p.Npad + n) * p.Kc + k] = (float)s;
        }
}

void launch_level6_compose(const Level6ComposeParams& p, hipStream_t s) {
    CCVPE_LAUNCH(level6_compose_kernel, dim3((p.Kc + 127) / 128, (p.N + 127) / 128, 16), dim3(256), 0, s, p);
    const size_t per = (size_t)p.N * p.Kc;
    const dim3 grid((unsigned)((per + 255) / 256), 4);
    if (p.wm == 4) CCVPE_LAUNCH(level6_filter_kernel<4>, grid, dim3(256), 0, s, p);
    else CCVPE_LAUNCH(level6_filter_kernel<2>, grid, dim3(256), 0, s, p);
}

}
```

Measured before the change: 2725 queries/s.

## Extend composed deconv+conv Winograd path to decoder level 5

Generalises the level-6 composed transposed-conv-plus-conv path, which folds the deconv weights into the following conv, to a 16x16 grid. By default it is applied to level 5 of the location decoder at batch >= 32, skipping that level's separate deconv and concat buffer. It also adds a 64-wide N tile to the composed GEMM so padding is not wasted when N is not a multiple of 128. In exchange it adds extra weight-composition memory and more kernel template variants, and the cached-tap scatter now writes a separate skip copy.

```diff
diff --git a/ccvpe_amd/csrc/ccvpe_api.hip b/ccvpe_amd/csrc/ccvpe_api.hip
--- a/ccvpe_amd/csrc/ccvpe_api.hip
+++ b/ccvpe_amd/csrc/ccvpe_api.hip
@@ -30,6 +30,7 @@
     if (const char* e = getenv("CCVPE_FUSE_L1")) s.fuse_level1 = std::atoi(e) != 0;
     if (const char* e = getenv("CCVPE_L1_TILE")) s.l1_tile = std::atoi(e);
     if (const char* e = getenv("CCVPE_COMPOSE_L6")) s.compose_l6 = std::atoi(e);
+    if (const char* e = getenv("CCVPE_COMPOSE_L5")) s.compose_l5 = std::atoi(e);
     if (const char* e = getenv("CCVPE_WINOGRAD")) s.wino = std::atoi(e) != 0;
     if (const char* e = getenv("CCVPE_GRAPH")) s.graph_mode = std::atoi(e) != 0;
     if (const char* e = getenv("CCVPE_STREAMS")) s.two_streams = std::atoi(e) >= 2;
diff --git a/ccvpe_amd/csrc/ccvpe_internal.h b/ccvpe_amd/csrc/ccvpe_internal.h
--- a/ccvpe_amd/csrc/ccvpe_internal.h
+++ b/ccvpe_amd/csrc/ccvpe_internal.h
@@ -101,6 +101,7 @@
     bool fuse_level1 = true;
     int l1_tile = 1;
     std::optional<int> compose_l6;
+    std::optional<int> compose_l5;
     bool wino = true;
     int graph_mode = 0;
     bool two_streams = true;
@@ -193,10 +194,13 @@
     int K = 0, Kc = 0, N = 0, Npad = 0;
 };
 static constexpr int LEVEL6_AUTO_MIN_BATCH = 8;
+static constexpr bool LEVEL5_AUTO_LOC = true;
+static constexpr bool LEVEL5_AUTO_ORI = false;
+static constexpr int LEVEL5_AUTO_MIN_BATCH = 32;
 struct ccvpe_handle_s;
 struct DecoderW;
-int level6_shape(const ccvpe_handle_s* h, const DecoderW& d, const struct DecLevel& l, int& K, int& Kc, int& N, int& Npad);
-int ensure_level6(ccvpe_handle_s* h, int wm);
+int level6_shape(const ccvpe_handle_s* h, const DecoderW& d, const struct DecLevel& l, int j, int& K, int& Kc, int& N, int& Npad);
+int ensure_level6(ccvpe_handle_s* h, int j, int wm, unsigned mask);
 void release_level6(ccvpe_handle_s* h);
 int compose_level1(ccvpe_handle_s* h, DecoderW& d, const std::vector<float>& w, const std::vector<float>& b, const std::vector<float>& wa,
                    const std::vector<float>& ba, int cin, int nscore);
@@ -333,6 +337,8 @@
     unsigned* tickets = nullptr;
     size_t alloc_tickets(size_t n) { const size_t o = ticket_words; ticket_words += (n + 15) & ~(size_t)15; return o; }
     int l6_wm = 0;
+    int l5_wm = 0;
+    unsigned l5_mask = 0;
     bool tiles_checked = false;
     bool two_streams = false;
     Tensor scratch2;
@@ -495,10 +501,11 @@
     float* grd_wh[6] = {nullptr};
     float grd_b2[6] = {0};
     DecoderW loc, ori;
-    Level6W l6[2];
-    int l6_wm = 0;
-    std::vector<void*> l6_allocs;
-    bool l6_failed = false;
+    Level6W l6[2][2];
+    int l6_wm[2] = {0, 0};
+    unsigned l6_have[2] = {0, 0};
+    std::vector<void*> l6_allocs[2];
+    bool l6_failed[2] = {false, false};
     std::vector<std::unique_ptr<Plan>> plans;
     Plan* last_plan = nullptr;
     float* snap[2] = {nullptr, nullptr};
diff --git a/ccvpe_amd/csrc/ccvpe_plan.hip b/ccvpe_amd/csrc/ccvpe_plan.hip
--- a/ccvpe_amd/csrc/ccvpe_plan.hip
+++ b/ccvpe_amd/csrc/ccvpe_plan.hip
@@ -318,25 +318,44 @@
     const int rpad = score_pad(rfull);
     Tensor loc_in[6], ori_in6;
     Tensor loc_cat[6], ori_cat[6];
+    const int l5_sw = h->sw.compose_l5.value_or(0);
+    const bool l5_forced = l5_sw >= 1 && l5_sw <= 4;
+    unsigned l5_mask = !h->finalized || h->cfg.reserved[0] != 0 || !h->sw.wino ? 0u
+                       : h->sw.compose_l5 ? (!l5_forced ? 0u : l5_sw == 3 ? 1u : l5_sw == 4 ? 2u : 3u)
+                       : (B >= LEVEL5_AUTO_MIN_BATCH && !h->l6_failed[1]) ? (LEVEL5_AUTO_LOC ? 1u : 0u) | (LEVEL5_AUTO_ORI ? 2u : 0u) : 0u;
+    Level6Params l5p[2] = {};
+    for (int d = 0; d < 2; ++d) {
+        if (!(l5_mask >> d & 1)) continue;
+        Level6Params& q = l5p[d];
+        q.wm = 4; q.gs = 16; q.B = B;
+        bool ok = level6_shape(h, d ? h->ori : h->loc, d ? vs.ori[1] : vs.loc[1], 1, q.K, q.Kc, q.N, q.Npad) == 0;
+        q.R = level6_rows(B, q.wm, q.gs, &q.bm);
+        q.bn = (ok && q.N % 128 != 0 && q.bm >= 64 && l5_sw != 2) ? 64 : 128;
+        ok = ok && level6_supported(q) && q.K == (d ? vs.ori[0].out : 8 + vs.match_ch[1]);
+        if (!ok && l5_forced) return ccvpe_fail(CCVPE_ESTATE, "composed level 5: the packed weights do not fit the plan's level-5 inputs");
+        if (!ok) l5_mask &= ~(1u << d);
+    }
+    pl.l5_wm = l5_mask ? 4 : 0;
+    pl.l5_mask = l5_mask;
     for (int j = 0; j < 6; ++j) {
         const int hw_in = 8 << j;
         loc_in[j] = pl.alloc(B, hw_in, hw_in, 8 + vs.match_ch[j]);
-        loc_cat[j] = pl.alloc(B, hw_in * 2, hw_in * 2, deconv_width(vs.loc[j], h->sw.pad_concat) + vs.loc[j].skip);
-        ori_cat[j] = pl.alloc(B, hw_in * 2, hw_in * 2, deconv_width(vs.ori[j], h->sw.pad_concat) + vs.ori[j].skip);
+        if (!(j == 1 && (l5_mask & 1u))) loc_cat[j] = pl.alloc(B, hw_in * 2, hw_in * 2, deconv_width(vs.loc[j], h->sw.pad_concat) + vs.loc[j].skip);
+        if (!(j == 1 && (l5_mask & 2u))) ori_cat[j] = pl.alloc(B, hw_in * 2, hw_in * 2, deconv_width(vs.ori[j], h->sw.pad_concat) + vs.ori[j].skip);
         if (h->cfg.reserved[0] == 1 && j < 5 && h->sw.split_planes) { loc_cat[j].split = true; ori_cat[j].split = true; }
     }
     const bool l6_forced = h->sw.compose_l6 && (*h->sw.compose_l6 == 1 || *h->sw.compose_l6 == 2);
     int l6_wm = !h->finalized || h->cfg.reserved[0] != 0 || !h->sw.wino ? 0
                 : h->sw.compose_l6 ? (*h->sw.compose_l6 == 1 ? 4 : *h->sw.compose_l6 == 2 ? 2 : 0)
-                : (B >= LEVEL6_AUTO_MIN_BATCH && !h->l6_failed) ? 4 : 0;
+                : (B >= LEVEL6_AUTO_MIN_BATCH && !h->l6_failed[0]) ? 4 : 0;
     Level6Params l6p[2] = {};
     if (l6_wm) {
         bool ok = true;
         for (int d = 0; d < 2; ++d) {
             Level6Params& q = l6p[d];
-            q.wm = l6_wm; q.B = B;
-            ok = ok && level6_shape(h, d ? h->ori : h->loc, d ? vs.ori[0] : vs.loc[0], q.K, q.Kc, q.N, q.Npad) == 0;
-            q.R = level6_rows(B, l6_wm, &q.bm);
+            q.wm = l6_wm; q.gs = 8; q.bn = 128; q.B = B;
+            ok = ok && level6_shape(h, d ? h->ori : h->loc, d ? vs.ori[0] : vs.loc[0], 0, q.K, q.Kc, q.N, q.Npad) == 0;
+            q.R = level6_rows(B, l6_wm, 8, &q.bm);
             ok = ok && level6_supported(q) && q.K == (d ? rpad + D : loc_in[0].C);
         }
         if (!ok && l6_forced) return ccvpe_fail(CCVPE_ESTATE, "composed level 6: the packed weights do not fit the plan's level-6 inputs");
@@ -344,6 +363,7 @@
     }
     pl.l6_wm = l6_wm;
     Tensor skip15;
+    Tensor skip10;
     ori_in6 = pl.alloc(B, 8, 8, rpad + D);
     pl.taps["ori_in6"] = {ori_in6, 0, ori_in6.C};
 
@@ -356,13 +376,18 @@
         td[t].t[1] = ori_cat[t]; td[t].coff[1] = deconv_width(vs.ori[t], h->sw.pad_concat);
     }
     if (l6_wm) td[0].n = 0;
+    if (l5_mask == 3u) td[1].n = 0;
+    else if (l5_mask == 1u) { td[1].n = 1; td[1].t[0] = td[1].t[1]; td[1].coff[0] = td[1].coff[1]; }
+    else if (l5_mask == 2u) td[1].n = 1;
     size_t coff[6];
     cache_layout(vs, B, coff);
     if (!cached) {
         plan_encoder(h, pl, h->sat_enc, false, B, CCVPE_SAT_HW, CCVPE_SAT_HW, false, td, senc, "sat");
         skip15 = senc.tap[TAP_BLOCK[0]];
+        skip10 = senc.tap[TAP_BLOCK[1]];
     } else {
         if (l6_wm) skip15 = pl.alloc(B, 16, 16, TAP_C[0]);
+        if (l5_mask) skip10 = pl.alloc(B, 32, 32, TAP_C[1]);
         size_t one[6];
         cache_layout(vs, 1, one);
         for (int t = 0; t < 5; ++t) {
@@ -371,14 +396,25 @@
             const size_t src_off = coff[t + 1], src_off1 = one[t + 1];
             const int C = TAP_C[t], hw = TAP_HW[t];
             const long long P = (long long)B * TAP_HW[t];
-            if (t == 0 && l6_wm) {
-                const Tensor sk = skip15;
+            if ((t == 0 && l6_wm) || (t == 1 && l5_mask == 3u)) {
+                const Tensor sk = t == 0 ? skip15 : skip10;
                 pl.add("sat.cached_tap" + std::to_string(TAP_BLOCK[t]), {sk}, [=](const Ctx& c) {
                     if (c.tile_index)
                         launch_gather_channels(c.cache_in + src_off1 * c.n_tiles, C, hw, c.tile_index, B, c.dst(sk), Dst{nullptr, 0, 0, 0, 0}, 1, c.stream);
                     else
                         launch_scatter_channels(c.cache_in + src_off, C, P, c.dst(sk), Dst{nullptr, 0, 0, 0, 0}, 1, c.stream);
                 }, 0, 4.0 * P * C * 2);
+                continue;
+            }
+            if (t == 1 && l5_mask) {
+                const Tensor sk = skip10, cat = (l5_mask & 1u) ? oc : lc;
+                const int off = (l5_mask & 1u) ? ocoff : lcoff;
+                pl.add("sat.cached_tap" + std::to_string(TAP_BLOCK[t]), {sk, cat}, [=](const Ctx& c) {
+                    if (c.tile_index)
+                        launch_gather_channels(c.cache_in + src_off1 * c.n_tiles, C, hw, c.tile_index, B, c.dst(sk), c.dst(cat, off), 2, c.stream);
+                    else
+                        launch_scatter_channels(c.cache_in + src_off, C, P, c.dst(sk), c.dst(cat, off), 2, c.stream);
+                }, 0, 4.0 * P * C * 3);
                 continue;
             }
             pl.add("sat.cached_tap" + std::to_string(TAP_BLOCK[t]), {lc, oc}, [=](const Ctx& c) {
@@ -431,20 +467,22 @@
         const int hin = 8 << j, hout = hin * 2;
         const DecLevel& l = lv[j];
         Tensor mid = pl.alloc(B, hout, hout, l.mid);
-        if (j == 0 && l6_wm) {
-            const Level6W* w6 = &h->l6[&dw == &h->ori ? 1 : 0];
-            const Level6Params lp = l6p[&dw == &h->ori ? 1 : 0];
-            const int G = 4 * level6_positions(l6_wm);
+        const int dec = &dw == &h->ori ? 1 : 0;
+        if ((j == 0 && l6_wm) || (j == 1 && (l5_mask >> dec & 1))) {
+            const Level6W* w6 = &h->l6[j][dec];
+            const Level6Params lp = j == 0 ? l6p[dec] : l5p[dec];
+            const int G = 4 * level6_positions(lp.wm);
             Tensor V = pl.alloc(G, 1, lp.R, lp.Kc), Mp = pl.alloc(G, 1, lp.R, lp.N), sk = pl.alloc(B, hout, hout, l.mid);
-            const Tensor s15 = skip15;
-            pl.add(tag + ".l6_transform", {din, V}, [=](const Ctx& c) {
+            const Tensor s15 = j == 0 ? skip15 : skip10;
+            const std::string pre = j == 0 ? ".l6_" : ".l5_";
+            pl.add(tag + pre + "transform", {din, V}, [=](const Ctx& c) {
                 Level6Params q = lp; q.x = c.ptr(din); q.v = c.ptr(V);
                 launch_level6_transform(q, c.stream);
             }, 0.0, 4.0 * ((double)din.numel() + (double)V.numel()));
-            pl.add(tag + ".l6_gemm", {V, Mp}, [=](const Ctx& c) {
+            pl.add(tag + pre + "gemm", {V, Mp}, [=](const Ctx& c) {
                 Level6Params q = lp; q.v = c.ptr(V); q.wc = w6->wc; q.mp = c.ptr(Mp);
                 launch_level6_gemm(q, c.stream);
-            }, 2.0 * G * lp.R * (double)lp.N * lp.Kc, 4.0 * ((double)V.numel() + (double)G * lp.Npad * lp.Kc + (double)Mp.numel()));
+            }, 2.0 * G * lp.R * (double)round_up(lp.N, lp.bn) * lp.Kc, 4.0 * ((double)V.numel() + (double)G * round_up(lp.N, lp.bn) * lp.Kc + (double)Mp.numel()));
             {
                 const PackedConv* pc = &w6->skip;
                 pl.add_conv(tag + ".conv_skip", {s15, sk}, B * hout * hout, lp.N, round_up(9 * l.skip, 32), [=](const Ctx& c, int tile) {
@@ -457,7 +495,7 @@
                 pl.ops.back().wino4_ok = pl.ops.back().wino_ok && lp.N >= h->sw.wino4_min_n && !h->sw.no_wino4;
                 pl.ops.back().wino4x_ok = pl.ops.back().wino_ok && lp.N >= 24 && conv_wino4x_config(lp.N) >= 0 && !h->sw.no_wino4x;
             }
-            pl.add(tag + ".l6_combine", {Mp, sk, mid}, [=](const Ctx& c) {
+            pl.add(tag + pre + "combine", {Mp, sk, mid}, [=](const Ctx& c) {
                 Level6Params q = lp; q.mp = c.ptr(Mp); q.skip = c.ptr(sk); q.bc = w6->bc; q.out = c.ptr(mid);
                 launch_level6_combine(q, c.stream);
             }, 0.0, 4.0 * ((double)Mp.numel() + 2.0 * (double)mid.numel()));
diff --git a/ccvpe_amd/csrc/ccvpe_tune.hip b/ccvpe_amd/csrc/ccvpe_tune.hip
--- a/ccvpe_amd/csrc/ccvpe_tune.hip
+++ b/ccvpe_amd/csrc/ccvpe_tune.hip
@@ -171,10 +171,17 @@
     auto pl = std::make_unique<Plan>();
     int rc = build_plan(h, *pl, key);
     if (rc) return rc;
-    if (pl->l6_wm && (rc = ensure_level6(h, pl->l6_wm)) != 0) {
+    if (pl->l6_wm && (rc = ensure_level6(h, 0, pl->l6_wm, 3u)) != 0) {
         if (h->sw.compose_l6) return rc;
         (void)hipGetLastError();
-        h->l6_failed = true;
+        h->l6_failed[0] = true;
+        pl = std::make_unique<Plan>();
+        if ((rc = build_plan(h, *pl, key))) return rc;
+    }
+    if (pl->l5_wm && (rc = ensure_level6(h, 1, pl->l5_wm, pl->l5_mask)) != 0) {
+        if (h->sw.compose_l5) return rc;
+        (void)hipGetLastError();
+        h->l6_failed[1] = true;
         pl = std::make_unique<Plan>();
         if ((rc = build_plan(h, *pl, key))) return rc;
     }
diff --git a/ccvpe_amd/csrc/ccvpe_weights.hip b/ccvpe_amd/csrc/ccvpe_weights.hip
--- a/ccvpe_amd/csrc/ccvpe_weights.hip
+++ b/ccvpe_amd/csrc/ccvpe_weights.hip
@@ -323,16 +323,20 @@
     return 0;
 }
 
+static void release_level(ccvpe_handle_s* h, int j) {
+    for (void* p : h->l6_allocs[j]) (void)hipFree(p);
+    h->l6_allocs[j].clear();
+    h->l6[j][0] = Level6W{}; h->l6[j][1] = Level6W{};
+    h->l6_wm[j] = 0; h->l6_have[j] = 0;
+}
 void release_level6(ccvpe_handle_s* h) {
-    for (void* p : h->l6_allocs) (void)hipFree(p);
-    h->l6_allocs.clear();
-    h->l6[0] = Level6W{}; h->l6[1] = Level6W{};
-    h->l6_wm = 0;
-}
-
-int level6_shape(const ccvpe_handle_s* h, const DecoderW& d, const DecLevel& l, int& K, int& Kc, int& N, int& Npad) {
-    const PackedConv& dc = d.deconv[0];
-    const PackedConv& ac = d.conva[0];
+    release_level(h, 0);
+    release_level(h, 1);
+}
+
+int level6_shape(const ccvpe_handle_s* h, const DecoderW& d, const DecLevel& l, int j, int& K, int& Kc, int& N, int& Npad) {
+    const PackedConv& dc = d.deconv[j];
+    const PackedConv& ac = d.conva[j];
     const int cw = deconv_width(l, h->sw.pad_concat);
     if (!dc.w || !ac.w || ac.cinp != cw + l.skip || dc.N != 4 * cw || l.dout % 8 || dc.cinp % 4 || ac.N % 4 || l.skip % 8) return -1;
     K = dc.cinp; Kc = round_up(K, 32); N = ac.N; Npad = round_up(N, 128);
@@ -341,21 +345,22 @@
 
 struct Level6AllocScope {
     ccvpe_handle_s* h;
+    int j;
     std::vector<void*> allocs;
     std::vector<size_t> bytes;
-    explicit Level6AllocScope(ccvpe_handle_s* h_) : h(h_) { allocs.swap(h->dev_allocs); bytes.swap(h->dev_alloc_bytes); }
+    Level6AllocScope(ccvpe_handle_s* h_, int j_) : h(h_), j(j_) { allocs.swap(h->dev_allocs); bytes.swap(h->dev_alloc_bytes); }
     ~Level6AllocScope() {
-        h->l6_allocs.insert(h->l6_allocs.end(), h->dev_allocs.begin(), h->dev_allocs.end());
+        h->l6_allocs[j].insert(h->l6_allocs[j].end(), h->dev_allocs.begin(), h->dev_allocs.end());
         h->dev_allocs.swap(allocs); h->dev_alloc_bytes.swap(bytes);
     }
     Level6AllocScope(const Level6AllocScope&) = delete;
     Level6AllocScope& operator=(const Level6AllocScope&) = delete;
 };
 
-static int derive_level6(ccvpe_handle_s* h, Level6W& o, const DecoderW& d, const DecLevel& l, int wm) {
-    const PackedConv& dc = d.deconv[0];
-    const PackedConv& ac = d.conva[0];
-    if (level6_shape(h, d, l, o.K, o.Kc, o.N, o.Npad)) return ccvpe_fail(CCVPE_ESTATE, "level 6 cannot be composed from these packed weights");
+static int derive_level6(ccvpe_handle_s* h, Level6W& o, const DecoderW& d, const DecLevel& l, int j, int wm) {
+    const PackedConv& dc = d.deconv[j];
+    const PackedConv& ac = d.conva[j];
+    if (level6_shape(h, d, l, j, o.K, o.Kc, o.N, o.Npad)) return ccvpe_fail(CCVPE_ESTATE, "level %d cannot be composed from these packed weights", 6 - j);
     const int cw = deconv_width(l, h->sw.pad_concat), cinw = cw + l.skip, N = ac.N;
     const size_t arows = (size_t)round_up(N, conv_igemm_npad());
     std::vector<float> aw(arows * ac.Kpad), ba(N), bd(4 * cw);
@@ -383,7 +388,7 @@
                 bc[(size_t)(rcase * 3 + ccase) * N + n] = (float)acc;
             }
     {
-        Level6AllocScope scope(h);
+        Level6AllocScope scope(h, j);
         if (int rc = upload(h, bc, &o.bc)) return rc;
         if (int rc = pack_conv(h, o.skip, N, 9, l.skip, l.skip, identity_map(l.skip), [&](int n, int t, int c) { return wa(n, t, cw + c); },
                                std::vector<float>(N, 0.f), 3, 3)) return rc;
@@ -392,7 +397,7 @@
     const size_t wc_bytes = (size_t)4 * P * o.Npad * o.Kc * sizeof(float), w2_bytes = (size_t)16 * N * o.Kc * sizeof(double);
     void *wc = nullptr, *w2 = nullptr;
     HIPCHK(hipMalloc(&wc, wc_bytes));
-    h->l6_allocs.push_back(wc);
+    h->l6_allocs[j].push_back(wc);
     o.wc = (float*)wc;
     HIPCHK(hipMemset(wc, 0, wc_bytes));
     HIPCHK(hipMalloc(&w2, w2_bytes));
@@ -402,18 +407,20 @@
     launch_level6_compose(cp, nullptr);
     const hipError_t e = hipDeviceSynchronize();
     (void)hipFree(w2);
-    if (e != hipSuccess) return ccvpe_fail(CCVPE_EHIP, "composing level 6 failed: %s", hipGetErrorString(e));
-    return 0;
-}
-
-int ensure_level6(ccvpe_handle_s* h, int wm) {
-    if (h->l6_wm == wm) return 0;
+    if (e != hipSuccess) return ccvpe_fail(CCVPE_EHIP, "composing level %d failed: %s", 6 - j, hipGetErrorString(e));
+    return 0;
+}
+
+int ensure_level6(ccvpe_handle_s* h, int j, int wm, unsigned mask) {
+    if (h->l6_wm[j] == wm && (h->l6_have[j] & mask) == mask) return 0;
     if (!h->finalized) return ccvpe_fail(CCVPE_ESTATE, "ccvpe_finalize_weights has not been called");
-    release_level6(h);
-    int rc = derive_level6(h, h->l6[0], h->loc, h->vs.loc[0], wm);
-    if (!rc) rc = derive_level6(h, h->l6[1], h->ori, h->vs.ori[0], wm);
-    if (rc) { release_level6(h); return rc; }
-    h->l6_wm = wm;
+    if (h->l6_wm[j] != wm) release_level(h, j);
+    int rc = 0;
+    for (int d = 0; d < 2 && !rc; ++d)
+        if ((mask >> d & 1) && !(h->l6_have[j] >> d & 1)) rc = derive_level6(h, h->l6[j][d], d ? h->ori : h->loc, d ? h->vs.ori[j] : h->vs.loc[j], j, wm);
+    if (rc) { release_level(h, j); return rc; }
+    h->l6_wm[j] = wm;
+    h->l6_have[j] |= mask;
     return 0;
 }
 
@@ -469,7 +476,7 @@
         if (!h->host.count(k) && !optional) return ccvpe_fail(CCVPE_EKEY, "key '%s' was skipped but is required", k.c_str());
     }
     release_level6(h);
-    h->l6_failed = false;
+    h->l6_failed[0] = h->l6_failed[1] = false;
     for (void* p : h->dev_allocs) (void)hipFree(p);
     h->dev_allocs.clear();
     h->dev_alloc_bytes.clear();
@@ -570,7 +577,7 @@
     if (hd.sz_encoder != sizeof(EncoderW) || hd.sz_decoder != sizeof(DecoderW) || hd.sz_conv != sizeof(PackedConv)) return bad("descriptor layout mismatch");
     if (hd.n_allocs == 0 || hd.n_allocs > 100000 || hd.n_relocs > 100000) return bad("implausible buffer / relocation counts");
     release_level6(h);
-    h->l6_failed = false;
+    h->l6_failed[0] = h->l6_failed[1] = false;
     for (void* p : h->dev_allocs) (void)hipFree(p);
     h->dev_allocs.clear(); h->dev_alloc_bytes.clear(); h->plans.clear(); h->last_plan = nullptr; h->finalized = false;
     bool ok = true;
diff --git a/ccvpe_amd/csrc/kernels.h b/ccvpe_amd/csrc/kernels.h
--- a/ccvpe_amd/csrc/kernels.h
+++ b/ccvpe_amd/csrc/kernels.h
@@ -295,6 +295,8 @@
 
 struct Level6Params {
     int wm;
+    int gs;
+    int bn;
     int B;
     int K, Kc;
     int N, Npad;
@@ -308,7 +310,7 @@
     float* out;
 };
 int level6_positions(int wm);
-int level6_rows(int B, int wm, int* bm_out);
+int level6_rows(int B, int wm, int gs, int* bm_out);
 bool level6_supported(const Level6Params& p);
 void launch_level6_transform(const Level6Params& p, hipStream_t s);
 void launch_level6_gemm(const Level6Params& p, hipStream_t s);
diff --git a/ccvpe_amd/csrc/kernels_level6.hip b/ccvpe_amd/csrc/kernels_level6.hip
--- a/ccvpe_amd/csrc/kernels_level6.hip
+++ b/ccvpe_amd/csrc/kernels_level6.hip
@@ -35,17 +35,17 @@
 };
 
 int level6_positions(int wm) { return (wm + 1) * (wm + 1); }
-int level6_rows(int B, int wm, int* bm_out) {
-    const int t = 8 / wm, rows = B * t * t;
+int level6_rows(int B, int wm, int gs, int* bm_out) {
+    const int t = gs / wm, rows = B * t * t;
     const int bm = rows > 64 ? 128 : rows > 32 ? 64 : 32;
     if (bm_out) *bm_out = bm;
     return (rows + bm - 1) / bm * bm;
 }
 
-template <int M>
+template <int M, int GS>
 __global__ __launch_bounds__(128) void level6_transform_kernel(const Level6Params p) {
     using W = Wino<M>;
-    constexpr int NP = W::NP, T = 8 / M;
+    constexpr int NP = W::NP, T = GS / M;
     const int k = (blockIdx.x * 128 + threadIdx.x) * 4;
     if (k >= p.Kc) return;
     const int row = blockIdx.y, cls = blockIdx.z;
@@ -59,7 +59,7 @@
         for (int j = 0; j < NP; ++j) {
             const int y = y0 + i, x = x0 + j;
             d[i][j] = f32x4{0.f, 0.f, 0.f, 0.f};
-            if (live && (unsigned)y < 8u && (unsigned)x < 8u) d[i][j] = *reinterpret_cast<const f32x4*>(p.x + ((size_t)(b * 8 + y) * 8 + x) * p.K + k);
+            if (live && (unsigned)y < (unsigned)GS && (unsigned)x < (unsigned)GS) d[i][j] = *reinterpret_cast<const f32x4*>(p.x + ((size_t)(b * GS + y) * GS + x) * p.K + k);
         }
     f32x4 c[NP][NP];
 #pragma unroll
@@ -89,9 +89,9 @@
         }
 }
 
-template <int BM, int WGM, int WGN>
+template <int BM, int BN, int WGM, int WGN>
 __global__ __launch_bounds__(256) void level6_gemm_kernel(const Level6Params p) {
-    constexpr int BN = 128, MT = 32;
+    constexpr int MT = 32;
     constexpr int WM = BM / WGM, WN = BN / WGN, TM = WM / MT, TN = WN / MT;
     static_assert(WGM * WGN == 4 && TM >= 1 && TN >= 1 && TM * MT * WGM == BM && TN * MT * WGN == BN, "whole MFMA tiles, 4 waves");
     constexpr int AR = BM / 32, BR = BN / 32;
@@ -103,7 +103,7 @@
 
     const int tid = threadIdx.x, lane = tid & 63, wave = tid >> 6;
     const int wm = wave / WGN, wn = wave % WGN;
-    const int nbn = p.Npad / BN, mblocks = p.R / BM;
+    const int nbn = (p.N + BN - 1) / BN, mblocks = p.R / BM;
     const int lid = xcd_remap(blockIdx.x, gridDim.x);
     const int nb = lid % nbn, rest = lid / nbn;
     const int mb = rest % mblocks, g = rest / mblocks;
@@ -206,10 +206,10 @@
     }
 }
 
-template <int M>
+template <int M, int GS>
 __global__ __launch_bounds__(64) void level6_combine_kernel(const Level6Params p) {
     using W = Wino<M>;
-    constexpr int NP = W::NP, T = 8 / M;
+    constexpr int NP = W::NP, T = GS / M, HO = 2 * GS;
     const int n = (blockIdx.x * 64 + threadIdx.x) * 4;
     if (n >= p.N) return;
     const int row = blockIdx.y, cls = blockIdx.z;
@@ -242,8 +242,8 @@
             for (int v = 0; v < NP; ++v)
                 if (W::at(j, v) != 0.f) s += W::at(j, v) * c[i][v];
             const int oy = 2 * (M * ty + i) + py, ox = 2 * (M * tx + j) + px;
-            const int rcase = oy == 0 ? 1 : oy == 15 ? 2 : 0, ccase = ox == 0 ? 1 : ox == 15 ? 2 : 0;
-            const size_t e = ((size_t)(b * 16 + oy) * 16 + ox) * p.N + n;
+            const int rcase = oy == 0 ? 1 : oy == HO - 1 ? 2 : 0, ccase = ox == 0 ? 1 : ox == HO - 1 ? 2 : 0;
+            const size_t e = ((size_t)(b * HO + oy) * HO + ox) * p.N + n;
             s += *reinterpret_cast<const f32x4*>(p.skip + e);
             s += *reinterpret_cast<const f32x4*>(p.bc + (rcase * 3 + ccase) * p.N + n);
 #pragma unroll
@@ -255,35 +255,49 @@
 bool level6_supported(const Level6Params& p) {
     int bm = 0;
     return (p.wm == 4 || p.wm == 2) && p.B > 0 && p.K > 0 && p.K % 4 == 0 && p.Kc % BK == 0 && p.Kc >= p.K && p.N > 0 && p.N % 4 == 0 &&
-           p.Npad % 128 == 0 && p.Npad >= p.N && p.R == level6_rows(p.B, p.wm, &bm) && p.bm == bm;
+           p.Npad % 128 == 0 && p.Npad >= p.N && (p.gs == 8 || p.gs == 16) && p.R == level6_rows(p.B, p.wm, p.gs, &bm) && p.bm == bm &&
+           (p.bn == 128 || (p.bn == 64 && p.bm >= 64));
 }
 
 void launch_level6_transform(const Level6Params& p, hipStream_t s) {
     const dim3 grid((p.Kc / 4 + 127) / 128, p.R, 4);
-    if (p.wm == 4) CCVPE_LAUNCH(level6_transform_kernel<4>, grid, dim3(128), 0, s, p);
-    else CCVPE_LAUNCH(level6_transform_kernel<2>, grid, dim3(128), 0, s, p);
-}
-
-template <int BM, int WGM, int WGN>
+    if (p.gs == 8) {
+        if (p.wm == 4) CCVPE_LAUNCH((level6_transform_kernel<4, 8>), grid, dim3(128), 0, s, p);
+        else CCVPE_LAUNCH((level6_transform_kernel<2, 8>), grid, dim3(128), 0, s, p);
+    } else {
+        if (p.wm == 4) CCVPE_LAUNCH((level6_transform_kernel<4, 16>), grid, dim3(128), 0, s, p);
+        else CCVPE_LAUNCH((level6_transform_kernel<2, 16>), grid, dim3(128), 0, s, p);
+    }
+}
+
+template <int BM, int BN, int WGM, int WGN>
 static void launch_gemm_t(const Level6Params& p, hipStream_t s) {
-    constexpr size_t lds = std::max<size_t>(2 * (BM + 128) * LDK, BM * (128 + 4)) * sizeof(float);
+    constexpr size_t lds = std::max<size_t>(2 * (BM + BN) * LDK, BM * (BN + 4)) * sizeof(float);
     static LdsAttr attr;
-    auto kern = level6_gemm_kernel<BM, WGM, WGN>;
+    auto kern = level6_gemm_kernel<BM, BN, WGM, WGN>;
     ensure_dynamic_lds(attr, reinterpret_cast<const void*>(kern), lds);
-    const int blocks = 4 * level6_positions(p.wm) * (p.R / BM) * (p.Npad / 128);
+    const int blocks = 4 * level6_positions(p.wm) * (p.R / BM) * ((p.N + BN - 1) / BN);
     CCVPE_LAUNCH(kern, dim3(blocks), dim3(256), lds, s, p);
 }
 void launch_level6_gemm(const Level6Params& p, hipStream_t s) {
-    if (p.bm == 128) launch_gemm_t<128, 2, 2>(p, s);
-    else if (p.bm == 64) launch_gemm_t<64, 2, 2>(p, s);
-    else launch_gemm_t<32, 1, 4>(p, s);
+    if (p.bn == 64) {
+        if (p.bm == 128) launch_gemm_t<128, 64, 2, 2>(p, s);
+        else launch_gemm_t<64, 64, 2, 2>(p, s);
+    } else if (p.bm == 128) launch_gemm_t<128, 128, 2, 2>(p, s);
+    else if (p.bm == 64) launch_gemm_t<64, 128, 2, 2>(p, s);
+    else launch_gemm_t<32, 128, 1, 4>(p, s);
 }
 
 void launch_level6_combine(const Level6Params& p, hipStream_t s) {
-    const int t = 8 / p.wm;
+    const int t = p.gs / p.wm;
     const dim3 grid((p.N / 4 + 63) / 64, p.B * t * t, 4);
-    if (p.wm == 4) CCVPE_LAUNCH(level6_combine_kernel<4>, grid, dim3(64), 0, s, p);
-    else CCVPE_LAUNCH(level6_combine_kernel<2>, grid, dim3(64), 0, s, p);
+    if (p.gs == 8) {
+        if (p.wm == 4) CCVPE_LAUNCH((level6_combine_kernel<4, 8>), grid, dim3(64), 0, s, p);
+        else CCVPE_LAUNCH((level6_combine_kernel<2, 8>), grid, dim3(64), 0, s, p);
+    } else {
+        if (p.wm == 4) CCVPE_LAUNCH((level6_combine_kernel<4, 16>), grid, dim3(64), 0, s, p);
+        else CCVPE_LAUNCH((level6_combine_kernel<2, 16>), grid, dim3(64), 0, s, p);
+    }
 }
 
 __device__ __forceinline__ int k_index_dev(int cin, int taps, int tap, int c) {
```

Result: no change. 2734 queries/s, median of 5 (+0.3%).
